# josiahbjorgaard/mca-paper

Hardware: AMD Instinct MI355X
Metric: training samples/sec (fwd+bwd+opt), CMU 4-modality MCA (higher is better)
Workload: dtype bf16; 1 GPU; synthetic CMU 4-modality (MCA fcl), N=2538 D=512 L=5 H=8 F=88, lengths=full, p_drop=0.0; per_gpu_batch=32, global_batch=32, parallelism=dp1, inputs=device-resident, same batch every step, finite_checks=on (device flag, polled), attention_operands=bf16, attention_backward=bf16 one-pass, launch=hipGraph replay (one launch per step), collectives=none

## Files before the change

### include/mca_hip.h

```cpp
#ifndef MCA_HIP_H
#define MCA_HIP_H
#include <stdint.h>

#ifdef __cplusplus
extern "C" {
#endif

typedef void* mca_stream_t;

#define MCA_OK 0
#define MCA_E_BADARG (-1)
#define MCA_E_ALIGN (-2)
#define MCA_E_UNSUPPORTED (-3)
#define MCA_E_LAUNCH (-4)

const char* mca_version(void);

int mca_gemm_nt(const uint16_t* A, int64_t lda, const uint16_t* B, int64_t ldb,
                void* C, int64_t ldc, int out_bf16,
                const float* bias, const float* residual, int64_t ldres, int64_t res_period,
                int64_t M, int64_t N, int64_t K, mca_stream_t stream);

int mca_gemm_nt_lnres(const uint16_t* A, int64_t lda, const uint16_t* B, int64_t ldb, float* C, int64_t ldc,
                      const float* x, int64_t ldx, const float* mean, const float* rstd, const float* gamma,
                      int64_t M, int64_t N, int64_t K, mca_stream_t stream);

int mca_gemm_nt_geglu_bwd(const uint16_t* A, int64_t lda, const uint16_t* B, int64_t ldb, const uint16_t* h,
                          uint16_t* dh, int64_t ldh, int64_t ip, int64_t M, int64_t K, mca_stream_t stream);

int mca_gemm_nt_geglu_fwd(const uint16_t* A, int64_t lda, const uint16_t* W1, int64_t ldb, uint16_t* h, int64_t ldh,
                          uint16_t* g, int64_t ldg, int64_t ip, int64_t M, int64_t K, mca_stream_t stream);

int mca_gemm_tn_acc(const uint16_t* A, int64_t lda, const uint16_t* B, int64_t ldb,
                    float* C, int64_t ldc, int64_t R, int64_t N, int64_t K, mca_stream_t stream);

#define MCA_TN_MAX_GROUP 8
typedef struct mca_tn_desc {
  const uint16_t* A; int64_t lda;
  const uint16_t* B; int64_t ldb;
  float* C; int64_t ldc;
  int64_t N, K;
} mca_tn_desc;
int mca_gemm_tn_acc_group(const mca_tn_desc* d, int n, int64_t R, mca_stream_t stream);

int mca_layernorm_fwd(const float* x, int64_t ldx, const float* gamma, const float* beta,
                      const uint8_t* rowmask, const float* add, int64_t period,
                      float* y, int64_t ldy, int64_t y_bstride,
                      uint16_t* y_bf16, int64_t ld_bf16, int cols_pad,
                      float* mean, float* rstd, int64_t rows, int cols, float eps, mca_stream_t stream);

int mca_layernorm_bwd(const float* dy, int64_t ldy, int64_t y_bstride, int64_t period,
                      const float* x, int64_t ldx, const float* gamma,
                      const float* mean, const float* rstd, const uint8_t* rowmask,
                      float* dx, int64_t lddx, uint16_t* dx_bf16, int64_t ld_bf16,
                      float* dgamma, float* dbeta, float* dxsum, int64_t rows, int cols, mca_stream_t stream);

int mca_geglu_fwd(const uint16_t* h, uint16_t* g, int64_t rows, int ip, mca_stream_t stream);
int mca_geglu_bwd(const uint16_t* dg, const uint16_t* h, uint16_t* dh, int64_t rows, int ip,
                  mca_stream_t stream);

int mca_cast_pad_bf16(const float* src, int64_t lds, int64_t rows, int64_t cols,
                      uint16_t* dst, int64_t ldd, int64_t rows_pad, int64_t cols_pad, int transpose,
                      mca_stream_t stream);
typedef struct { const void* src; void* dst; int64_t lds, rows, cols, ldd, rows_pad, cols_pad; int32_t transpose; float scale; } mca_cast_desc;
int mca_cast_pad_bf16_multi(const mca_cast_desc* descs_dev, int n, mca_stream_t stream);
int mca_f32_to_bf16(const float* src, int64_t lds, uint16_t* dst, int64_t ldd, int64_t rows, int64_t cols,
                    float scale, mca_stream_t stream);
int mca_bcast_rows(const float* src, int64_t lds, float* dst, int64_t ldd, int64_t dst_bstride,
                   int64_t period, int64_t rows, int cols, mca_stream_t stream);
int mca_reduce_rows(const float* src, int64_t lds, int64_t src_bstride, int64_t period,
                    float* dst, int64_t ldd, int64_t rows, int cols, mca_stream_t stream);

int mca_embedding_renorm(float* weight, int64_t rows, int cols, float max_norm, mca_stream_t stream);
int mca_tab_value_fwd(const float* x, const float* w1, const float* b1, uint16_t* h1, uint8_t* padmask,
                      int64_t rows, int cols, float max_value, float padding_value, mca_stream_t stream);
int mca_tab_value_bwd(const float* dh1, int64_t ld, const uint16_t* h1, const float* x, float* dw1, float* db1,
                      int64_t rows, int cols, float max_value, mca_stream_t stream);

#define MCA_MAX_MODALITIES 16
typedef struct { const void* mask; uint8_t* rowmask; int32_t elem_bytes, n, offset, pad_; } mca_mask_desc;
typedef struct { mca_mask_desc m[MCA_MAX_MODALITIES]; int32_t n_mod, batch, n_tokens, n_fusion; } mca_pack_masks_args;
int mca_pack_masks(const mca_pack_masks_args* args, uint8_t* padding, int32_t* present, mca_stream_t stream);

typedef struct { const float* p[MCA_MAX_MODALITIES]; int64_t n[MCA_MAX_MODALITIES]; int32_t count, pad_; } mca_finite_args;
int mca_nonfinite_flag(const mca_finite_args* args, int32_t* flag, int bit, mca_stream_t stream);
int mca_flag_to_host(const int32_t* flag, int32_t* host_pinned, mca_stream_t stream);

int mca_build_keyinfo(const uint8_t* padding, const uint8_t* kgroup, uint8_t* keyinfo,
                      uint8_t* ktile_flags, int batch, int nk, int nk_pad, mca_stream_t stream);

int mca_build_keyhot(const uint8_t* keyinfo, uint16_t* khot, int batch, int nk_pad, mca_stream_t stream);

int mca_attn_vmean(const uint16_t* V, int64_t kv_bstride, int64_t kv_ld, float* vmean,
                   int batch, int nk, int heads, mca_stream_t stream);
int mca_attn_vmean_if_needed(const uint16_t* V, int64_t kv_bstride, int64_t kv_ld, float* vmean, int batch, int nk,
                             int heads, const int32_t* present, int32_t full_bits, mca_stream_t stream);

typedef struct {
  const uint16_t* q; int64_t q_bstride; int64_t q_ld;
  const uint16_t* k; const uint16_t* v; int64_t kv_bstride; int64_t kv_ld;
  uint16_t* o; int64_t o_bstride; int64_t o_ld;
  float* lse;
  const uint32_t* qmask;
  const uint8_t* keyinfo;
  const uint8_t* ktile_flags;
  const int32_t* q_ptr; const uint32_t* q_kt; const int32_t* q_order;
  const float* vmean;
  int batch, heads, nq, nk, nk_pad, n_qtiles, n_ktiles;
  float scale;
  int flags;
  const uint16_t* khot;
} mca_attn_fwd_args;
#define MCA_ATTN_Q_PRESCALED 1
#define MCA_ATTN_LAZY_REFERENCE 2
int mca_attn_fwd(const mca_attn_fwd_args* args, mca_stream_t stream);

int mca_rows_copy_add(const float* src, int64_t src_bstride, float* dst, int64_t dst_bstride, int64_t rows, int cols,
                      int batch, int accumulate, mca_stream_t stream);
int mca_segment_mean_fwd(const float* x, const uint8_t* padding, const int32_t* seg_start, int n_seg, float* out,
                         int32_t* counts, int batch, int n_tokens, int cols, mca_stream_t stream);
int mca_segment_mean_bwd(const float* d_out, const uint8_t* padding, const uint8_t* seg_of_row, const int32_t* counts,
                         int n_seg, float* dx, int batch, int n_tokens, int cols, mca_stream_t stream);

typedef struct { uint8_t* q8; uint8_t* qs; uint8_t* k8; uint8_t* ks; uint8_t* v8t; uint8_t* vs; int n_ktiles; } mca_attn_fp8_operands;
int mca_attn_quant_mxfp8(const uint16_t* q, int64_t q_bstride, int64_t q_ld, const uint16_t* k, const uint16_t* v,
                         int64_t kv_bstride, int64_t kv_ld, const mca_attn_fp8_operands* f, int batch, int heads, int n,
                         mca_stream_t stream);
int mca_attn_fwd_fp8(const mca_attn_fwd_args* args, const mca_attn_fp8_operands* f, mca_stream_t stream);

typedef struct { uint8_t* q8; uint8_t* qs; uint8_t* k8; uint8_t* ks; uint8_t* v8; uint8_t* vs; uint8_t* do8; uint8_t* dos; int n_ktiles; } mca_attn_fp8_bwd_operands;
int mca_attn_quant_bwd_mxfp8(const uint16_t* q, int64_t q_bstride, int64_t q_ld, const uint16_t* k, const uint16_t* v,
                             int64_t kv_bstride, int64_t kv_ld, const uint16_t* d_o, int64_t o_bstride, int64_t o_ld,
                             const mca_attn_fp8_bwd_operands* f, int which, int batch, int heads, int n, mca_stream_t stream);
int mca_attn_bwd_prep(const uint16_t* o, const uint16_t* d_o, int64_t o_bstride, int64_t o_ld,
                      const float* lse, float* delta, float* dvmean,
                      int batch, int heads, int nq, int nk, mca_stream_t stream);

typedef struct {
  const uint16_t* q; int64_t q_bstride; int64_t q_ld;
  const uint16_t* k; const uint16_t* v; int64_t kv_bstride; int64_t kv_ld;
  const uint16_t* d_o; int64_t o_bstride; int64_t o_ld;
  const float* lse; const float* delta; const float* dvmean;
  void* dq; int64_t dq_bstride; int64_t dq_ld; int dq_f32;
  uint16_t* dk; uint16_t* dv; int64_t dkv_bstride; int64_t dkv_ld;
  const uint32_t* qmask; const uint8_t* keyinfo; const uint8_t* ktile_flags;
  const int32_t* q_ptr; const uint32_t* q_kt; const int32_t* q_order; int n_qtiles128, n_ktiles64;
  const int32_t* k_wg; const uint32_t* k_qt; int n_qtiles64, n_kblocks256;
  int batch, heads, nq, nk, nk_pad;
  float scale;
  int flags;
  const uint16_t* khot; const uint16_t* qblk;
  int kblock_keys;
} mca_attn_bwd2_args;
int mca_attn_bwd_dq(const mca_attn_bwd2_args* args, mca_stream_t stream);
int mca_attn_bwd_dkv(const mca_attn_bwd2_args* args, mca_stream_t stream);
int mca_attn_bwd_dq_fp8(const mca_attn_bwd2_args* args, const mca_attn_fp8_bwd_operands* f, mca_stream_t stream);
int mca_attn_bwd_dkv_fp8(const mca_attn_bwd2_args* args, const mca_attn_fp8_bwd_operands* f, mca_stream_t stream);

typedef struct {
  const uint16_t* q; int64_t q_bstride; int64_t q_ld;
  const uint16_t* k; const uint16_t* v; int64_t kv_bstride; int64_t kv_ld;
  const uint16_t* d_o; int64_t o_bstride; int64_t o_ld;
  int64_t q_hstride, o_hstride;
  const float* rowc; const float* dvmean;
  uint16_t* dq; int64_t dq_bstride; int64_t dq_ld;
  uint16_t* dk; uint16_t* dv; int64_t dkv_bstride; int64_t dkv_ld;
  float* dq_acc;
  const uint8_t* keyinfo; const uint8_t* ktile_flags; const uint16_t* khot; const uint16_t* qblk;
  const int32_t* qt_desc; const int32_t* kb_desc; const uint32_t* kb_qt; const uint8_t* visit;
  int n_qtiles, n_kblocks, max_list;
  int n_entries;
  int batch, heads, n, nk_pad, n_ktiles64;
  float scale;
  int flags;
  int split;
} mca_attn_bwd1_args;
int mca_attn_bwd_onepass(const mca_attn_bwd1_args* args, mca_stream_t stream);
int mca_attn_bwd_prep_onepass(const uint16_t* o, const uint16_t* d_o, int64_t o_bstride, int64_t o_ld, const float* lse,
                              const int32_t* row_slot, float* rowc, float* dvmean, int batch, int heads, int n, int n_qtiles,
                              const uint16_t* q, int64_t q_bstride, int64_t q_ld, uint16_t* q_hm, uint16_t* do_hm,
                              mca_stream_t stream);

typedef struct { int32_t slot_a, slot_b; uint32_t and_bits, or_bits; } mca_loss_term;
int64_t mca_contrastive_workspace_bytes(int B, int T);
int mca_contrastive_fwd_bwd(const float* pooled_all, const uint32_t* present_all,
                            const mca_loss_term* terms, int T, const float* logit_scale,
                            int B, int b_local, int row0, int R, int D,
                            float* term_loss, float* loss, float* d_pooled, float* d_logit_scale,
                            void* workspace, mca_stream_t stream);

#define MCA_SQNORM_WORDS 1026
int mca_grad_sqnorm(const float* g, int64_t n, float* sqnorm, mca_stream_t stream);
int mca_adamw_step(float* p, const float* g, float* m, float* v, int64_t n,
                   float lr, float beta1, float beta2, float eps, float weight_decay,
                   float bias_corr1, float bias_corr2, float max_norm, const float* sqnorm,
                   const int32_t* skip_flag, const float* hyper, mca_stream_t stream);
int mca_adamw_hyper(float* hyper, float lr, float bias_corr1, float bias_corr2, mca_stream_t stream);

int mca_rows_normalize_f32(const float* x, int64_t ldx, float* y, int64_t ldy, int64_t n, int64_t d, mca_stream_t stream);
int mca_cosine_rank_f32(const float* q, int64_t ldq, const int32_t* qidx, int64_t nq, const float* t, int64_t ldt, int64_t nt,
                        int64_t d, float* s_true, int32_t* rank, mca_stream_t stream);
int64_t mca_pair_gauss_workspace(int64_t n);
int mca_pair_gauss_sum_f32(const float* x, int64_t ldx, int64_t n, int64_t d, float t, double* partials, int64_t n_partials,
                           double* sum_out, float* value_out, mca_stream_t stream);
int mca_probe_nt_f32(const float* x, int64_t ldx, const int32_t* xidx, const float* w, int64_t ldw, const float* bias, float* y,
                     int64_t ldy, int64_t M, int64_t N, int64_t K, int act, float p, uint64_t seed, int64_t step, mca_stream_t stream);
int64_t mca_probe_head_blocks(int64_t B);
int mca_probe_head_f32(const float* a, int64_t lda, const int32_t* aidx, int64_t K, const float* w, const float* bias, int64_t L,
                       const float* labels, const int32_t* yidx, int64_t B, int loss_type, float* pred, float* dz, float* da,
                       float dact_scale, float* loss_part, mca_stream_t stream);
int64_t mca_probe_tn_workspace(int64_t R, int64_t N, int64_t K);
int mca_probe_tn_f32(const float* a, int64_t lda, const float* b, int64_t ldb, const int32_t* bidx, int64_t R, int64_t N, int64_t K,
                     float* partials, int64_t n_partials, float* gw, float* gb, mca_stream_t stream);
int mca_probe_loss_accum(const float* loss_part, int64_t n, int64_t count, float* acc, mca_stream_t stream);

#ifdef __cplusplus
}
#endif
#endif
```

### mca-paper_amd/csrc/attention_bwd1.hip

```cpp
#include "common.h"

#define DH 64
#define TQ 64
#define TKB 256
#define B1_NST 2
#define B1_STAGE_U16 (TQ * DH * 2 + 256 + TQ * 16)
#define B1_MAX_QT 256
#define B1_MAX_KB 64
#define B1_MAX_LIST 256
#define B1_MAX_META 768
typedef unsigned u32x4v __attribute__((ext_vector_type(4)));
typedef unsigned u32x2v __attribute__((ext_vector_type(2)));

__device__ __forceinline__ int b1_off(int r, int c) {
  const int s = ((r >> 1) & 7) ^ (((r >> 1) & 1) << 2);
  return r * 64 + ((c ^ s) << 3);
}
__device__ __forceinline__ int b1_swz(int r) { return ((r >> 1) & 7) ^ (((r >> 1) & 1) << 2); }

#define B1_DMA(SRC, DST, BYTES) __builtin_amdgcn_global_load_lds((const __attribute__((address_space(1))) void*)(SRC), (__attribute__((address_space(3))) void*)(DST), BYTES, 0, 0)

__global__ __launch_bounds__(256, 1) void attn_bwd1_kernel(mca_attn_bwd1_args a, int dbg) {
  extern __shared__ __attribute__((aligned(16))) u16 lds[];
  u16* stage_s = lds;
  u16* kimg = stage_s + B1_NST * B1_STAGE_U16;
  u16* dsimg = kimg + TKB * DH;
  uint32_t* list_s = reinterpret_cast<uint32_t*>(dsimg + 2 * TKB * TQ);
  uint8_t* first_s = reinterpret_cast<uint8_t*>(list_s + B1_MAX_LIST);
  uint8_t* last_s = first_s + B1_MAX_QT;
  uint8_t* live_s = last_s + B1_MAX_QT;
  float* dvm_s = reinterpret_cast<float*>(live_s + B1_MAX_KB);

  const int lin = (dbg & 16) ? (int)blockIdx.x : xcd_remap((int)blockIdx.x, (int)gridDim.x);
  const int h = lin % a.heads, b = lin / a.heads;
  const int tid = threadIdx.x, lane = tid & 63, wave = __builtin_amdgcn_readfirstlane(tid >> 6);
  const int l31 = lane & 31, lh = lane >> 5;
  const int tq = (lane & 15) >> 2, tp = lane & 3, tg = (lane >> 4) & 1;
  const int64_t bh = (int64_t)b * a.heads + h;

  const u16* qbase = a.q + (int64_t)b * a.q_bstride + h * (a.q_hstride ? a.q_hstride : (int64_t)DH);
  const u16* obase = a.d_o + (int64_t)b * a.o_bstride + h * (a.o_hstride ? a.o_hstride : (int64_t)DH);
  const u16* kbase = a.k + (int64_t)b * a.kv_bstride + h * DH;
  const u16* vbase = a.v + (int64_t)b * a.kv_bstride + h * DH;
  const float* rowc_g = a.rowc + bh * (int64_t)(a.n_qtiles + 1) * 128;
  float* acc_g = a.dq_acc + bh * (int64_t)(a.n_qtiles + 1) * (TQ * DH);
  const uint8_t* kinfo_g = a.keyinfo + (int64_t)b * a.nk_pad;
  const u16* khot_g = a.khot + (int64_t)b * a.nk_pad * 16;

  if (tid < a.n_kblocks) {
    const int4 d = reinterpret_cast<const int4*>(a.kb_desc)[tid];
    const uint8_t* fl = a.ktile_flags + (int64_t)b * a.n_ktiles64;
    int live = 0;
    for (int t = d.x >> 6; t <= (d.x + d.y - 1) >> 6; t++) live |= fl[t];
    live_s[tid] = live ? 1 : 0;
  }
  if (tid < DH) dvm_s[tid] = a.dvmean[(int64_t)b * a.heads * DH + h * DH + tid];
  __syncthreads();
  for (int qt = tid; qt < a.n_qtiles; qt += 256) {
    int first = 255, last = 255;
    for (int kb = 0; kb < a.n_kblocks; kb++)
      if (live_s[kb] && a.visit[kb * a.n_qtiles + qt]) { if (first == 255) first = kb; last = kb; }
    first_s[qt] = (uint8_t)first; last_s[qt] = (uint8_t)last;
  }
  __syncthreads();
  for (int qt = 0; qt < a.n_qtiles; qt++) {
    if (first_s[qt] != 255) continue;
    const int2 qd = reinterpret_cast<const int2*>(a.qt_desc)[qt];
    for (int i = tid; i < qd.y * 8; i += 256)
      *reinterpret_cast<uint4*>(a.dq + (int64_t)b * a.dq_bstride + (int64_t)(qd.x + (i >> 3)) * a.dq_ld + h * DH + (i & 7) * 8) = make_uint4(0, 0, 0, 0);
  }

  int rowfrag[4];
#pragma unroll
  for (int st = 0; st < 4; st++) rowfrag[st] = b1_off(l31, 2 * st + lh);
  const float dk_scale = 0.6931471805599453f;

  for (int kbi = 0; kbi < a.n_kblocks; kbi++) {
    if (!live_s[kbi]) continue;
    const int4 kd = reinterpret_cast<const int4*>(a.kb_desc)[kbi];
    const int key_start = __builtin_amdgcn_readfirstlane(kd.x), n_keys = __builtin_amdgcn_readfirstlane(kd.y);
    const int e_begin = __builtin_amdgcn_readfirstlane(kd.z), n_ent = __builtin_amdgcn_readfirstlane(kd.w);
    for (int i = tid; i < n_ent; i += 256) list_s[i] = a.kb_qt[e_begin + i];

    bf16x8 kf[2][4], vf[2][4], khf[2];
    bool ok[2];
    int keyrow[2];
#pragma unroll
    for (int kb = 0; kb < 2; kb++) {
      const int slot = wave * 64 + kb * 32 + l31;
      const bool valid = slot < n_keys;
      const int key = key_start + (valid ? slot : n_keys - 1);
      keyrow[kb] = valid ? key : -1;
      ok[kb] = valid && kinfo_g[key] != 31;
#pragma unroll
      for (int s = 0; s < 4; s++) {
        kf[kb][s] = *reinterpret_cast<const bf16x8*>(kbase + (int64_t)key * a.kv_ld + 16 * s + 8 * lh);
// ... 280 lines not shown
  asm volatile("s_mov_b32 m0, %2\n\ts_nop 0\n\tglobal_load_lds_dword %0, %1" :: "v"(OFF), "s"(BASE), "s"(LDS_DST) : "memory")
#define LDS_P(T, ADDR) reinterpret_cast<__attribute__((address_space(3))) T*>(static_cast<uintptr_t>(ADDR))
#define LDS_R8(ADDR) (*LDS_P(const bf16x8, ADDR))
#define LDS_RF4(ADDR) (*LDS_P(const f32x4, ADDR))
#define LDS_TR(ADDR) __builtin_amdgcn_ds_read_tr16_b64_v4i16(LDS_P(bf16x4, ADDR))

MCA_TRACE_BUFFER(attn_bwd1)
#ifdef MCA_TRACE_BUILD
#define B1_STAMP() do { if (trace_on) { const unsigned long long t_ = __builtin_amdgcn_s_memtime(); if (lane == 0) mca_trace_attn_bwd1[tr_n & 1023] = t_; tr_n++; } } while (0)
#define B1_NOTE(V) do { if (trace_on) { if (lane == 0) mca_trace_attn_bwd1[tr_n & 1023] = (unsigned long long)(V); tr_n++; } } while (0)
#define B1_TR(K_) asm volatile("s_memtime %0" : "=s"(tr_t[K_]))
#define B1_TR_END() do { asm volatile("s_memtime %0\n\ts_waitcnt lgkmcnt(0)" : "=s"(tr_t[6]) :: "memory");                      \
                         if (trace_on && it == 8 && lane == 0) {                                                                 \
                           for (int k_ = 0; k_ < 7; k_++) mca_trace_attn_bwd1[512 + tr_blk * 8 + k_] = tr_t[k_]; } } while (0)
#else
#define B1_STAMP() do {} while (0)
#define B1_NOTE(V) do {} while (0)
#define B1_TR(K_) do {} while (0)
#define B1_TR_END() do {} while (0)
#endif
#define M_QT(M) ((M).x & 0xffff)
#define M_FIRST(M) (((M).x >> 16) & 1)
#define M_LAST(M) (((M).x >> 17) & 1)
#define M_ROWS(M) ((int)((unsigned)(M).x >> 20))
#define M_ROW0(M) ((M).y)

__device__ __forceinline__ void attn_bwd1p_body(const mca_attn_bwd1_args& a, const int dbg, u16* lds) {
  u16* stage_s = lds;
  u16* kimg = stage_s + B1P_NST * B1_STAGE_U16;
  u16* dsimg = kimg + TKB * DH;
  int2* meta_s = reinterpret_cast<int2*>(dsimg + 2 * TKB * TQ);
  int4* kbd_s = reinterpret_cast<int4*>(meta_s + B1_MAX_META);
  int2* qtd_s = reinterpret_cast<int2*>(dsimg);
  uint8_t* first_s = reinterpret_cast<uint8_t*>(qtd_s + B1_MAX_QT);
  uint8_t* last_s = first_s + B1_MAX_QT;
  uint8_t* live_s = reinterpret_cast<uint8_t*>(kbd_s + B1_MAX_KB);
  float* dvm_s = reinterpret_cast<float*>(live_s + B1_MAX_KB);

  const int lin = (dbg & 16) ? (int)blockIdx.x : xcd_remap((int)blockIdx.x, (int)gridDim.x);
  const int S = a.split > 1 ? a.split : 1;
  const int bh_ = lin / S, sid = lin - bh_ * S;
  const int h = bh_ % a.heads, b = bh_ / a.heads;
  const int tid = threadIdx.x, lane = tid & 63, wave = __builtin_amdgcn_readfirstlane(tid >> 6);
#ifdef MCA_TRACE_BUILD
  const bool trace_on = lin == 0 && wave == 0 && (dbg & 8);
  int tr_n = 0, tr_blk = 0;
#endif
  const int l31 = lane & 31, lh = lane >> 5;
  const int tq = (lane & 15) >> 2, tp = lane & 3, tg = (lane >> 4) & 1;
  const int64_t bh = (int64_t)b * a.heads + h;

  const u16* qbase = a.q + (int64_t)b * a.q_bstride + h * (a.q_hstride ? a.q_hstride : (int64_t)DH);
  const u16* obase = a.d_o + (int64_t)b * a.o_bstride + h * (a.o_hstride ? a.o_hstride : (int64_t)DH);
  const u16* kbase = a.k + (int64_t)b * a.kv_bstride + h * DH;
  const u16* vbase = a.v + (int64_t)b * a.kv_bstride + h * DH;
  const float* rowc_g = a.rowc + bh * (int64_t)(a.n_qtiles + 1) * 128;
  float* acc_s = a.dq_acc + (bh * S + sid) * (int64_t)(a.n_qtiles + 1) * (TQ * DH) + wave * 1024;
  const uint8_t* kinfo_g = a.keyinfo + (int64_t)b * a.nk_pad;
  const u16* khot_g = a.khot + (int64_t)b * a.nk_pad * 16;

  if (tid < a.n_kblocks) {
    const int4 d = reinterpret_cast<const int4*>(a.kb_desc)[tid];
    const uint8_t* fl = a.ktile_flags + (int64_t)b * a.n_ktiles64;
    int live = 0;
    for (int t = d.x >> 6; t <= (d.x + d.y - 1) >> 6; t++) live |= fl[t];
    const bool mine = tid % S == sid;
    live_s[tid] = (live && mine) ? 1 : ((!live && mine) ? 2 : 0);
    kbd_s[tid] = d;
  }
  if (tid < DH) dvm_s[tid] = a.dvmean[(int64_t)b * a.heads * DH + h * DH + tid];
  for (int qt = tid; qt < a.n_qtiles; qt += 256) qtd_s[qt] = reinterpret_cast<const int2*>(a.qt_desc)[qt];
  if (tid == 0) { qtd_s[a.n_qtiles] = make_int2(0, 1); first_s[a.n_qtiles] = 255; last_s[a.n_qtiles] = 255; }
  __syncthreads();
  for (int qt = tid; qt < a.n_qtiles; qt += 256) {
    int first = 255, last = 255;
    for (int kb = 0; kb < a.n_kblocks; kb++)
      if (live_s[kb] == 1 && a.visit[kb * a.n_qtiles + qt]) { if (first == 255) first = kb; last = kb; }
    first_s[qt] = (uint8_t)first; last_s[qt] = (uint8_t)last;
  }
  int* mtot_s = reinterpret_cast<int*>(dvm_s + DH);
  if (tid == 0) {
    int off = 0;
    for (int kb = 0; kb < a.n_kblocks; kb++) {
      int4 d = kbd_s[kb];
      const int e_begin = d.z;
      d.z = off;
      if (live_s[kb] == 1) off += ((d.w + 2) & ~1) + 2;
      kbd_s[kb] = make_int4(d.x, d.y, d.z | (e_begin << 16), d.w);
    }
    *mtot_s = off;
  }
  __syncthreads();
  {
    const int total = *mtot_s;
    for (int e = tid; e < total; e += 256) {
      int kb = 0;
      for (int k = 1; k < a.n_kblocks; k++) if ((kbd_s[k].z & 0xffff) <= e) kb = k;
      while (live_s[kb] != 1) kb--;
      const int4 d = kbd_s[kb];
      const int mo = d.z & 0xffff, e_begin = d.z >> 16, n_ent = d.w, i = e - mo;
      const int qt = i < n_ent ? (int)(a.kb_qt[e_begin + i] & 0x7fffffffu) : a.n_qtiles;
      const int2 qd = qtd_s[qt];
      meta_s[e] = make_int2(qt | (((int)first_s[qt] == kb ? 1 : 0) << 16) | (((int)last_s[qt] == kb && S == 1 ? 2 : 0) << 16) | (qd.y << 20), qd.x);
    }
  }
  __syncthreads();
  for (int qt = 0; qt < a.n_qtiles; qt++) {
    if (first_s[qt] != 255) continue;
// ... 403 lines not shown
    tr_blk++;
#endif
    kbi = nxt;
  }
#ifdef MCA_TRACE_BUILD
  if (trace_on && lane == 0) mca_trace_attn_bwd1[1023] = (unsigned long long)tr_n;
#endif
  for (int kbi = 0; kbi < a.n_kblocks; kbi++) {
    if (live_s[kbi] != 2) continue;
    const int4 kd = reinterpret_cast<const int4*>(a.kb_desc)[kbi];
    for (int i = tid; i < kd.y * 8; i += 256) {
      const int key = kd.x + (i >> 3), c = i & 7;
      *reinterpret_cast<uint4*>(a.dk + (int64_t)b * a.dkv_bstride + (int64_t)key * a.dkv_ld + h * DH + c * 8) = make_uint4(0, 0, 0, 0);
      uint4 pv;
      pv.x = pack2bf(dvm_s[c * 8], dvm_s[c * 8 + 1]); pv.y = pack2bf(dvm_s[c * 8 + 2], dvm_s[c * 8 + 3]);
      pv.z = pack2bf(dvm_s[c * 8 + 4], dvm_s[c * 8 + 5]); pv.w = pack2bf(dvm_s[c * 8 + 6], dvm_s[c * 8 + 7]);
      *reinterpret_cast<uint4*>(a.dv + (int64_t)b * a.dkv_bstride + (int64_t)key * a.dkv_ld + h * DH + c * 8) = pv;
    }
  }
}
__global__ __launch_bounds__(256) void attn_bwd1_reduce_kernel(mca_attn_bwd1_args a) {
  const int qt = blockIdx.x, bh = blockIdx.y, h = bh % a.heads, b = bh / a.heads, S = a.split;
  const int tid = threadIdx.x, lane = tid & 63, wave = tid >> 6;
  const int2 qd = reinterpret_cast<const int2*>(a.qt_desc)[qt];
  const int r = (wave >> 1) * 32 + (lane & 31);
#pragma unroll
  for (int g = 0; g < 4; g++) {
    f32x4 acc = {0.f, 0.f, 0.f, 0.f};
    for (int s = 0; s < S; s++) {
      const f32x4 v = *reinterpret_cast<const f32x4*>(a.dq_acc + (((int64_t)bh * S + s) * (a.n_qtiles + 1) + qt) * (TQ * DH) + wave * 1024 + g * 256 + lane * 4);
      acc[0] += v[0]; acc[1] += v[1]; acc[2] += v[2]; acc[3] += v[3];
    }
    if (r < qd.y) {
      uint2 pk;
      pk.x = pack2bf(acc[0] * a.scale, acc[1] * a.scale); pk.y = pack2bf(acc[2] * a.scale, acc[3] * a.scale);
      *reinterpret_cast<uint2*>(a.dq + (int64_t)b * a.dq_bstride + (int64_t)(qd.x + r) * a.dq_ld + h * DH + (wave & 1) * 32 + 8 * g + 4 * (lane >> 5)) = pk;
    }
  }
}
__global__ __launch_bounds__(256, 1) void attn_bwd1p_kernel(mca_attn_bwd1_args a, int dbg) {
  extern __shared__ __attribute__((aligned(16))) u16 lds_dyn[];
  attn_bwd1p_body(a, dbg, lds_dyn);
}
#define B1P_LDS_BYTES ((B1P_NST * B1_STAGE_U16 + TKB * DH + 2 * TKB * TQ) * 2 + B1_MAX_META * 8 + B1_MAX_KB * 16 + B1_MAX_KB + DH * 4 + 16)

#define B1_LDS_BYTES ((B1_NST * B1_STAGE_U16 + TKB * DH + 2 * TKB * TQ) * 2 + B1_MAX_LIST * 4 + 2 * B1_MAX_QT + B1_MAX_KB + DH * 4)

extern "C" int mca_attn_bwd_onepass(const mca_attn_bwd1_args* a, mca_stream_t stream) {
  if (!a || !a->q || !a->k || !a->v || !a->d_o || !a->rowc || !a->dvmean || !a->dq || !a->dk || !a->dv || !a->dq_acc) return MCA_E_BADARG;
  if (!a->keyinfo || !a->ktile_flags || !a->khot || !a->qblk || !a->qt_desc || !a->kb_desc || !a->kb_qt || !a->visit) return MCA_E_BADARG;
  if (a->batch <= 0 || a->heads <= 0 || a->n <= 0 || a->n_qtiles <= 0 || a->n_kblocks <= 0) return MCA_E_BADARG;
  if (a->n_qtiles >= B1_MAX_QT || a->n_kblocks > B1_MAX_KB || a->max_list + 6 > B1_MAX_LIST ||
      a->n_entries + 4 * a->n_kblocks > B1_MAX_META) return MCA_E_UNSUPPORTED;
  if (a->q_ld % 8 || a->kv_ld % 8 || a->o_ld % 8 || a->q_bstride % 8 || a->kv_bstride % 8 || a->o_bstride % 8 || a->q_hstride % 8 || a->o_hstride % 8) return MCA_E_ALIGN;
  if ((uintptr_t)a->q % 16 || (uintptr_t)a->k % 16 || (uintptr_t)a->v % 16 || (uintptr_t)a->d_o % 16 || (uintptr_t)a->khot % 16 || (uintptr_t)a->qblk % 16) return MCA_E_ALIGN;
  if (a->dq_ld % 8 || a->dq_bstride % 8 || (uintptr_t)a->dq % 16 || a->dkv_ld % 8 || a->dkv_bstride % 8 || (uintptr_t)a->dk % 16 || (uintptr_t)a->dv % 16) return MCA_E_ALIGN;
  if ((uintptr_t)a->dq_acc % 16 || (uintptr_t)a->rowc % 4 || (uintptr_t)a->kb_desc % 16 || (uintptr_t)a->qt_desc % 8) return MCA_E_ALIGN;
  if (a->nk_pad < a->n || a->n_ktiles64 != (a->n + 63) / 64) return MCA_E_BADARG;
  if (!(a->flags & MCA_ATTN_Q_PRESCALED)) return MCA_E_UNSUPPORTED;
  if ((int64_t)a->batch * a->heads > 0x7fffffff) return MCA_E_UNSUPPORTED;
  static bool attr_set[64] = {false};
  bool* done = mca_dev_flag(attr_set);
  if (!*done) {
    if (hipFuncSetAttribute(reinterpret_cast<const void*>(attn_bwd1_kernel), hipFuncAttributeMaxDynamicSharedMemorySize, B1_LDS_BYTES) != hipSuccess ||
        hipFuncSetAttribute(reinterpret_cast<const void*>(attn_bwd1p_kernel), hipFuncAttributeMaxDynamicSharedMemorySize, B1P_LDS_BYTES) != hipSuccess)
      return MCA_E_LAUNCH;
    *done = true;
  }
  const bool packed = a->q_ld == DH && a->o_ld == DH && a->q_hstride && a->o_hstride;
  const int split = a->split > 1 ? a->split : 1;
  if (split > 8) return MCA_E_UNSUPPORTED;
  if (split > 1 && !packed) return MCA_E_UNSUPPORTED;
  if ((mca_knobs[9] & 64 && split == 1) || !packed) hipLaunchKernelGGL(attn_bwd1_kernel, dim3(a->batch * a->heads), dim3(256), B1_LDS_BYTES, as_stream(stream), *a, mca_knobs[9]);
  else hipLaunchKernelGGL(attn_bwd1p_kernel, dim3(a->batch * a->heads * split), dim3(256), B1P_LDS_BYTES, as_stream(stream), *a, mca_knobs[9]);
  if (split > 1) hipLaunchKernelGGL(attn_bwd1_reduce_kernel, dim3(a->n_qtiles, a->batch * a->heads), dim3(256), 0, as_stream(stream), *a);
  return launch_status();
}
```

### mca-paper_amd/csrc/attention_bwd2.hip

```cpp
#include "common.h"

#define DH 64
#define AQ 128
#define AK 64
#define MAX_KTILES 512
#define BQ 64
#define MAX_QTILES 2048
typedef unsigned u32x4v __attribute__((ext_vector_type(4)));

__device__ __forceinline__ int rt_off(int r, int c) {
  const int s = ((r >> 1) & 7) ^ (((r >> 1) & 1) << 2);
  return r * 64 + ((c ^ s) << 3);
}
__device__ __forceinline__ int row_off(int r, int c) { return r * 64 + ((c ^ ((r >> 1) & 7)) << 3); }

template <bool OUT_F32, bool HOT>
__global__ __launch_bounds__(256, 2) void attn_bwd_dq_kernel(mca_attn_bwd2_args a, int dbg) {
  constexpr bool PRESCALED = true;
  __shared__ __attribute__((aligned(16))) u16 lds[2 * 2 * AK * DH];
  __shared__ __attribute__((aligned(16))) uint8_t kinfo[2][AK];
  __shared__ __attribute__((aligned(16))) u16 hot_s[2][AK * 16];
  __shared__ uint8_t flags_s[MAX_KTILES];
  __shared__ uint32_t live_s[MAX_KTILES + 2];
  __shared__ int n_live_s;
// ... 498 lines not shown
#pragma unroll
    for (int n = 0; n < 2; n++)
#pragma unroll
      for (int g = 0; g < 4; g++) {
        const int d = n * 32 + 8 * g + 4 * lh;
        uint2 pk;
        pk.x = pack2bf(dk[n][4 * g] * dk_scale, dk[n][4 * g + 1] * dk_scale);
        pk.y = pack2bf(dk[n][4 * g + 2] * dk_scale, dk[n][4 * g + 3] * dk_scale);
        *reinterpret_cast<uint2*>(dkp + d) = pk;
        const f32x4 dvm = *reinterpret_cast<const f32x4*>(dvm_s + d);
        pk.x = pack2bf(dv[n][4 * g] + dvm[0], dv[n][4 * g + 1] + dvm[1]);
        pk.y = pack2bf(dv[n][4 * g + 2] + dvm[2], dv[n][4 * g + 3] + dvm[3]);
        *reinterpret_cast<uint2*>(dvp + d) = pk;
      }
  }
}
#define DKV_LDS_BYTES (2 * BQ * DH * 2 * 2 + 2 * 192 * 4 + MAX_QTILES * 4 + DH * 4 + 2 * BQ * 16 * 2)

extern "C" int mca_attn_bwd_dkv(const mca_attn_bwd2_args* a, mca_stream_t stream) {
  const int rc = check_bwd2(a);
  if (rc != MCA_OK) return rc;
  if (!a->dk || !a->dv || !a->dvmean || !a->k_wg || !a->k_qt) return MCA_E_BADARG;
  const int BKEYS = a->kblock_keys ? a->kblock_keys : 256;
  if (BKEYS != 256 && BKEYS != 128) return MCA_E_UNSUPPORTED;
  if (a->n_qtiles64 != (a->nq + BQ - 1) / BQ || a->n_kblocks256 != (a->nk + BKEYS - 1) / BKEYS) return MCA_E_BADARG;
  if (a->nk_pad < a->n_kblocks256 * BKEYS) return MCA_E_BADARG;
  if (a->dkv_ld % 4 || a->dkv_bstride % 4 || (uintptr_t)a->dk % 8 || (uintptr_t)a->dv % 8 || (uintptr_t)a->k_wg % 16) return MCA_E_ALIGN;
  if (a->n_qtiles64 > MAX_QTILES) return MCA_E_UNSUPPORTED;
  if ((a->khot != nullptr) != (a->qblk != nullptr)) return MCA_E_BADARG;
  if ((uintptr_t)a->khot % 16 || (uintptr_t)a->qblk % 16) return MCA_E_ALIGN;
  if (!(a->flags & MCA_ATTN_Q_PRESCALED)) return MCA_E_UNSUPPORTED;
  int dev = 0;
  static bool attr_set[64] = {false};
  if (hipGetDevice(&dev) != hipSuccess || dev < 0 || dev >= 64) return MCA_E_LAUNCH;
  if (!attr_set[dev]) {
    if (hipFuncSetAttribute(reinterpret_cast<const void*>(attn_bwd_dkv_kernel<8>), hipFuncAttributeMaxDynamicSharedMemorySize, DKV_LDS_BYTES) != hipSuccess ||
        hipFuncSetAttribute(reinterpret_cast<const void*>(attn_bwd_dkv_kernel<4>), hipFuncAttributeMaxDynamicSharedMemorySize, DKV_LDS_BYTES) != hipSuccess)
      return MCA_E_LAUNCH;
    attr_set[dev] = true;
  }
  const dim3 grid(a->n_kblocks256, a->heads, a->batch);
#define DKV_LAUNCH(W) hipLaunchKernelGGL((attn_bwd_dkv_kernel<W>), grid, dim3(64 * W), DKV_LDS_BYTES, as_stream(stream), *a, mca_knobs[9])
  if (BKEYS == 256) DKV_LAUNCH(8); else DKV_LAUNCH(4);
#undef DKV_LAUNCH
  return launch_status();
}

#define PREP_ROWS 32
__device__ __forceinline__ void attn_bwd_prep_block(const int bx, const int by, const u16* __restrict__ o, const u16* __restrict__ d_o,
                                                    int64_t bstride, int64_t ld, float* __restrict__ delta, int heads, int nq,
                                                    const float* __restrict__ lse, const int32_t* __restrict__ row_slot,
                                                    float* __restrict__ rowc, int n_qtiles,
                                                    const u16* __restrict__ qsrc, int64_t q_bstride, int64_t q_ld,
                                                    u16* __restrict__ q_hm, u16* __restrict__ do_hm) {
  __shared__ float del_s[8][PREP_ROWS];
  const int b = by, tid = threadIdx.x, lane = tid & 63, wave = tid >> 6;
  const int cols = heads * DH;
  const int q_begin = bx * PREP_ROWS;
  int q_end = q_begin + PREP_ROWS; if (q_end > nq) q_end = nq;
  for (int c0 = 0; c0 < cols; c0 += 512) {
    const int h0 = c0 / DH;
    const int c = c0 + lane * 8;
    const int hl = lane >> 3;
    bf16x8 ovs[PREP_ROWS / 4], dvs[PREP_ROWS / 4], qvs[PREP_ROWS / 4];
#pragma unroll
    for (int k = 0; k < PREP_ROWS / 4; k++) {
      int q = q_begin + wave + 4 * k; if (q > nq - 1) q = nq - 1;
      const int cc = c < cols ? c : 0;
      ovs[k] = *reinterpret_cast<const bf16x8*>(o + (int64_t)b * bstride + (int64_t)q * ld + cc);
      dvs[k] = *reinterpret_cast<const bf16x8*>(d_o + (int64_t)b * bstride + (int64_t)q * ld + cc);
      if (do_hm) qvs[k] = *reinterpret_cast<const bf16x8*>(qsrc + (int64_t)b * q_bstride + (int64_t)q * q_ld + cc);
    }
#pragma unroll
    for (int k = 0; k < PREP_ROWS / 4; k++) {
      const int q = q_begin + wave + 4 * k;
      if (q >= q_end) break;
      if (do_hm && c < cols) {
        const int64_t dst = (((int64_t)b * heads + h0 + hl) * nq + q) * DH + (lane & 7) * 8;
        *reinterpret_cast<bf16x8*>(do_hm + dst) = dvs[k];
        *reinterpret_cast<bf16x8*>(q_hm + dst) = qvs[k];
      }
      float part = 0.f;
      if (c < cols) {
#pragma unroll
        for (int j = 0; j < 8; j++) part += bf2f((u16)dvs[k][j]) * bf2f((u16)ovs[k][j]);
      }
      part += __shfl_xor(part, 1, WAVE); part += __shfl_xor(part, 2, WAVE); part += __shfl_xor(part, 4, WAVE);
      if ((lane & 7) == 0) del_s[hl][q - q_begin] = part;
    }
    __syncthreads();
    {
      const int hh = tid / PREP_ROWS, r = tid % PREP_ROWS;
      if (h0 + hh < heads && q_begin + r < q_end) {
        if (!row_slot) delta[((int64_t)b * heads + h0 + hh) * nq + q_begin + r] = del_s[hh][r];
        else {
          const int q = q_begin + r, slot = row_slot[q];
          float* dst = rowc + (((int64_t)b * heads + h0 + hh) * (n_qtiles + 1) + (slot >> 6)) * 128 + (slot & 63);
          dst[0] = -lse[((int64_t)b * heads + h0 + hh) * nq + q];
          dst[64] = -del_s[hh][r];
        }
      }
    }
    __syncthreads();
  }
}

#define DVM_MAX_LIST 4096
__device__ __forceinline__ void attn_dvmean_block(const int bx, const int by, const u16* __restrict__ d_o, int64_t bstride, int64_t ld,
                                                  const float* __restrict__ lse, float* __restrict__ dvmean,
                                                  int heads, int nq, float inv_nk) {
  __shared__ int list_s[DVM_MAX_LIST];
  __shared__ int n_s;
  __shared__ float red[32][DH + 1];
  const int h = bx, b = by, tid = threadIdx.x, lane = tid & 63, wave = tid >> 6;
  const float* l = lse + ((int64_t)b * heads + h) * nq;
  float* out = dvmean + (int64_t)b * heads * DH + h * DH;
  {
    int anyu = 0;
    for (int q = tid; q < nq; q += 256) anyu |= (l[q] == INFINITY) ? 1 : 0;
    if (tid == 0) n_s = 0;
    if (!__syncthreads_or(anyu)) { if (tid < DH) out[tid] = 0.f; return; }
  }
  const int cl = tid & 7, rg = tid >> 3;
  float acc[8] = {0, 0, 0, 0, 0, 0, 0, 0};
  auto flush = [&]() {
    const int n = n_s;
    for (int i = rg; i < n; i += 32) {
      const bf16x8 v = *reinterpret_cast<const bf16x8*>(d_o + (int64_t)b * bstride + (int64_t)list_s[i] * ld + h * DH + cl * 8);
#pragma unroll
      for (int j = 0; j < 8; j++) acc[j] += bf2f((u16)v[j]);
    }
    __syncthreads();
    if (tid == 0) n_s = 0;
    __syncthreads();
  };
  for (int q0 = 0; q0 < nq; q0 += 256) {
    const int q = q0 + tid;
    const bool uni = q < nq && l[q] == INFINITY;
    const unsigned long long m = __ballot(uni);
    for (int w = 0; w < 4; w++) {
      if (wave == w && m) {
        const int base = n_s;
        if (uni) list_s[base + __popcll(m & ((1ull << lane) - 1ull))] = q;
        if (lane == 0) n_s = base + __popcll(m);
      }
      __syncthreads();
    }
    if (n_s > DVM_MAX_LIST - 256) flush();
  }
  flush();
#pragma unroll
  for (int j = 0; j < 8; j++) red[rg][cl * 8 + j] = acc[j];
  __syncthreads();
  if (tid < DH) {
    float t = 0.f;
    for (int r = 0; r < 32; r++) t += red[r][tid];
    out[tid] = t * inv_nk;
  }
}
__global__ __launch_bounds__(256) void attn_bwd_prep_kernel(const u16* __restrict__ o, const u16* __restrict__ d_o, int64_t bstride, int64_t ld,
                                                             const float* __restrict__ lse, float* __restrict__ delta,
                                                             float* __restrict__ dvmean, int heads, int nq, float inv_nk, int n_prep,
                                                             const int32_t* __restrict__ row_slot, float* __restrict__ rowc, int n_qtiles,
                                                             const u16* __restrict__ qsrc, int64_t q_bstride, int64_t q_ld,
                                                             u16* __restrict__ q_hm, u16* __restrict__ do_hm) {
  if ((int)blockIdx.x < n_prep) attn_bwd_prep_block((int)blockIdx.x, (int)blockIdx.y, o, d_o, bstride, ld, delta, heads, nq, lse, row_slot, rowc, n_qtiles,
                                                    qsrc, q_bstride, q_ld, q_hm, do_hm);
  else attn_dvmean_block((int)blockIdx.x - n_prep, (int)blockIdx.y, d_o, bstride, ld, lse, dvmean, heads, nq, inv_nk);
}
extern "C" int mca_attn_bwd_prep(const uint16_t* o, const uint16_t* d_o, int64_t o_bstride, int64_t o_ld,
                                 const float* lse, float* delta, float* dvmean, int batch, int heads, int nq, int nk,
                                 mca_stream_t stream) {
  if (!o || !d_o || !lse || !delta || !dvmean || batch <= 0 || heads <= 0 || nq <= 0 || nk <= 0) return MCA_E_BADARG;
  if (o_ld % 8 || o_bstride % 8 || (uintptr_t)o % 16 || (uintptr_t)d_o % 16) return MCA_E_ALIGN;
  if (heads > 65535 || batch > 65535) return MCA_E_UNSUPPORTED;
  const int n_prep = (nq + PREP_ROWS - 1) / PREP_ROWS;
  hipLaunchKernelGGL(attn_bwd_prep_kernel, dim3(n_prep + heads, batch), dim3(256), 0, as_stream(stream), o, d_o, o_bstride, o_ld, lse, delta,
                     dvmean, heads, nq, 1.f / (float)nk, n_prep, (const int32_t*)nullptr, (float*)nullptr, 0, (const u16*)nullptr, (int64_t)0, (int64_t)0,
                     (u16*)nullptr, (u16*)nullptr);
  return launch_status();
}
extern "C" int mca_attn_bwd_prep_onepass(const uint16_t* o, const uint16_t* d_o, int64_t o_bstride, int64_t o_ld, const float* lse,
                                         const int32_t* row_slot, float* rowc, float* dvmean, int batch, int heads, int n, int n_qtiles,
                                         const uint16_t* q, int64_t q_bstride, int64_t q_ld, uint16_t* q_hm, uint16_t* do_hm,
                                         mca_stream_t stream) {
  if (!o || !d_o || !lse || !row_slot || !rowc || !dvmean || batch <= 0 || heads <= 0 || n <= 0 || n_qtiles <= 0) return MCA_E_BADARG;
  if ((q_hm != nullptr) != (do_hm != nullptr) || (q_hm && !q)) return MCA_E_BADARG;
  if (q_hm && (q_ld % 8 || q_bstride % 8 || (uintptr_t)q % 16 || (uintptr_t)q_hm % 16 || (uintptr_t)do_hm % 16)) return MCA_E_ALIGN;
  if (o_ld % 8 || o_bstride % 8 || (uintptr_t)o % 16 || (uintptr_t)d_o % 16) return MCA_E_ALIGN;
  if (heads > 65535 || batch > 65535) return MCA_E_UNSUPPORTED;
  const int n_prep = (n + PREP_ROWS - 1) / PREP_ROWS;
  hipLaunchKernelGGL(attn_bwd_prep_kernel, dim3(n_prep + heads, batch), dim3(256), 0, as_stream(stream), o, d_o, o_bstride, o_ld, lse, (float*)nullptr,
                     dvmean, heads, n, 1.f / (float)n, n_prep, row_slot, rowc, n_qtiles, q, q_bstride, q_ld, q_hm, do_hm);
  return launch_status();
}
```

### mca-paper_amd/csrc/attention_fwd.hip

```cpp
#include "common.h"

#define AQ 128
#define AK 64
#define DH 64
#define MAX_KTILES 512
typedef unsigned u32x4v __attribute__((ext_vector_type(4)));

MCA_TRACE_BUFFER(attn_fwd)
#ifdef MCA_TRACE_BUILD
#define FW_STAMP() do { if (tracing && ti < 1017) mca_trace_attn_fwd[ti++] = __builtin_readcyclecounter(); } while (0)
#else
#define FW_STAMP() do { } while (0)
#endif

__device__ __forceinline__ int k_off(int r, int c) { return r * 64 + ((c ^ ((r >> 1) & 7)) << 3); }
__device__ __forceinline__ int v_off(int r, int c) { return r * 64 + ((c ^ (((r >> 1) & 1) << 2)) << 3); }

__global__ __launch_bounds__(256) void attn_fwd_kernel(mca_attn_fwd_args a, int dbg) {
  constexpr bool PRESCALED = true;
  __shared__ __attribute__((aligned(16))) u16 lds[2 * 2 * AK * DH];
  __shared__ __attribute__((aligned(16))) uint8_t kinfo[2][AK];
  __shared__ __attribute__((aligned(16))) u16 hot_s[2][AK * 16];
  __shared__ uint8_t flags_s[MAX_KTILES];
  __shared__ uint32_t live_s[MAX_KTILES];
  __shared__ int n_live_s;
  u16* Ks = lds;
  u16* Vs = lds + 2 * AK * DH;

  const int lin0 = (int)(blockIdx.x + gridDim.x * (blockIdx.y + gridDim.y * blockIdx.z));
  const int lin = (dbg & 16) ? lin0 : xcd_remap(lin0, (int)(gridDim.x * gridDim.y * gridDim.z));
  const int qt = a.q_order[lin % (int)gridDim.x];
  const int h = (lin / (int)gridDim.x) % (int)gridDim.y, b = lin / (int)(gridDim.x * gridDim.y);
  const int tid = threadIdx.x, lane = tid & 63, wave = tid >> 6;
  const int l31 = lane & 31, lh = lane >> 5;
  const int q0 = qt * AQ + wave * 32;
  int qrow = q0 + l31;
  const bool qvalid = qrow < a.nq;
  if (qrow > a.nq - 1) qrow = a.nq - 1;

  bf16x8 qf[4];
  {
    const u16* qp = a.q + (int64_t)b * a.q_bstride + (int64_t)qrow * a.q_ld + h * DH + 8 * lh;
#pragma unroll
    for (int s = 0; s < 4; s++) qf[s] = *reinterpret_cast<const bf16x8*>(qp + 16 * s);
  }
  const uint32_t qm = a.qmask[qrow];
  const bool use_hot = a.khot != nullptr;
  bf16x8 qblk;
#pragma unroll
  for (int j = 0; j < 8; j++) {
    const int g = 8 * lh + j;
    qblk[j] = (g < 15 && ((qm >> g) & 1u)) ? (short)0 : (short)0xC700;
  }
  const float c2 = PRESCALED ? 1.f : a.scale * 1.4426950408889634f;

  f32x16 o[2];
#pragma unroll
  for (int n = 0; n < 2; n++)
#pragma unroll
    for (int r = 0; r < 16; r++) o[n][r] = 0.f;
  float m_run = -INFINITY, l_run = 0.f;

  const u16* kbase = a.k + (int64_t)b * a.kv_bstride + h * DH;
  const u16* vbase = a.v + (int64_t)b * a.kv_bstride + h * DH;
  const uint8_t* kinfo_g = a.keyinfo + (int64_t)b * a.nk_pad;
  const u16* khot_g = use_hot ? a.khot + (int64_t)b * a.nk_pad * 16 : nullptr;
  {
    const uint8_t* flags_g = a.ktile_flags + (int64_t)b * a.n_ktiles;
    for (int i = tid; i < a.n_ktiles; i += 256) flags_s[i] = flags_g[i];
  }
  __syncthreads();

  int srow[2], sc[2];
  unsigned loff[2];
#pragma unroll
  for (int i = 0; i < 2; i++) {
    const int id = tid + 256 * i; srow[i] = id >> 3; sc[i] = id & 7;
    loff[i] = (unsigned)(srow[i] * (int)a.kv_ld + sc[i] * 8);
  }
  const int last_kt = a.n_ktiles - 1;
  bf16x8 rk[2], rv[2];
  uint32_t rinfo = 0;
  uint4 rhot = make_uint4(0, 0, 0, 0);
  auto gload = [&](int kt) {
    if (use_hot) { if (tid < 128) rhot = *reinterpret_cast<const uint4*>(khot_g + ((int64_t)kt * AK + (tid >> 1)) * 16 + (tid & 1) * 8); }
    else if (tid < 16) rinfo = *reinterpret_cast<const uint32_t*>(kinfo_g + kt * AK + tid * 4);
    const u16* kb = kbase + (int64_t)kt * AK * a.kv_ld;
    const u16* vb = vbase + (int64_t)kt * AK * a.kv_ld;
    if (kt != last_kt) {
#pragma unroll
      for (int i = 0; i < 2; i++) {
        rk[i] = *reinterpret_cast<const bf16x8*>(kb + loff[i]);
        rv[i] = *reinterpret_cast<const bf16x8*>(vb + loff[i]);
      }
    } else {
#pragma unroll
      for (int i = 0; i < 2; i++) {
        int key = kt * AK + srow[i]; if (key > a.nk - 1) key = a.nk - 1;
        rk[i] = *reinterpret_cast<const bf16x8*>(kbase + (int64_t)key * a.kv_ld + sc[i] * 8);
        rv[i] = *reinterpret_cast<const bf16x8*>(vbase + (int64_t)key * a.kv_ld + sc[i] * 8);
      }
    }
  };
  auto swrite = [&](int buf) {
#pragma unroll
    for (int i = 0; i < 2; i++) {
      *reinterpret_cast<bf16x8*>(Ks + buf * AK * DH + k_off(srow[i], sc[i])) = rk[i];
      *reinterpret_cast<bf16x8*>(Vs + buf * AK * DH + v_off(srow[i], sc[i])) = rv[i];
    }
    if (use_hot) { if (tid < 128) *reinterpret_cast<uint4*>(&hot_s[buf][(tid >> 1) * 16 + (tid & 1) * 8]) = rhot; }
    else if (tid < 16) *reinterpret_cast<uint32_t*>(&kinfo[buf][tid * 4]) = rinfo;
  };

  if (wave == 0) {
    const int lb = a.q_ptr[qt], le = a.q_ptr[qt + 1];
    int n = 0;
    for (int i0 = lb; i0 < le; i0 += 64) {
// ... 115 lines not shown
    buf ^= 1;
    it = nit;
  }

#ifdef MCA_TRACE_BUILD
  if (tracing) {
    mca_trace_attn_fwd[1020] = __builtin_amdgcn_s_memrealtime() - rt0; mca_trace_attn_fwd[1021] = __builtin_readcyclecounter() - cy0;
  }
#endif
  const bool uniform = !(l_run > 0.f) || m_run < -16384.f * c2;
  const float inv = uniform ? 0.f : 1.f / l_run;
  if (qvalid) {
    if (lh == 0) a.lse[((int64_t)b * a.heads + h) * a.nq + qrow] = uniform ? INFINITY : m_run + log2f(l_run);
    u16* op = a.o + (int64_t)b * a.o_bstride + (int64_t)qrow * a.o_ld + h * DH;
    const float* vm = a.vmean + (int64_t)b * a.heads * DH + h * DH;
#pragma unroll
    for (int n = 0; n < 2; n++)
#pragma unroll
      for (int g = 0; g < 4; g++) {
        const int d = n * 32 + 8 * g + 4 * lh;
        float v0, v1, v2, v3;
        if (uniform) { v0 = vm[d]; v1 = vm[d + 1]; v2 = vm[d + 2]; v3 = vm[d + 3]; }
        else { v0 = o[n][4 * g] * inv; v1 = o[n][4 * g + 1] * inv; v2 = o[n][4 * g + 2] * inv; v3 = o[n][4 * g + 3] * inv; }
        uint2 pk; pk.x = pack2bf(v0, v1); pk.y = pack2bf(v2, v3);
        *reinterpret_cast<uint2*>(op + d) = pk;
      }
  }
}



__global__ __launch_bounds__(256, 4) void attn_fwd4_kernel(mca_attn_fwd_args a, int dbg) {
  __shared__ __attribute__((aligned(16))) u16 lds[2 * 2 * AK * DH + 2 * AK * 16];
  __shared__ uint8_t flags_s[MAX_KTILES];
  __shared__ uint32_t live_s[MAX_KTILES];
  __shared__ int n_live_s;
  u16* Ks = lds;
  u16* Vs = lds + 2 * AK * DH;
  u16* Hs = lds + 4 * AK * DH;

  const int lin0 = (int)(blockIdx.x + gridDim.x * (blockIdx.y + gridDim.y * blockIdx.z));
  const int lin = (dbg & 16) ? lin0 : xcd_remap(lin0, (int)(gridDim.x * gridDim.y * gridDim.z));
  const int qt = a.q_order[lin % (int)gridDim.x];
  const int h = (lin / (int)gridDim.x) % (int)gridDim.y, b = lin / (int)(gridDim.x * gridDim.y);
  const int tid = threadIdx.x, lane = tid & 63, wave = __builtin_amdgcn_readfirstlane(tid >> 6);
  const int l31 = lane & 31, lh = lane >> 5;
  const int q0 = qt * AQ + wave * 32;
  int qrow = q0 + l31;
  const bool qvalid = qrow < a.nq;
  if (qrow > a.nq - 1) qrow = a.nq - 1;

  bf16x8 qf[4];
  {
    const u16* qp = a.q + (int64_t)b * a.q_bstride + (int64_t)qrow * a.q_ld + h * DH + 8 * lh;
#pragma unroll
    for (int s = 0; s < 4; s++) qf[s] = *reinterpret_cast<const bf16x8*>(qp + 16 * s);
  }
  const uint32_t qm = a.qmask[qrow];
  const uint32_t qm8 = ((qm >> (8 * lh)) & 0xffu) & (lh ? 0x7fu : 0xffu);

  f32x16 o[2];
#pragma unroll
  for (int n = 0; n < 2; n++)
#pragma unroll
    for (int r = 0; r < 16; r++) o[n][r] = 0.f;
  float m_run = -INFINITY, l_run = 0.f;

  const u16* kbase = a.k + (int64_t)b * a.kv_bstride + h * DH;
  const u16* vbase = a.v + (int64_t)b * a.kv_bstride + h * DH;
  const u16* khot_g = a.khot + (int64_t)b * a.nk_pad * 16;
  {
    const uint8_t* flags_g = a.ktile_flags + (int64_t)b * a.n_ktiles;
    for (int i = tid; i < a.n_ktiles; i += 256) flags_s[i] = flags_g[i];
  }
  __syncthreads();

  int prow[2];
  unsigned koff[2], voff[2];
#pragma unroll
  for (int i = 0; i < 2; i++) {
    const int p = 256 * i + tid, r = p >> 3, sl = p & 7;
    prow[i] = r;
    koff[i] = (unsigned)(r * (int)a.kv_ld + ((sl ^ ((r >> 1) & 7)) << 3));
    voff[i] = (unsigned)(r * (int)a.kv_ld + ((sl ^ (((r >> 1) & 1) << 2)) << 3));
  }
  const int last_kt = a.n_ktiles - 1;
  auto stage = [&](int kt, int buf) {
    const u16* kb = kbase + (int64_t)kt * AK * a.kv_ld;
    const u16* vb = vbase + (int64_t)kt * AK * a.kv_ld;
#pragma unroll
    for (int i = 0; i < 2; i++) {
      unsigned ko = koff[i], vo = voff[i];
      if (kt == last_kt) {
        int key = kt * AK + prow[i]; const int over = key - (a.nk - 1);
        if (over > 0) { ko -= (unsigned)(over * (int)a.kv_ld); vo -= (unsigned)(over * (int)a.kv_ld); }
      }
      u16* dk = Ks + buf * AK * DH + (i * 4 + wave) * 512;
      u16* dv = Vs + buf * AK * DH + (i * 4 + wave) * 512;
      __builtin_amdgcn_global_load_lds((const __attribute__((address_space(1))) void*)(kb + ko), (__attribute__((address_space(3))) void*)dk, 16, 0, 0);
      __builtin_amdgcn_global_load_lds((const __attribute__((address_space(1))) void*)(vb + vo), (__attribute__((address_space(3))) void*)dv, 16, 0, 0);
    }
    if (wave < 2) {
      u16* dh = Hs + buf * AK * 16 + wave * 512;
      __builtin_amdgcn_global_load_lds((const __attribute__((address_space(1))) void*)(khot_g + (int64_t)kt * (AK * 16) + tid * 8),
                                       (__attribute__((address_space(3))) void*)dh, 16, 0, 0);
    }
  };

  if (wave == 0) {
    const int lb = a.q_ptr[qt], le = a.q_ptr[qt + 1];
    int n = 0;
    for (int i0 = lb; i0 < le; i0 += 64) {
      const int i = i0 + lane;
      const uint32_t e = i < le ? a.q_kt[i] : 0u;
      const uint8_t fl = i < le ? flags_s[e & 0x7fffffffu] : (uint8_t)0;
      const bool keep = fl != 0;
      const unsigned long long m = __ballot(keep);
      if (keep) live_s[n + __popcll(m & ((1ull << lane) - 1ull))] = (e & 0x7fffffffu) | (((e >> 31) && fl == 2) ? 0x80000000u : 0u);
      n += __popcll(m);
    }
    if (lane == 0) n_live_s = n;
  }
// ... 75 lines not shown
            const bf16x4 v4 = lds_read_tr16(vs + v_off(key, d >> 3) + (d & 7));
#pragma unroll
            for (int e = 0; e < 4; e++) vf[4 * t + e] = v4[e];
          }
          o[n] = __builtin_amdgcn_mfma_f32_32x32x16_bf16(vf, *reinterpret_cast<const bf16x8*>(&pw[kb][sp]), o[n], 0, 0, 0);
        }
    asm volatile("s_waitcnt vmcnt(0)" ::: "memory");
    __syncthreads();
    buf ^= 1;
  }

  const bool uniform = !(l_run > 0.f) || m_run < -16384.f;
  const float inv = uniform ? 0.f : 1.f / l_run;
  if (qvalid) {
    if (lh == 0) a.lse[((int64_t)b * a.heads + h) * a.nq + qrow] = uniform ? INFINITY : m_run + log2f(l_run);
    u16* op = a.o + (int64_t)b * a.o_bstride + (int64_t)qrow * a.o_ld + h * DH;
    const float* vm = a.vmean + (int64_t)b * a.heads * DH + h * DH;
#pragma unroll
    for (int n = 0; n < 2; n++)
#pragma unroll
      for (int g = 0; g < 4; g++) {
        const int d = n * 32 + 8 * g + 4 * lh;
        float v0, v1, v2, v3;
        if (uniform) { v0 = vm[d]; v1 = vm[d + 1]; v2 = vm[d + 2]; v3 = vm[d + 3]; }
        else { v0 = o[n][4 * g] * inv; v1 = o[n][4 * g + 1] * inv; v2 = o[n][4 * g + 2] * inv; v3 = o[n][4 * g + 3] * inv; }
        uint2 pk; pk.x = pack2bf(v0, v1); pk.y = pack2bf(v2, v3);
        *reinterpret_cast<uint2*>(op + d) = pk;
      }
  }
}

__global__ __launch_bounds__(256, 3) void attn_fwd4l_kernel(mca_attn_fwd_args a, int dbg, float thr) {
  __shared__ __attribute__((aligned(16))) u16 lds[2 * 2 * AK * DH + 2 * AK * 16];
  __shared__ uint8_t flags_s[MAX_KTILES];
  __shared__ uint32_t live_s[MAX_KTILES];
  __shared__ int n_live_s;
  u16* Ks = lds;
  u16* Vs = lds + 2 * AK * DH;
  u16* Hs = lds + 4 * AK * DH;

  const int lin0 = (int)(blockIdx.x + gridDim.x * (blockIdx.y + gridDim.y * blockIdx.z));
  const int lin = (dbg & 16) ? lin0 : xcd_remap(lin0, (int)(gridDim.x * gridDim.y * gridDim.z));
  const int qt = a.q_order[lin % (int)gridDim.x];
  const int h = (lin / (int)gridDim.x) % (int)gridDim.y, b = lin / (int)(gridDim.x * gridDim.y);
  const int tid = threadIdx.x, lane = tid & 63, wave = __builtin_amdgcn_readfirstlane(tid >> 6);
  const int l31 = lane & 31, lh = lane >> 5;
  const int q0 = qt * AQ + wave * 32;
  int qrow = q0 + l31;
  const bool qvalid = qrow < a.nq;
  if (qrow > a.nq - 1) qrow = a.nq - 1;

  bf16x8 qf[4];
  {
    const u16* qp = a.q + (int64_t)b * a.q_bstride + (int64_t)qrow * a.q_ld + h * DH + 8 * lh;
#pragma unroll
    for (int s = 0; s < 4; s++) qf[s] = *reinterpret_cast<const bf16x8*>(qp + 16 * s);
  }
  const uint32_t qm = a.qmask[qrow];
  const uint32_t qm8 = ((qm >> (8 * lh)) & 0xffu) & (lh ? 0x7fu : 0xffu);

  f32x16 o[2];
#pragma unroll
  for (int n = 0; n < 2; n++)
#pragma unroll
    for (int r = 0; r < 16; r++) o[n][r] = 0.f;
  f32x16 negm;
#pragma unroll
  for (int r = 0; r < 16; r++) negm[r] = 0.f;
  float l_run = 0.f;

  const u16* kbase = a.k + (int64_t)b * a.kv_bstride + h * DH;
  const u16* vbase = a.v + (int64_t)b * a.kv_bstride + h * DH;
  const u16* khot_g = a.khot + (int64_t)b * a.nk_pad * 16;
  {
    const uint8_t* flags_g = a.ktile_flags + (int64_t)b * a.n_ktiles;
    for (int i = tid; i < a.n_ktiles; i += 256) flags_s[i] = flags_g[i];
  }
  __syncthreads();

  int prow[2];
  unsigned koff[2], voff[2];
#pragma unroll
  for (int i = 0; i < 2; i++) {
    const int p = 256 * i + tid, r = p >> 3, sl = p & 7;
    prow[i] = r;
    koff[i] = (unsigned)(r * (int)a.kv_ld + ((sl ^ ((r >> 1) & 7)) << 3));
    voff[i] = (unsigned)(r * (int)a.kv_ld + ((sl ^ (((r >> 1) & 1) << 2)) << 3));
  }
  const int last_kt = a.n_ktiles - 1;
  auto stage = [&](int kt, int buf) {
    const u16* kb = kbase + (int64_t)kt * AK * a.kv_ld;
    const u16* vb = vbase + (int64_t)kt * AK * a.kv_ld;
#pragma unroll
    for (int i = 0; i < 2; i++) {
      unsigned ko = koff[i], vo = voff[i];
      if (kt == last_kt) {
        int key = kt * AK + prow[i]; const int over = key - (a.nk - 1);
        if (over > 0) { ko -= (unsigned)(over * (int)a.kv_ld); vo -= (unsigned)(over * (int)a.kv_ld); }
      }
      u16* dk = Ks + buf * AK * DH + (i * 4 + wave) * 512;
      u16* dv = Vs + buf * AK * DH + (i * 4 + wave) * 512;
      __builtin_amdgcn_global_load_lds((const __attribute__((address_space(1))) void*)(kb + ko), (__attribute__((address_space(3))) void*)dk, 16, 0, 0);
      __builtin_amdgcn_global_load_lds((const __attribute__((address_space(1))) void*)(vb + vo), (__attribute__((address_space(3))) void*)dv, 16, 0, 0);
    }
    if (wave < 2) {
      u16* dh = Hs + buf * AK * 16 + wave * 512;
      __builtin_amdgcn_global_load_lds((const __attribute__((address_space(1))) void*)(khot_g + (int64_t)kt * (AK * 16) + tid * 8),
                                       (__attribute__((address_space(3))) void*)dh, 16, 0, 0);
    }
  };

  if (wave == 0) {
    const int lb = a.q_ptr[qt], le = a.q_ptr[qt + 1];
    int n = 0;
    for (int i0 = lb; i0 < le; i0 += 64) {
      const int i = i0 + lane;
      const uint32_t e = i < le ? a.q_kt[i] : 0u;
      const uint8_t fl = i < le ? flags_s[e & 0x7fffffffu] : (uint8_t)0;
      const bool keep = fl != 0;
      const unsigned long long m = __ballot(keep);
      if (keep) live_s[n + __popcll(m & ((1ull << lane) - 1ull))] = (e & 0x7fffffffu) | (((e >> 31) && fl == 2) ? 0x80000000u : 0u);
      n += __popcll(m);
    }
    if (lane == 0) n_live_s = n;
  }
// ... 71 lines not shown
#pragma unroll
      for (int sp = 0; sp < 2; sp++)
#pragma unroll
        for (int n = 0; n < 2; n++) {
          bf16x8 vf;
#pragma unroll
          for (int t = 0; t < 2; t++) {
            const int key = kb * 32 + 16 * sp + 8 * t + 4 * lh + tq;
            const int d = n * 32 + 16 * tg + 4 * tp;
            const bf16x4 v4 = lds_read_tr16(vs + v_off(key, d >> 3) + (d & 7));
#pragma unroll
            for (int e = 0; e < 4; e++) vf[4 * t + e] = v4[e];
          }
          o[n] = __builtin_amdgcn_mfma_f32_32x32x16_bf16(vf, *reinterpret_cast<const bf16x8*>(&pw[kb][sp]), o[n], 0, 0, 0);
        }
    asm volatile("s_waitcnt vmcnt(0)" ::: "memory");
    __syncthreads();
    buf ^= 1;
  }

  const float l_tot = l_run + __shfl_xor(l_run, 32, WAVE);
  const float m_run = -negm[0];
  const bool uniform = !(l_tot > 0.f);
  const float inv = uniform ? 0.f : 1.f / l_tot;
  if (qvalid) {
    if (lh == 0) a.lse[((int64_t)b * a.heads + h) * a.nq + qrow] = uniform ? INFINITY : m_run + log2f(l_tot);
    u16* op = a.o + (int64_t)b * a.o_bstride + (int64_t)qrow * a.o_ld + h * DH;
    const float* vm = a.vmean + (int64_t)b * a.heads * DH + h * DH;
#pragma unroll
    for (int n = 0; n < 2; n++)
#pragma unroll
      for (int g = 0; g < 4; g++) {
        const int d = n * 32 + 8 * g + 4 * lh;
        float v0, v1, v2, v3;
        if (uniform) { v0 = vm[d]; v1 = vm[d + 1]; v2 = vm[d + 2]; v3 = vm[d + 3]; }
        else { v0 = o[n][4 * g] * inv; v1 = o[n][4 * g + 1] * inv; v2 = o[n][4 * g + 2] * inv; v3 = o[n][4 * g + 3] * inv; }
        uint2 pk; pk.x = pack2bf(v0, v1); pk.y = pack2bf(v2, v3);
        *reinterpret_cast<uint2*>(op + d) = pk;
      }
  }
}

extern "C" int mca_attn_fwd(const mca_attn_fwd_args* a, mca_stream_t stream) {
  if (!a || !a->q || !a->k || !a->v || !a->o || !a->lse || !a->qmask || !a->keyinfo || !a->ktile_flags || !a->q_ptr ||
      !a->q_kt || !a->q_order || !a->vmean)
    return MCA_E_BADARG;
  if (a->batch <= 0 || a->heads <= 0 || a->nq <= 0 || a->nk <= 0) return MCA_E_BADARG;
  if (a->n_qtiles != (a->nq + AQ - 1) / AQ || a->n_ktiles != (a->nk + AK - 1) / AK) return MCA_E_BADARG;
  if (a->nk_pad < a->n_ktiles * AK || a->nk_pad % 4) return MCA_E_BADARG;
  if (a->q_ld % 8 || a->kv_ld % 8 || a->o_ld % 4 || a->q_bstride % 8 || a->kv_bstride % 8 || a->o_bstride % 4) return MCA_E_ALIGN;
  if ((uintptr_t)a->q % 16 || (uintptr_t)a->k % 16 || (uintptr_t)a->v % 16 || (uintptr_t)a->o % 8 ||
      (uintptr_t)a->keyinfo % 4)
    return MCA_E_ALIGN;
  if (a->heads > 65535 || a->batch > 65535 || a->n_ktiles > MAX_KTILES) return MCA_E_UNSUPPORTED;
  const dim3 grid(a->n_qtiles, a->heads, a->batch);
  if (!(a->flags & MCA_ATTN_Q_PRESCALED)) return MCA_E_UNSUPPORTED;
  if ((uintptr_t)a->khot % 16) return MCA_E_ALIGN;
  const bool dma = a->khot && (int64_t)a->kv_ld * 64 < (1ll << 30);
  if (dma && (a->flags & MCA_ATTN_LAZY_REFERENCE))
    hipLaunchKernelGGL(attn_fwd4l_kernel, grid, dim3(256), 0, as_stream(stream), *a, mca_knobs[9], 12.f);
  else if (dma)
    hipLaunchKernelGGL(attn_fwd4_kernel, grid, dim3(256), 0, as_stream(stream), *a, mca_knobs[9]);
  else
    hipLaunchKernelGGL(attn_fwd_kernel, grid, dim3(256), 0, as_stream(stream), *a, mca_knobs[9] | mca_knobs[8]);
  return launch_status();
}

__global__ __launch_bounds__(64) void build_keyinfo_kernel(const uint8_t* __restrict__ padding,
                                                            const uint8_t* __restrict__ kgroup,
                                                            uint8_t* __restrict__ keyinfo, uint8_t* __restrict__ flags,
                                                            int nk, int nk_pad, int n_ktiles) {
  const int b = blockIdx.y, kt = blockIdx.x, lane = threadIdx.x;
  const int key = kt * AK + lane;
  uint8_t info = 31;
  if (key < nk && !padding[(int64_t)b * nk + key]) info = kgroup[key];
  if (key < nk_pad) keyinfo[(int64_t)b * nk_pad + key] = info;
  const unsigned long long valid = __ballot(info != 31);
  if (lane == 0 && kt < n_ktiles) {
    const int in_tile = (nk - kt * AK) < AK ? (nk - kt * AK) : AK;
    const int nvalid = __popcll(valid);
    flags[(int64_t)b * n_ktiles + kt] = nvalid == 0 ? 0 : (nvalid == AK && in_tile == AK ? 2 : 1);
  }
}
extern "C" int mca_build_keyinfo(const uint8_t* padding, const uint8_t* kgroup, uint8_t* keyinfo,
                                 uint8_t* ktile_flags, int batch, int nk, int nk_pad, mca_stream_t stream) {
  if (!padding || !kgroup || !keyinfo || !ktile_flags || batch <= 0 || nk <= 0) return MCA_E_BADARG;
  const int n_ktiles = (nk + AK - 1) / AK;
  if (nk_pad < n_ktiles * AK) return MCA_E_BADARG;
  const int ntile_pad = (nk_pad + AK - 1) / AK;
  hipLaunchKernelGGL(build_keyinfo_kernel, dim3(ntile_pad, batch), dim3(64), 0, as_stream(stream), padding, kgroup,
                     keyinfo, ktile_flags, nk, nk_pad, n_ktiles);
  return launch_status();
}

__global__ __launch_bounds__(256) void build_keyhot_kernel(const uint8_t* __restrict__ keyinfo, u16* __restrict__ khot, int64_t n) {
  const int64_t i = (int64_t)blockIdx.x * 256 + threadIdx.x;
  if (i >= n) return;
  const int g = keyinfo[i] >= 15 ? 15 : keyinfo[i];
  uint32_t w[8];
#pragma unroll
  for (int k = 0; k < 8; k++) w[k] = (g >> 1) == k ? (0x3F80u << (16 * (g & 1))) : 0u;
  uint4* dst = reinterpret_cast<uint4*>(khot + i * 16);
  dst[0] = make_uint4(w[0], w[1], w[2], w[3]);
  dst[1] = make_uint4(w[4], w[5], w[6], w[7]);
}
extern "C" int mca_build_keyhot(const uint8_t* keyinfo, uint16_t* khot, int batch, int nk_pad, mca_stream_t stream) {
  if (!keyinfo || !khot || batch <= 0 || nk_pad <= 0) return MCA_E_BADARG;
  if ((uintptr_t)khot % 16) return MCA_E_ALIGN;
  const int64_t n = (int64_t)batch * nk_pad;
  hipLaunchKernelGGL(build_keyhot_kernel, dim3((unsigned)((n + 255) / 256)), dim3(256), 0, as_stream(stream), keyinfo, khot, n);
  return launch_status();
}

__global__ __launch_bounds__(512) void vmean_kernel(const u16* __restrict__ V, int64_t bstride, int64_t ld,
                                                     float* __restrict__ vmean, int nk, int cols,
                                                     const int32_t* __restrict__ present, int32_t full_bits) {
  __shared__ float red[64][65];
  const int b = blockIdx.y, c0 = blockIdx.x * 64;
  if (present && present[b] == full_bits) return;
  const int cl = threadIdx.x & 7, rg = threadIdx.x >> 3;
  const u16* base = V + (int64_t)b * bstride + c0 + cl * 8;
  float acc[8] = {0, 0, 0, 0, 0, 0, 0, 0};
  for (int j = rg; j < nk; j += 64) {
    const bf16x8 v = *reinterpret_cast<const bf16x8*>(base + (int64_t)j * ld);
#pragma unroll
    for (int e = 0; e < 8; e++) acc[e] += bf2f((u16)v[e]);
  }
#pragma unroll
  for (int e = 0; e < 8; e++) red[rg][cl * 8 + e] = acc[e];
  __syncthreads();
  if (threadIdx.x < 64) {
    float t = 0.f;
    for (int r = 0; r < 64; r++) t += red[r][threadIdx.x];
    vmean[(int64_t)b * cols + c0 + threadIdx.x] = t * (1.f / (float)nk);
  }
}
extern "C" int mca_attn_vmean(const uint16_t* V, int64_t kv_bstride, int64_t kv_ld, float* vmean, int batch, int nk,
                              int heads, mca_stream_t stream) {
  if (!V || !vmean || batch <= 0 || nk <= 0 || heads <= 0) return MCA_E_BADARG;
  const int cols = heads * DH;
  if (kv_ld % 8 || kv_bstride % 8 || (uintptr_t)V % 16) return MCA_E_ALIGN;
  if (batch > 65535) return MCA_E_UNSUPPORTED;
  hipLaunchKernelGGL(vmean_kernel, dim3(heads, batch), dim3(512), 0, as_stream(stream), V, kv_bstride, kv_ld, vmean, nk, cols,
                     (const int32_t*)nullptr, 0);
  return launch_status();
}
extern "C" int mca_attn_vmean_if_needed(const uint16_t* V, int64_t kv_bstride, int64_t kv_ld, float* vmean, int batch, int nk,
                                        int heads, const int32_t* present, int32_t full_bits, mca_stream_t stream) {
  if (!V || !vmean || !present || batch <= 0 || nk <= 0 || heads <= 0) return MCA_E_BADARG;
  const int cols = heads * DH;
  if (kv_ld % 8 || kv_bstride % 8 || (uintptr_t)V % 16) return MCA_E_ALIGN;
  if (batch > 65535) return MCA_E_UNSUPPORTED;
  hipLaunchKernelGGL(vmean_kernel, dim3(heads, batch), dim3(512), 0, as_stream(stream), V, kv_bstride, kv_ld, vmean, nk, cols,
                     present, full_bits);
  return launch_status();
}
```

### mca-paper_amd/csrc/gemm.hip

```cpp
#include "common.h"

#define g_knob mca_knobs

#define BM 128
#define BN 128
#define BK 64

static int num_cus() {
  static int n = 0;
  if (!n) {
    int dev = 0;
    if (hipGetDevice(&dev) != hipSuccess || hipDeviceGetAttribute(&n, hipDeviceAttributeMultiprocessorCount, dev) != hipSuccess || n <= 0) n = 256;
  }
  return n;
}

#define PS_PANELS 4
__device__ __forceinline__ void ps_tile_decode(int tile, int tiles_m, int tiles_n, int flat, int& tm, int& tn) {
  if (flat == 1) { tm = tile / tiles_n; tn = tile % tiles_n; return; }
  const int P = flat > 1 ? flat : PS_PANELS;
  const int per_group = P * tiles_n;
  const int g = tile / per_group;
  const int gh = (g + 1) * P <= tiles_m ? P : tiles_m - g * P;
  const int rem = tile - g * per_group;
// ... 604 lines not shown
#pragma unroll
            for (int e = 0; e < 4; e++) {
              float t = __uint_as_float(o[u][e]);
              if (BIAS) t += __uint_as_float(bvec[0][e]);
              if (MODE == 2) t += __uint_as_float(pre[(i * 8 + u) % NPRE][e]);
              ov[e] = __float_as_uint(t);
            }
            float* cp = reinterpret_cast<float*>(Cv) + (int64_t)m * ldc + nw + 4 * (lane & 15);
            if (m < M) PS_GSTORE(cp, ov);
          }
        } else {
          u32x4v o[4][2];
#pragma unroll
          for (int u = 0; u < 4; u++) {
            const int row = (lane >> 3) + 8 * u, ch = 2 * (lane & 7);
            NT_DSREAD(o[u][0], scratch + (unsigned)(row * 256 + ((ch ^ (row & 15)) << 4)));
            NT_DSREAD(o[u][1], scratch + (unsigned)(row * 256 + (((ch + 1) ^ (row & 15)) << 4)));
          }
          asm volatile("s_waitcnt lgkmcnt(0)" ::: "memory");
#pragma unroll
          for (int u = 0; u < 4; u++) {
            const int m = mw + i * 32 + (lane >> 3) + 8 * u;
            const u32x4v av = pre[((i * 4 + u) * 2) % NPRE], gv = pre[((i * 4 + u) * 2 + 1) % NPRE];
            u32x4v da, dgt;
#pragma unroll
            for (int e = 0; e < 4; e++) {
              const float d0 = __uint_as_float(o[u][e >> 1][2 * (e & 1)]), d1 = __uint_as_float(o[u][e >> 1][2 * (e & 1) + 1]);
              const float a0 = __uint_as_float(av[e] << 16), a1 = __uint_as_float(av[e] & 0xffff0000u);
              const float g0 = __uint_as_float(gv[e] << 16), g1 = __uint_as_float(gv[e] & 0xffff0000u);
              float ge0, dge0, ge1, dge1;
              gelu_pair(g0, ge0, dge0); gelu_pair(g1, ge1, dge1);
              da[e] = pack2bf(d0 * ge0, d1 * ge1);
              dgt[e] = pack2bf(d0 * a0 * dge0, d1 * a1 * dge1);
            }
            u16* cp = reinterpret_cast<u16*>(Cv) + (int64_t)m * ldc + nw + 8 * (lane & 7);
            if (m < M) { PS_GSTORE(cp, da); PS_GSTORE(cp + N, dgt); }
          }
        }
      }
    }
    if (edge) ps_wait_vm<0>();
    PS_STAMP();
    first = false;
    v = vn;
  }
}


#define P2_STAGE (512 * 32)
#define P2_LDS_BYTES (5 * P2_STAGE * 2)
template <bool GEGLU>
__global__ __launch_bounds__(512) void gemm_nt_persist256_kernel(
    const u16* __restrict__ A, int64_t lda, const u16* __restrict__ B, int64_t ldb, u16* __restrict__ C, int64_t ldc,
    u16* __restrict__ G, int64_t ldg, int M, int N, int K, int tiles_n, int nwg, int dbg) {
  extern __shared__ __attribute__((aligned(16))) u16 lds2[];
  constexpr int NST = GEGLU ? 24 : 16;
  const int tid = threadIdx.x, lane = tid & 63, wave = tid >> 6;
  const int wm = wave >> 1, wn = wave & 1;
  const int l31 = lane & 31, lh = lane >> 5;
  const int nkt = K / 32;
  const int tiles_m = nwg / tiles_n;
  const unsigned lds_base = (unsigned)(uintptr_t)(__attribute__((address_space(3))) const u16*)lds2;
  const unsigned scratch = lds_base + 3u * (unsigned)(P2_STAGE * 2) + (unsigned)wave * 8192u;

  unsigned fa_addr[2], fb_addr[4];
#pragma unroll
  for (int i = 0; i < 2; i++) { const int r = wm * 64 + i * 32 + l31; fa_addr[i] = lds_base + (unsigned)(r * 64 + ((lh ^ gl_sw<32>(r)) << 4)); }
#pragma unroll
  for (int j = 0; j < 4; j++) { const int r = wn * 128 + j * 32 + l31; fb_addr[j] = lds_base + 256u * 64u + (unsigned)(r * 64 + ((lh ^ gl_sw<32>(r)) << 4)); }

  const u16* ga[2];
  const u16* gb[2];
  auto tile_ptrs = [&](int tile) {
    int tm, tn;
    ps_tile_decode(tile, tiles_m, tiles_n, 0, tm, tn);
    const int m0 = tm * 256, n0 = tn * 256;
#pragma unroll
    for (int i = 0; i < 2; i++) {
      const int p = (i * 8 + wave) * 64 + lane, r = p >> 2, c = (p & 3) ^ gl_sw<32>(r);
      int ra = m0 + r; if (ra > M - 1) ra = M - 1;
      ga[i] = A + (int64_t)ra * lda + c * 8;
      const int rb = GEGLU ? (r < 128 ? tn * 128 + r : N + tn * 128 + (r - 128)) : n0 + r;
      gb[i] = B + (int64_t)rb * ldb + c * 8;
    }
  };
  auto stage = [&](int k0, int st) {
    u16* base = lds2 + st * P2_STAGE;
#pragma unroll
    for (int i = 0; i < 2; i++) {
      __builtin_amdgcn_global_load_lds((const __attribute__((address_space(1))) void*)(ga[i] + k0),
                                       (__attribute__((address_space(3))) void*)(base + (i * 8 + wave) * 512), 16, 0, 0);
      __builtin_amdgcn_global_load_lds((const __attribute__((address_space(1))) void*)(gb[i] + k0),
                                       (__attribute__((address_space(3))) void*)(base + 256 * 32 + (i * 8 + wave) * 512), 16, 0, 0);
    }
  };

  int v = blockIdx.x;
  if (v >= nwg) return;
  tile_ptrs(xcd_remap(v, nwg));
  stage(0, 0); stage(32, 1); stage(64, 2);
  bool first = true;
  while (v < nwg) {
    const int tile = xcd_remap(v, nwg);
    int tm, tn;
    ps_tile_decode(tile, tiles_m, tiles_n, 0, tm, tn);
    const int m0 = tm * 256, n0 = tn * 256;
    f32x16 acc[2][4];
// ... 26 lines not shown
      if (kt < 2) { if (first) asm volatile("s_waitcnt vmcnt(8) lgkmcnt(0)" ::: "memory"); else { asm volatile("s_waitcnt lgkmcnt(0)" ::: "memory"); ps_wait_vm<8 + NST>(); } }
      else if (kt + 3 < nkt) asm volatile("s_waitcnt vmcnt(8) lgkmcnt(0)" ::: "memory");
      else if (kt + 2 < nkt) asm volatile("s_waitcnt vmcnt(4) lgkmcnt(0)" ::: "memory");
      else asm volatile("s_waitcnt vmcnt(0) lgkmcnt(0)" ::: "memory");
      __builtin_amdgcn_s_barrier();
      P2_SB
      const unsigned son = (unsigned)nxt * (unsigned)(P2_STAGE * 2);
      const bool fetch = kt + 4 < nkt;
      P2_GROUP_READING(1, 0, son, if (fetch) stage((kt + 4) * 32, prev); P2_SB)
      prev = slot; slot = nxt;
    }
    {
      const unsigned so = (unsigned)slot * (unsigned)(P2_STAGE * 2);
      asm volatile("s_waitcnt lgkmcnt(0)" ::: "memory"); P2_SB
      P2_GROUP_READING(0, 1, so, )
      asm volatile("s_waitcnt lgkmcnt(0)" ::: "memory"); P2_SB
      P2_MM(1, 0, 0) P2_MM(1, 0, 1) P2_MM(1, 0, 2) P2_MM(1, 0, 3) P2_MM(1, 1, 0) P2_MM(1, 1, 1) P2_MM(1, 1, 2) P2_MM(1, 1, 3)
    }
#undef P2_SB
#undef P2_RA
#undef P2_RB
#undef P2_MM
#undef P2_GROUP_READING
    __builtin_amdgcn_s_barrier();
    const int mw = m0 + wm * 64, nw = GEGLU ? (wn == 0 ? tn * 128 : N + tn * 128) : n0 + wn * 128;
    const bool edge = m0 + 256 > M;
    const int vn = v + gridDim.x;
    const bool has_next = vn < nwg;
    if (has_next) {
      tile_ptrs(xcd_remap(vn, nwg));
      stage(0, 0); stage(32, 1); stage(64, 2);
    }
#pragma unroll
    for (int i = 0; i < 2; i++) {
#pragma unroll
      for (int j = 0; j < 4; j++)
#pragma unroll
        for (int q = 0; q < 4; q++) {
          u32x2v pk;
          pk[0] = pack2bf(acc[i][j][4 * q], acc[i][j][4 * q + 1]); pk[1] = pack2bf(acc[i][j][4 * q + 2], acc[i][j][4 * q + 3]);
          const int ch = j * 4 + q;
          PS_DSW64(scratch + (unsigned)(l31 * 256 + ((ch ^ (l31 & 15)) << 4) + 8 * lh), pk);
        }
      u32x4v o[8];
#pragma unroll
      for (int u = 0; u < 8; u++) {
        const int row = (lane >> 4) + 4 * u, ch = lane & 15;
        NT_DSREAD(o[u], scratch + (unsigned)(row * 256 + ((ch ^ (row & 15)) << 4)));
      }
      asm volatile("s_waitcnt lgkmcnt(0)" ::: "memory");
#pragma unroll
      for (int u = 0; u < 8; u++) {
        const int m = mw + i * 32 + (lane >> 4) + 4 * u;
        u16* cp = C + (int64_t)m * ldc + nw + 8 * (lane & 15);
        if (m < M) PS_GSTORE(cp, o[u]);
      }
      if (GEGLU) {
        asm volatile("s_waitcnt lgkmcnt(0)\n\ts_barrier" ::: "memory");
        const unsigned sa = lds_base + 3u * (unsigned)(P2_STAGE * 2) + (unsigned)(wave & ~1) * 8192u, sg = sa + 8192u;
        u32x4v av[4], gv[4];
#pragma unroll
        for (int u = 0; u < 4; u++) {
          const int row = 16 * wn + (lane >> 4) + 4 * u, ch = lane & 15;
          NT_DSREAD(av[u], sa + (unsigned)(row * 256 + ((ch ^ (row & 15)) << 4)));
          NT_DSREAD(gv[u], sg + (unsigned)(row * 256 + ((ch ^ (row & 15)) << 4)));
        }
        asm volatile("s_waitcnt lgkmcnt(0)" ::: "memory");
#pragma unroll
        for (int u = 0; u < 4; u++) {
          const int m = m0 + wm * 64 + i * 32 + 16 * wn + (lane >> 4) + 4 * u;
          u32x4v gg;
#pragma unroll
          for (int e = 0; e < 4; e++) {
            const float a0 = __uint_as_float(av[u][e] << 16), a1 = __uint_as_float(av[u][e] & 0xffff0000u);
            const float g0 = __uint_as_float(gv[u][e] << 16), g1 = __uint_as_float(gv[u][e] & 0xffff0000u);
            float ge0, ge1, unused;
            gelu_pair(g0, ge0, unused); gelu_pair(g1, ge1, unused);
            gg[e] = pack2bf(a0 * ge0, a1 * ge1);
          }
          u16* gp = G + (int64_t)m * ldg + tn * 128 + 8 * (lane & 15);
          if (m < M) PS_GSTORE(gp, gg);
        }
        if (i == 0) asm volatile("s_barrier" ::: "memory");
      }
    }
    if (edge) ps_wait_vm<0>();
    first = false;
    v = vn;
  }
}

extern "C" int mca_gemm_nt(const uint16_t* A, int64_t lda, const uint16_t* B, int64_t ldb, void* C, int64_t ldc,
                           int out_bf16, const float* bias, const float* residual, int64_t ldres,
                           int64_t res_period, int64_t M, int64_t N, int64_t K, mca_stream_t stream) {
  if (!A || !B || !C || M <= 0 || N <= 0 || K <= 0) return MCA_E_BADARG;
  if (K % 64 || lda % 8 || ldb % 8 || (uintptr_t)A % 16 || (uintptr_t)B % 16) return MCA_E_ALIGN;
  if (lda < K || ldb < K || ldc < N) return MCA_E_BADARG;
  if (M > (1LL << 30) || N > (1LL << 30)) return MCA_E_UNSUPPORTED;
  const int tiles_m = (int)((M + BM - 1) / BM), tiles_n = (int)((N + BN - 1) / BN);
  const int nwg = tiles_m * tiles_n;
  const int res = !residual ? 0 : (res_period > 0 ? 2 : 1);
  const bool big = M >= 2048 && g_knob[1] != 1;
  const int nwg2 = (int)((M + BM2 - 1) / BM2) * tiles_n;
#define NT_LAUNCH_G(OB, RS)                                                                                              \
  hipLaunchKernelGGL((gemm_nt_glds_kernel<OB, RS, 64, 0>), dim3(nwg), dim3(256), 0, as_stream(stream), A, lda, B, ldb, C,   \
                     ldc, bias, residual, ldres, res_period, (int)M, (int)N, (int)K, tiles_n, nwg)
#define NT_LAUNCH_256(OB, RS, PFV)                                                                                          \
  do {                                                                                                                   \
    static bool attr_dev[64] = {false}; bool& attr = *mca_dev_flag(attr_dev);                                                                                            \
    if (!attr) {                                                                                                         \
      if (hipFuncSetAttribute(reinterpret_cast<const void*>(gemm_nt_256_kernel<OB, RS, PFV, 0>),                            \
                              hipFuncAttributeMaxDynamicSharedMemorySize, NT256_LDS_BYTES) != hipSuccess)                \
        return MCA_E_LAUNCH;                                                                                             \
      attr = true;                                                                                                       \
    }                                                                                                                    \
    hipLaunchKernelGGL((gemm_nt_256_kernel<OB, RS, PFV, 0>), dim3(nwg2), dim3(512), NT256_LDS_BYTES, as_stream(stream), A, lda, \
                       B, ldb, C, ldc, bias, residual, ldres, res_period, (int)M, (int)N, (int)K, tiles_n, nwg2);        \
  } while (0)
#define NT_PICK_PF(OB, RS) do { if (big) NT_LAUNCH_256(OB, RS, 0); else NT_LAUNCH_G(OB, RS); } while (0)
  const bool c16 = (uintptr_t)C % 16 == 0 && ldc % (out_bf16 ? 8 : 4) == 0;
  const bool ps_res = res == 1 && !out_bf16 && ldres % 4 == 0 && (uintptr_t)residual % 16 == 0 && g_knob[7] == 3;
  if (big && g_knob[7] == 0 && g_knob[10] != 1 && out_bf16 && res == 0 && !bias && N % 256 == 0 && K >= 192 && K % 32 == 0 && c16) {
    static bool attr_dev[64] = {false}; bool& attr = *mca_dev_flag(attr_dev);
    if (!attr) {
      if (hipFuncSetAttribute(reinterpret_cast<const void*>(gemm_nt_persist256_kernel<false>), hipFuncAttributeMaxDynamicSharedMemorySize,
                              P2_LDS_BYTES) != hipSuccess)
        return MCA_E_LAUNCH;
      attr = true;
    }
    const int tn2 = (int)(N / 256), nw2 = (int)((M + 255) / 256) * tn2;
    const int grid = nw2 < num_cus() ? nw2 : num_cus();
    hipLaunchKernelGGL(gemm_nt_persist256_kernel<false>, dim3(grid), dim3(512), P2_LDS_BYTES, as_stream(stream), A, lda, B, ldb,
                       reinterpret_cast<u16*>(C), ldc, (u16*)nullptr, (int64_t)0, (int)M, (int)N, (int)K, tn2, nw2, g_knob[0]);
    return launch_status();
  }
  if (big && (g_knob[7] == 0 || g_knob[7] == 3) && N % BN == 0 && K >= 320 && c16 && (res == 0 || ps_res) && (!bias || (uintptr_t)bias % 16 == 0)) {
    const int grid = nwg2 < num_cus() ? nwg2 : num_cus();
#define NT_LAUNCH_PS(MODE, BI)                                                                                               \
  do {                                                                                                                   \
    static bool attr_dev[64] = {false}; bool& attr = *mca_dev_flag(attr_dev);                                                                                            \
    if (!attr) {                                                                                                         \
      if (hipFuncSetAttribute(reinterpret_cast<const void*>(gemm_nt_persist_kernel<MODE, BI>),                           \
                              hipFuncAttributeMaxDynamicSharedMemorySize, NTPS_LDS_BYTES) != hipSuccess)                 \
        return MCA_E_LAUNCH;                                                                                             \
      attr = true;                                                                                                       \
    }                                                                                                                    \
    hipLaunchKernelGGL((gemm_nt_persist_kernel<MODE, BI>), dim3(grid), dim3(512), NTPS_LDS_BYTES, as_stream(stream), A, lda, B, \
                       ldb, C, ldc, bias, residual, ldres, (int)M, (int)N, (int)K, tiles_n, nwg2, g_knob[0]);            \
  } while (0)
    if (out_bf16) { if (bias) NT_LAUNCH_PS(0, true); else NT_LAUNCH_PS(0, false); }
    else if (res == 0) { if (bias) NT_LAUNCH_PS(1, true); else NT_LAUNCH_PS(1, false); }
    else { if (bias) NT_LAUNCH_PS(2, true); else NT_LAUNCH_PS(2, false); }
    return launch_status();
  }
  const bool pf = big && !out_bf16 && res == 1 && N % BN == 0 && K >= 512 && ldres % 4 == 0 && ldc % 4 == 0 &&
                  (uintptr_t)residual % 16 == 0 && (uintptr_t)C % 16 == 0 && (!bias || (uintptr_t)bias % 4 == 0) && g_knob[4] != 1;
  if (pf) { NT_LAUNCH_256(false, 1, 1); return launch_status(); }
  if (out_bf16) { if (res == 0) NT_PICK_PF(true, 0); else if (res == 1) NT_PICK_PF(true, 1); else NT_PICK_PF(true, 2); }
  else { if (res == 0) NT_PICK_PF(false, 0); else if (res == 1) NT_PICK_PF(false, 1); else NT_PICK_PF(false, 2); }
  return launch_status();
}


extern "C" int mca_gemm_nt_lnres(const uint16_t* A, int64_t lda, const uint16_t* B, int64_t ldb, float* C, int64_t ldc,
                                 const float* x, int64_t ldx, const float* mean, const float* rstd, const float* gamma,
                                 int64_t M, int64_t N, int64_t K, mca_stream_t stream) {
  if (!A || !B || !C || !x || !mean || !rstd || !gamma || M <= 0 || N <= 0 || K <= 0) return MCA_E_BADARG;
  if (K % 64 || lda % 8 || ldb % 8 || ldc % 4 || ldx % 4 || (uintptr_t)A % 16 || (uintptr_t)B % 16 || (uintptr_t)C % 16 ||
      (uintptr_t)x % 16 || (uintptr_t)gamma % 16)
    return MCA_E_ALIGN;
  if (lda < K || ldb < K || ldc < N || ldx < N) return MCA_E_BADARG;
  if (M < 2048 || M > (1LL << 30) || N % BN || K < 512) return MCA_E_UNSUPPORTED;
  const int tiles_n = (int)(N / BN);
  const int nwg2 = (int)((M + BM2 - 1) / BM2) * tiles_n;
  static bool attr_dev[64] = {false}; bool& attr = *mca_dev_flag(attr_dev);
  if (!attr) {
    if (hipFuncSetAttribute(reinterpret_cast<const void*>(gemm_nt_256_kernel<false, 1, 1, 2>), hipFuncAttributeMaxDynamicSharedMemorySize,
                            NT256LN_LDS_BYTES) != hipSuccess)
      return MCA_E_LAUNCH;
    attr = true;
  }
  hipLaunchKernelGGL((gemm_nt_256_kernel<false, 1, 1, 2>), dim3(nwg2), dim3(512), NT256LN_LDS_BYTES, as_stream(stream), A, lda, B, ldb,
                     (void*)C, ldc, (const float*)nullptr, x, ldx, (int64_t)0, (int)M, (int)N, (int)K, tiles_n, nwg2, mean, rstd, gamma);
  return launch_status();
}

extern "C" int mca_gemm_nt_geglu_bwd(const uint16_t* A, int64_t lda, const uint16_t* B, int64_t ldb, const uint16_t* h,
                                     uint16_t* dh, int64_t ldh, int64_t ip, int64_t M, int64_t K, mca_stream_t stream) {
  if (!A || !B || !h || !dh || M <= 0 || ip <= 0 || K <= 0) return MCA_E_BADARG;
  if (K % 64 || lda % 8 || ldb % 8 || ldh % 8 || ip % 8 || (uintptr_t)A % 16 || (uintptr_t)B % 16 || (uintptr_t)h % 16 || (uintptr_t)dh % 16)
    return MCA_E_ALIGN;
  if (lda < K || ldb < K || ldh < 2 * ip) return MCA_E_BADARG;
  if (M > (1LL << 30)) return MCA_E_UNSUPPORTED;
  const int64_t N = ip;
  const int tiles_n = (int)((N + BN - 1) / BN);
  const float* hres = reinterpret_cast<const float*>(h);
  void* C = dh;
  if (M >= 40960 && g_knob[1] != 1) {
    const int nwg2 = (int)((M + BM2 - 1) / BM2) * tiles_n;
    static bool attr_dev[64] = {false}; bool& attr = *mca_dev_flag(attr_dev);
    if (!attr) {
      if (hipFuncSetAttribute(reinterpret_cast<const void*>(gemm_nt_256_kernel<true, 0, 0, 1>), hipFuncAttributeMaxDynamicSharedMemorySize,
                              NT256_LDS_BYTES) != hipSuccess ||
          hipFuncSetAttribute(reinterpret_cast<const void*>(gemm_nt_persist_kernel<3, false>), hipFuncAttributeMaxDynamicSharedMemorySize,
                              NTPS_LDS_BYTES) != hipSuccess)
        return MCA_E_LAUNCH;
      attr = true;
    }
    if (g_knob[7] != 1 && N % BN == 0 && K >= 320) {
      const int grid = nwg2 < num_cus() ? nwg2 : num_cus();
      hipLaunchKernelGGL((gemm_nt_persist_kernel<3, false>), dim3(grid), dim3(512), NTPS_LDS_BYTES, as_stream(stream), A, lda, B, ldb, C, ldh,
                         nullptr, hres, ldh, (int)M, (int)N, (int)K, tiles_n, nwg2, g_knob[0]);
// ... 677 lines not shown
```

### mca-paper_amd/engine.py

```python
from __future__ import annotations

import os

import ctypes as C
import math
from typing import Callable, Dict, List, Optional

import numpy as np
import torch

from . import hip
from .encoders import EmbeddedSequenceEncoder, TabularEncoder
from .hip import AttnBwd1Args, AttnBwd2Args, AttnFp8BwdOperands, AttnFp8Operands, AttnFwdArgs, LossTerm, call, ptr, stream_ptr

LN_EPS = 1e-5
FWD_BQ, FWD_BK = 128, 64
BWD_BQ = 64


def _pad_to(x: int, m: int) -> int:
    return (x + m - 1) // m * m


def _dev(a: np.ndarray, device) -> torch.Tensor:
    return torch.from_numpy(np.ascontiguousarray(a)).to(device)


def debug_options() -> dict:
    opts = {"overlap_wgrad": None, "group_wgrad": True, "mask_mfma": True, "dkv_keys": 128, "lazy_softmax": True,
            "onepass": None}
    for item in filter(None, os.environ.get("MCA_DEBUG", "").split(",")):
        k, _, v = item.partition("=")
        k = k.strip()
        if k not in opts:
            raise ValueError(f"MCA_DEBUG: unknown switch '{k}' (known: {sorted(opts)})")
        opts[k] = int(v) if k == "dkv_keys" else (v.strip() not in ("0", "", "false"))
    return opts


class _Sched:

    def __init__(self, s, device):
        self.s = s
        pack = lambda idx, full: (idx.astype(np.uint32) | (full.astype(np.uint32) << 31)).view(np.int32)
        self.q_ptr, self.q_kt, self.q_order = _dev(s.q_ptr, device), _dev(pack(s.q_kt, s.q_full), device), _dev(s.q_order, device)
        self.k_ptr, self.k_qt, self.k_order = _dev(s.k_ptr, device), _dev(pack(s.k_qt, s.k_full), device), _dev(s.k_order, device)
        wg = np.zeros((len(s.k_order), 4), np.int32)
        for i, kb in enumerate(s.k_order):
            lo, hi = int(s.k_ptr[kb]), int(s.k_ptr[kb + 1])
            wg[i] = (kb, lo, hi - lo, int(s.k_qt[lo]) if hi > lo else 0)
        self.k_wg = _dev(wg, device)


class _OnePassSched:

    def __init__(self, s, device):
        self.s = s
        self.qt_desc, self.kb_desc = _dev(s.qt_desc.astype(np.int32), device), _dev(s.kb_desc.astype(np.int32), device)
        self.kb_qt = _dev(s.kb_qt.astype(np.uint32).view(np.int32), device)
        self.visit, self.row_slot = _dev(s.visit.astype(np.uint8), device), _dev(s.row_slot.astype(np.int32), device)
        self.n_qt, self.n_kb, self.max_list = len(s.qt_desc), len(s.kb_desc), int(s.kb_desc[:, 3].max())
        self.n_entries = int(len(s.kb_qt))
        self.fits = self.n_qt < 256 and self.n_kb <= 64 and self.max_list + 6 <= 256 and self.n_entries + 4 * self.n_kb <= 768


class FusionEngine:
    def __init__(self, model):
        self.model = model
        p0 = next(model.parameters())
        self.eao = model.attn_pool is None
        if p0.device.type != "cuda":
            raise hip.MCAHipError("the MCA step runs only on a HIP device: move the model to cuda first "
                                  "(there is no CPU fallback)")
        hip.lib()
        self.device = p0.device
        self.D, self.H, self.L = model.dim, model.heads, model.depth
        st = model.structure
        self.st = st
        self.N, self.R, self.F, self.M = st.n_tokens, st.n_return, st.num_fusion_tokens, st.n_modalities
        if self.D != self.H * 64:
            raise NotImplementedError("native path needs dim == heads * 64")
        self.I = model.layers[0].ff.inner_dim if self.L else int(self.D * 4 * 2 / 3)
        self.Ip = _pad_to(self.I, 64)
# ... 181 lines not shown
        if not force and v == self._weights_version:
            return
        if getattr(self, "_cast_table", None) is not None:
            call("mca_cast_pad_bf16_multi", ptr(self._cast_table), self._cast_n, stream_ptr())
            self._weights_version = v
            return
        self._cast_list = []
        m, D, I, Ip = self.model, self.D, self.I, self.Ip
        for i, ly in enumerate(m.layers):
            w = self.wl[i]
            self._cast(ly.attn.to_q.weight.data, w["qkv"], scale=self.q_scale)
            self._cast(ly.attn.to_kv.weight.data, w["qkv"], dst_row0=D)
            self._cast(ly.attn.to_q.weight.data, w["qkvT"], transpose=True)
            self._cast(ly.attn.to_kv.weight.data, w["qkvT"], transpose=True, dst_col0=D)
            self._cast(ly.attn.to_out.weight.data, w["o"])
            self._cast(ly.attn.to_out.weight.data, w["oT"], transpose=True)
            w1 = ly.ff.feedforward[0].weight.data
            self._cast(w1[:I], w["w1"])
            self._cast(w1[I:], w["w1"], dst_row0=Ip)
            self._cast(w1[:I], w["w1T"], transpose=True)
            self._cast(w1[I:], w["w1T"], transpose=True, dst_col0=Ip)
            w2 = ly.ff.feedforward[2].weight.data
            self._cast(w2, w["w2"])
            self._cast(w2, w["w2T"], transpose=True)
        ap = m.attn_pool
        if ap is not None:
            self._cast(ap.to_q.weight.data, self.wp["q"], scale=self.q_scale); self._cast(ap.to_q.weight.data, self.wp["qT"], transpose=True)
            self._cast(ap.to_kv.weight.data, self.wp["kv"]); self._cast(ap.to_kv.weight.data, self.wp["kvT"], transpose=True)
            self._cast(ap.to_out.weight.data, self.wp["o"]); self._cast(ap.to_out.weight.data, self.wp["oT"], transpose=True)
        for name in m.modality_types:
            enc = m.encoders[name]
            if isinstance(enc, EmbeddedSequenceEncoder):
                self._cast(enc.token_encoder[1].weight.data, self.we[name]["w"])
                self._cast(enc.token_encoder[1].weight.data, self.we[name]["wT"], transpose=True)
            elif isinstance(enc, TabularEncoder):
                self._cast(enc.value_encoder.linear2.weight.data, self.we[name]["w2"])
                self._cast(enc.value_encoder.linear2.weight.data, self.we[name]["w2T"], transpose=True)
        arr = (hip.CastDesc * len(self._cast_list))(*self._cast_list)
        self._cast_n = len(self._cast_list)
        self._cast_table = torch.frombuffer(bytearray(bytes(arr)), dtype=torch.uint8).to(self.device)
        call("mca_cast_pad_bf16_multi", ptr(self._cast_table), self._cast_n, stream_ptr())
        self._weights_version = v

    def workspace(self, b: int) -> dict:
        if b in self._ws:
            return self._ws[b]
        D, N, H, Ip, R, dev = self.D, self.N, self.H, self.Ip, self.R, self.device
        T = b * N
        f32 = lambda *s: torch.empty(*s, dtype=torch.float32, device=dev)
        bf = lambda *s: torch.empty(*s, dtype=torch.bfloat16, device=dev)
        u8 = lambda *s: torch.empty(*s, dtype=torch.uint8, device=dev)
        ws = dict(b=b, T=T, gen=0)
        ws["x"] = [f32(T, D) for _ in range(self.L + 1)]
        ws["layers"] = [dict(x1=f32(T, D), m1=f32(T), r1=f32(T), m2=f32(T), r2=f32(T), xn_b=bf(T, D), qkv=bf(T, 3 * D),
                             o=bf(T, D), lse=f32(b, H, N), x1n_b=bf(T, D), h=bf(T, 2 * Ip), g=bf(T, Ip),
                             dxo_b=bf(T, D), dx1_b=bf(T, D), dh=bf(T, 2 * Ip), dqkv=bf(T, 3 * D))
                        for _ in range(self.L)]
        ws["xn"], ws["x1n"] = f32(T, D), f32(T, D)
        ws["mf"], ws["rf"] = f32(T), f32(T)
        ws["t_b"], ws["kvp"] = (None, None) if self.eao else (bf(T, D), bf(T, 2 * D))
        ws["rt_b"], ws["qp"], ws["op"], ws["lse_p"] = bf(R, D), bf(R, D), bf(b * R, D), f32(b, H, R)
        ws["pooled"] = f32(b * R, D)
        if self.eao:
            ws["seg_counts"] = torch.zeros(b, R, dtype=torch.int32, device=dev)
        ws["vmean"], ws["dvmean"], ws["delta"], ws["delta_p"] = torch.zeros(b, D, dtype=torch.float32, device=dev), f32(b, D), f32(b, H, N), f32(b, H, R)
        ws["keyinfo"], ws["kflags"] = u8(b, self.nk_pad), u8(b, (N + 63) // 64)
        ws["khot"] = bf(b, self.nk_pad, 16) if self.mask_mfma else None
        ws["padding"] = u8(b, N)
        ws["present"] = torch.zeros(b, dtype=torch.int32, device=dev)
        ws["present_native"] = torch.zeros(b, dtype=torch.int32, device=dev)
        ws["dxa"], ws["dxb"], ws["dx_b"] = f32(T, D), f32(T, D), bf(T, D)
        ws["dg"], ws["do"] = bf(T, Ip), bf(T, D)
        ws["dpool_b"], ws["dop"], ws["dqp32"], ws["dqp_sum"], ws["dqp_b"] = bf(b * R, D), bf(b * R, D), f32(b * R, D), f32(R, D), bf(R, D)
        ws["dkvp"], ws["drt"] = (None if self.eao else bf(T, 2 * D)), f32(R, D)
        ws["enc"] = {}
        for mi, name in enumerate(self.model.modality_types):
            enc = self.model.encoders[name]
            n = self.st.token_dims[mi]
            rows = b * n
            if isinstance(enc, EmbeddedSequenceEncoder):
                kp = self.we[name]["kp"]
                ws["enc"][name] = dict(xin_b=bf(rows, kp), m0=f32(rows), r0=f32(rows), y=f32(rows, D), m2=f32(rows), r2=f32(rows),
                                       dy=f32(rows, D), dy_b=bf(rows, D), dxin=f32(rows, kp), mask=u8(rows))
            elif isinstance(enc, TabularEncoder):
                ws["enc"][name] = dict(h1_b=bf(rows, D), y=f32(rows, D), m2=f32(rows), r2=f32(rows), dy=f32(rows, D),
                                       dy_b=bf(rows, D), dh1=f32(rows, D), mask=u8(rows))
        ws["side"], ws["side_events"] = torch.cuda.Stream(device=dev), []
        self._ws[b] = ws
        return ws

    @staticmethod
    def gemm_nt(A, B, C, M, N, K, bias=None, residual=None, res_period=0):
        if hip.PROFILE is not None:
            hip.set_tag(f"{M}x{N}x{K}{'' if C.dtype == torch.bfloat16 else ' f32'}{' +res' if residual is not None else ''}")
        call("mca_gemm_nt", ptr(A), A.stride(0), ptr(B), B.stride(0), ptr(C), C.stride(0), int(C.dtype == torch.bfloat16),
             ptr(bias), ptr(residual), residual.stride(0) if residual is not None else 0, res_period, M, N, K, stream_ptr(),
             flops=2.0 * M * N * K)
        if hip.PROFILE is not None:
            hip.set_tag("")

    @staticmethod
    def gemm_tn_acc(A, B, Cgrad, R, N, K):
        call("mca_gemm_tn_acc", ptr(A), A.stride(0), ptr(B), B.stride(0), ptr(Cgrad), Cgrad.stride(0), R, N, K, stream_ptr(),
             flops=2.0 * R * N * K)

    @staticmethod
    def gemm_tn_acc_group(members, R):
        arr = (hip.TnDesc * len(members))()
        fl = 0.0
        for d, (A, B, Cg, N, K) in zip(arr, members):
            d.A, d.lda, d.B, d.ldb, d.C, d.ldc, d.N, d.K = ptr(A), A.stride(0), ptr(B), B.stride(0), ptr(Cg), Cg.stride(0), N, K
            fl += 2.0 * R * N * K
        call("mca_gemm_tn_acc_group", C.byref(arr), len(members), R, stream_ptr(), flops=fl)

    @staticmethod
    def ln_fwd(x, gamma, rows, cols, mean, rstd, beta=None, rowmask=None, add=None, period=0, y=None, ldy=0, y_bstride=0,
               y_bf16=None, cols_pad=0):
        call("mca_layernorm_fwd", ptr(x), x.stride(0), ptr(gamma), ptr(beta), ptr(rowmask), ptr(add), period,
             ptr(y), ldy, y_bstride, ptr(y_bf16), y_bf16.stride(0) if y_bf16 is not None else 0, cols_pad,
             ptr(mean), ptr(rstd), rows, cols, LN_EPS, stream_ptr())

    @staticmethod
    def ln_bwd(dy, ldy, x, gamma, mean, rstd, rows, cols, dgamma, dbeta=None, rowmask=None, dx=None, dx_bf16=None,
               y_bstride=0, period=0, dxsum=None):
        call("mca_layernorm_bwd", ptr(dy), ldy, y_bstride, period, ptr(x), x.stride(0), ptr(gamma), ptr(mean), ptr(rstd),
             ptr(rowmask), ptr(dx), dx.stride(0) if dx is not None else 0, ptr(dx_bf16),
             dx_bf16.stride(0) if dx_bf16 is not None else 0, ptr(dgamma), ptr(dbeta), ptr(dxsum), rows, cols, stream_ptr())

    def _attn_fwd(self, q, q_bstride, q_ld, kv, k_off, v_off, kv_ld, o, lse, qmask, sched, ws, b, nq, layer=0):
        N = self.N
        a = AttnFwdArgs()
        esz = 2
        a.q, a.q_bstride, a.q_ld = q, q_bstride, q_ld
        a.k, a.v = kv.data_ptr() + k_off * esz, kv.data_ptr() + v_off * esz
        a.kv_bstride, a.kv_ld = N * kv_ld, kv_ld
        a.o, a.o_bstride, a.o_ld = o.data_ptr(), nq * o.stride(0), o.stride(0)
        a.lse = lse.data_ptr()
        a.qmask, a.keyinfo, a.ktile_flags = qmask.data_ptr(), ws["keyinfo"].data_ptr(), ws["kflags"].data_ptr()
        a.q_ptr, a.q_kt, a.q_order = sched.q_ptr.data_ptr(), sched.q_kt.data_ptr(), sched.q_order.data_ptr()
        a.vmean = ws["vmean"].data_ptr()
        a.batch, a.heads, a.nq, a.nk, a.nk_pad = b, self.H, nq, N, self.nk_pad
        a.n_qtiles, a.n_ktiles, a.scale, a.flags = sched.s.n_q, sched.s.n_k, self.scale, self.attn_flags
        a.khot = ws["khot"].data_ptr() if ws.get("khot") is not None else None
        if ws.get("present_cur") is not None:
            call("mca_attn_vmean_if_needed", a.v, a.kv_bstride, a.kv_ld, ws["vmean"].data_ptr(), b, N, self.H, ptr(ws["present_cur"]),
                 (1 << self.M) - 1, stream_ptr())
        else:
            call("mca_attn_vmean", a.v, a.kv_bstride, a.kv_ld, ws["vmean"].data_ptr(), b, N, self.H, stream_ptr())
        hip.set_tag("pool" if nq != N else "layer")
        if self.attn_dtype == "fp8" and nq == N:
            f = self._fp8_operands(ws, b, layer)[1]
            ws[("fp8gen", layer)] = ws["gen"]
            call("mca_attn_quant_mxfp8", a.q, a.q_bstride, a.q_ld, a.k, a.v, a.kv_bstride, a.kv_ld, C.byref(f), b, self.H, N, stream_ptr())
            call("mca_attn_fwd_fp8", C.byref(a), C.byref(f), stream_ptr(), flops=4.0 * 64 * sched.s.allowed_pairs * self.H * b)
        else:
            call("mca_attn_fwd", C.byref(a), stream_ptr(), flops=4.0 * 64 * sched.s.allowed_pairs * self.H * b)
        hip.set_tag("")

    def _attn_bwd2(self, q, q_bstride, q_ld, kv, k_off, v_off, kv_ld, o, d_o, lse, delta, dq_ptr, dq_bstride, dq_ld, dq_f32, dkv,
                   dk_off, dv_off, dkv_ld, qmask, sched_f, sched_b, ws, b, nq, layer=0):
        N, esz = self.N, 2
        if self.use_onepass(ws, b, nq, dq_f32):
            return self._attn_bwd1(q, q_bstride, q_ld, kv, k_off, v_off, kv_ld, o, d_o, lse, dq_ptr, dq_bstride, dq_ld, dkv, dk_off, dv_off,
                                   dkv_ld, ws, b)
        call("mca_attn_bwd_prep", o.data_ptr(), d_o.data_ptr(), nq * o.stride(0), o.stride(0), lse.data_ptr(),
             delta.data_ptr(), ws["dvmean"].data_ptr(), b, self.H, nq, N, stream_ptr())
        a = AttnBwd2Args()
        a.q, a.q_bstride, a.q_ld = q, q_bstride, q_ld
        a.k, a.v = kv.data_ptr() + k_off * esz, kv.data_ptr() + v_off * esz
        a.kv_bstride, a.kv_ld = N * kv_ld, kv_ld
        a.d_o, a.o_bstride, a.o_ld = d_o.data_ptr(), nq * d_o.stride(0), d_o.stride(0)
        a.lse, a.delta, a.dvmean = lse.data_ptr(), delta.data_ptr(), ws["dvmean"].data_ptr()
        a.dq, a.dq_bstride, a.dq_ld, a.dq_f32 = dq_ptr, dq_bstride, dq_ld, int(dq_f32)
        a.dk, a.dv = dkv.data_ptr() + dk_off * esz, dkv.data_ptr() + dv_off * esz
        a.dkv_bstride, a.dkv_ld = N * dkv_ld, dkv_ld
        a.qmask, a.keyinfo, a.ktile_flags = qmask.data_ptr(), ws["keyinfo"].data_ptr(), ws["kflags"].data_ptr()
        a.q_ptr, a.q_kt, a.q_order = sched_f.q_ptr.data_ptr(), sched_f.q_kt.data_ptr(), sched_f.q_order.data_ptr()
        a.n_qtiles128, a.n_ktiles64 = sched_f.s.n_q, sched_f.s.n_k
        a.k_wg, a.k_qt, a.n_qtiles64, a.n_kblocks256 = sched_b.k_wg.data_ptr(), sched_b.k_qt.data_ptr(), sched_b.s.n_q, sched_b.s.n_k
        a.batch, a.heads, a.nq, a.nk, a.nk_pad, a.scale, a.flags = b, self.H, nq, N, self.nk_pad, self.scale, self.attn_flags
        if ws.get("khot") is not None:
            a.khot, a.qblk = ws["khot"].data_ptr(), (self.qblk_attn if qmask is self.qmask_attn else self.qblk_pool).data_ptr()
        a.kblock_keys = sched_b.s.bk
        pairs = sched_b.s.allowed_pairs
        hip.set_tag("pool" if nq != N else "layer")
        if self.fp8_backward_on(ws, nq):
            f, which = self._fp8_bwd_operands(ws, b, layer)
            call("mca_attn_quant_bwd_mxfp8", a.q, a.q_bstride, a.q_ld, a.k, a.v, a.kv_bstride, a.kv_ld, a.d_o, a.o_bstride, a.o_ld,
                 C.byref(f), which, b, self.H, N, stream_ptr())
            call("mca_attn_bwd_dkv_fp8", C.byref(a), C.byref(f), stream_ptr(), flops=8.0 * 64 * pairs * self.H * b * 0.6)
            call("mca_attn_bwd_dq_fp8", C.byref(a), C.byref(f), stream_ptr(), flops=8.0 * 64 * pairs * self.H * b * 0.4)
        else:
            call("mca_attn_bwd_dkv", C.byref(a), stream_ptr(), flops=8.0 * 64 * pairs * self.H * b * 0.6)
            call("mca_attn_bwd_dq", C.byref(a), stream_ptr(), flops=8.0 * 64 * pairs * self.H * b * 0.4)
        hip.set_tag("")

    ONEPASS_MIN_WG = 192

    def use_onepass(self, ws, b, nq, dq_f32=False) -> bool:
        if self.sched_onepass is None or nq != self.N or dq_f32 or ws.get("khot") is None:
            return False
        want = self.dbg["onepass"]
        return bool(want) if want is not None else b * self.H * self.onepass_split(b) >= self.ONEPASS_MIN_WG

    def onepass_split(self, b) -> int:
        wg = b * self.H
        return 1 if wg >= self.ONEPASS_MIN_WG else max(1, min(4, self.sched_onepass.n_kb if self.sched_onepass else 1, -(-256 // wg)))

    def backward_form(self, b) -> str:
        ws = {"khot": True if self.mask_mfma else None}
        if self.use_onepass(ws, b, self.N):
            return "bf16 one-pass" + (f" (key blocks split {self.onepass_split(b)} ways)" if self.onepass_split(b) > 1 else "")
        return "fp8 two-pass" if (self.attn_dtype == "fp8" and self.mask_mfma and self.dkv_keys == 128) else "bf16 two-pass"

    def _attn_bwd1(self, q, q_bstride, q_ld, kv, k_off, v_off, kv_ld, o, d_o, lse, dq_ptr, dq_bstride, dq_ld, dkv, dk_off, dv_off, dkv_ld, ws, b):
        N, esz, sc = self.N, 2, self.sched_onepass
        if "rowc" not in ws:
            rc = torch.empty(b, self.H, sc.n_qt + 1, 2, 64, dtype=torch.float32, device=self.device)
            rc[:, :, :, 0] = float("-inf"); rc[:, :, :, 1] = 0.0
            ws["rowc"] = rc
            ws["dq_acc"] = torch.empty(b * self.H * self.onepass_split(b) * (sc.n_qt + 1) * 4096, dtype=torch.float32, device=self.device)
            ws["q_hm"] = torch.zeros((b * self.H * N + 64) * 64, dtype=torch.bfloat16, device=self.device)
            ws["do_hm"] = torch.zeros((b * self.H * N + 64) * 64, dtype=torch.bfloat16, device=self.device)
        call("mca_attn_bwd_prep_onepass", o.data_ptr(), d_o.data_ptr(), N * o.stride(0), o.stride(0), lse.data_ptr(), sc.row_slot.data_ptr(),
             ws["rowc"].data_ptr(), ws["dvmean"].data_ptr(), b, self.H, N, sc.n_qt, q, q_bstride, q_ld, ws["q_hm"].data_ptr(),
             ws["do_hm"].data_ptr(), stream_ptr())
        a = AttnBwd1Args()
        a.q, a.q_bstride, a.q_hstride, a.q_ld = ws["q_hm"].data_ptr(), self.H * N * 64, N * 64, 64
        a.k, a.v = kv.data_ptr() + k_off * esz, kv.data_ptr() + v_off * esz
        a.kv_bstride, a.kv_ld = N * kv_ld, kv_ld
        a.d_o, a.o_bstride, a.o_hstride, a.o_ld = ws["do_hm"].data_ptr(), self.H * N * 64, N * 64, 64
        a.rowc, a.dvmean = ws["rowc"].data_ptr(), ws["dvmean"].data_ptr()
        a.dq, a.dq_bstride, a.dq_ld = dq_ptr, dq_bstride, dq_ld
        a.dk, a.dv = dkv.data_ptr() + dk_off * esz, dkv.data_ptr() + dv_off * esz
        a.dkv_bstride, a.dkv_ld = N * dkv_ld, dkv_ld
        a.dq_acc = ws["dq_acc"].data_ptr()
        a.keyinfo, a.ktile_flags, a.khot, a.qblk = ws["keyinfo"].data_ptr(), ws["kflags"].data_ptr(), ws["khot"].data_ptr(), self.qblk_attn.data_ptr()
        a.qt_desc, a.kb_desc, a.kb_qt, a.visit = sc.qt_desc.data_ptr(), sc.kb_desc.data_ptr(), sc.kb_qt.data_ptr(), sc.visit.data_ptr()
        a.n_qtiles, a.n_kblocks, a.max_list, a.n_entries = sc.n_qt, sc.n_kb, sc.max_list, sc.n_entries
        a.batch, a.heads, a.n, a.nk_pad, a.n_ktiles64 = b, self.H, N, self.nk_pad, (N + 63) // 64
        a.scale, a.flags, a.split = self.scale, self.attn_flags, self.onepass_split(b)
        hip.set_tag("layer")
        call("mca_attn_bwd_onepass", C.byref(a), stream_ptr(), flops=8.0 * 64 * sc.s.allowed_pairs * self.H * b)
        hip.set_tag("")

    def _encode(self, batch, ws, need_grad: bool, renorm: bool = True):
        m, D, N, b = self.model, self.D, self.N, ws["b"]
        x0 = ws["x"][0]
        ws["foreign"] = {}
        pk = hip.PackMasksArgs()
        keep = []
        native_idx = []
        for mi, name in enumerate(m.modality_types):
            enc = m.encoders[name]
            if not isinstance(enc, (EmbeddedSequenceEncoder, TabularEncoder)):
                continue
            n, off = self.st.token_dims[mi], self.offsets[mi]
            am = batch[name]["attention_mask"]
            if am.dtype == torch.bool or am.dtype == torch.uint8:
                eb = 1
            elif am.dtype == torch.int64:
                eb = 8
            else:
                am, eb = am.to(torch.bool), 1
            if not am.is_contiguous():
                am = am.contiguous()
            if am.shape != (b, n):
                raise AssertionError(f"{name}: attention_mask {tuple(am.shape)} != {(b, n)}")
            keep.append(am)
            d = pk.m[len(native_idx)]
            d.mask, d.elem_bytes, d.n, d.offset = am.data_ptr(), eb, n, off
            d.rowmask = ws["enc"][name]["mask"].data_ptr() if isinstance(enc, EmbeddedSequenceEncoder) else None
            native_idx.append(mi)
        foreign = len(native_idx) != len(m.modality_types)
        if native_idx:
            pk.n_mod, pk.batch, pk.n_tokens, pk.n_fusion = len(native_idx), b, N, (0 if foreign else self.F)
            call("mca_pack_masks", C.byref(pk), ptr(ws["padding"]), ptr(ws["present_native"]), stream_ptr())
        present = ws["present"]
        if not foreign:
            present = ws["present_native"]
        else:
            present.zero_()
            for k, mi in enumerate(native_idx):
                present |= ((ws["present_native"] >> k) & 1) << mi
# ... 22 lines not shown
                self._encode_tabular(name, enc, bm, ws, mi, renorm)
            else:
                with torch.enable_grad() if need_grad else torch.no_grad():
                    toks, amask = enc(bm)
                ws["foreign"][name] = toks
                x0.view(b, N, D)[:, off:off + n].copy_(toks.detach().float())
                ws["padding"].view(b, N)[:, off:off + n].copy_(amask.to(torch.bool))
                present |= ((amask == 0).sum(dim=1) != 0).to(torch.int32) << mi
        if self.F:
            call("mca_bcast_rows", ptr(m.fusion_tokens.data), D, x0.data_ptr() + (N - self.F) * D * 4, D, N * D, self.F,
                 b * self.F, D, stream_ptr())
            if foreign:
                ws["padding"].view(b, N)[:, N - self.F:] = 0
        if self.eao:
            pad2 = ws["padding"].view(b, N)
            for src, dst, n in self.st.copies:
                call("mca_rows_copy_add", x0.data_ptr() + src * D * 4, N * D, x0.data_ptr() + dst * D * 4, N * D, n, D, b, 0, stream_ptr())
                pad2[:, dst:dst + n].copy_(pad2[:, src:src + n])
        ws["present_cur"] = present
        bits = ((present[:, None] >> self._mod_shifts) & 1).to(torch.bool)
        return {name: bits[:, mi] for mi, name in enumerate(m.modality_types)}

    def _renorm_table(self, enc, n):
        emb = enc.token_encoder.embedding.weight
        call("mca_embedding_renorm", ptr(emb.data), n, self.D, float(enc.token_encoder.max_norm), stream_ptr())

    def _encode_tabular(self, name, enc, bm, ws, mi, renorm=True):
        D, N, b = self.D, self.N, ws["b"]
        n, off = self.st.token_dims[mi], self.offsets[mi]
        rows = b * n
        e, ve = ws["enc"][name], enc.value_encoder
        vals = bm["values"]
        if vals.dtype != torch.float32 or not vals.is_contiguous():
            vals = vals.float().contiguous()
        if vals.shape != (b, n):
            raise AssertionError(f"{vals.shape[1]} - {n}")
        e["values"] = vals
        emb = enc.token_encoder.embedding.weight
        if renorm:
            self._renorm_table(enc, n)
        call("mca_tab_value_fwd", ptr(vals), ptr(ve.linear1.weight.data), ptr(ve.linear1.bias.data), ptr(e["h1_b"]), ptr(e["mask"]),
             rows, D, float(ve.max_value), float(ve.padding_value), stream_ptr())
        self.gemm_nt(e["h1_b"], self.we[name]["w2"], e["y"], rows, D, D, bias=ve.linear2.bias)
        self.ln_fwd(e["y"], ve.norm.weight, rows, D, e["m2"], e["r2"], beta=ve.norm.bias, rowmask=e["mask"], add=emb.data,
                    period=n, y=ws["x"][0][off:], ldy=D, y_bstride=N * D)

    def forward_trunk(self, ws):
        m, D, N, H, Ip, R, b, T = self.model, self.D, self.N, self.H, self.Ip, self.R, ws["b"], ws["T"]
        call("mca_build_keyinfo", ptr(ws["padding"]), ptr(self.kgroup), ptr(ws["keyinfo"]), ptr(ws["kflags"]), b, N,
             self.nk_pad, stream_ptr())
        if ws["khot"] is not None:
            call("mca_build_keyhot", ptr(ws["keyinfo"]), ptr(ws["khot"]), b, self.nk_pad, stream_ptr())
        ln_in_gemm = self.fuse_ln_residual and T >= 2048 and D % 128 == 0 and D >= 512 and Ip >= 512
        for i, ly in enumerate(m.layers):
            w, a = self.wl[i], ws["layers"][i]
            xin, xout = ws["x"][i], ws["x"][i + 1]
            g = ly.norm.gamma
            self.ln_fwd(xin, g, T, D, a["m1"], a["r1"], y=None if ln_in_gemm else ws["xn"], ldy=D, y_bf16=a["xn_b"], cols_pad=D)
            self.gemm_nt(a["xn_b"], w["qkv"], a["qkv"], T, 3 * D, D)
            self._attn_fwd(a["qkv"].data_ptr(), N * 3 * D, 3 * D, a["qkv"], D, 2 * D, 3 * D, a["o"], a["lse"],
                           self.qmask_attn, self.sched_attn_f, ws, b, N, layer=i)
            if ln_in_gemm:
                call("mca_gemm_nt_lnres", ptr(a["o"]), D, ptr(w["o"]), D, ptr(a["x1"]), D, ptr(xin), D, ptr(a["m1"]), ptr(a["r1"]),
                     ptr(g.data), T, D, D, stream_ptr(), flops=2.0 * T * D * D)
            else:
                self.gemm_nt(a["o"], w["o"], a["x1"], T, D, D, residual=ws["xn"])
            self.ln_fwd(a["x1"], g, T, D, a["m2"], a["r2"], y=None if ln_in_gemm else ws["x1n"], ldy=D, y_bf16=a["x1n_b"], cols_pad=D)
            call("mca_gemm_nt_geglu_fwd", ptr(a["x1n_b"]), D, ptr(w["w1"]), D, ptr(a["h"]), 2 * Ip, ptr(a["g"]), Ip, Ip, T, D,
                 stream_ptr(), flops=2.0 * T * 2 * Ip * D)
            if ln_in_gemm:
                call("mca_gemm_nt_lnres", ptr(a["g"]), Ip, ptr(w["w2"]), Ip, ptr(xout), D, ptr(a["x1"]), D, ptr(a["m2"]), ptr(a["r2"]),
                     ptr(g.data), T, D, Ip, stream_ptr(), flops=2.0 * T * D * Ip)
            else:
                self.gemm_nt(a["g"], w["w2"], xout, T, D, Ip, residual=ws["x1n"])
        xl = ws["x"][self.L]
        if self.eao:
            self.ln_fwd(xl, m.norm.gamma, T, D, ws["mf"], ws["rf"], y=ws["xn"], ldy=D)
            call("mca_segment_mean_fwd", ptr(ws["xn"]), ptr(ws["padding"]), ptr(self.seg_start), R, ptr(ws["pooled"]),
                 ptr(ws["seg_counts"]), b, N, D, stream_ptr())
            return ws["pooled"]
        self.ln_fwd(xl, m.norm.gamma, T, D, ws["mf"], ws["rf"], y_bf16=ws["t_b"], cols_pad=D)
        self.gemm_nt(ws["t_b"], self.wp["kv"], ws["kvp"], T, 2 * D, D)
        call("mca_f32_to_bf16", ptr(m.return_tokens.data), D, ptr(ws["rt_b"]), D, R, D, 1.0, stream_ptr())
        self.gemm_nt(ws["rt_b"], self.wp["q"], ws["qp"], R, D, D)
        self._attn_fwd(ws["qp"].data_ptr(), 0, D, ws["kvp"], 0, D, 2 * D, ws["op"], ws["lse_p"], self.qmask_pool,
                       self.sched_pool_f, ws, b, R)
        self.gemm_nt(ws["op"], self.wp["o"], ws["pooled"], b * R, D, D, residual=m.return_tokens.data, res_period=R)
        return ws["pooled"]

    def loss_fwd_bwd(self, pooled_all, present_all, b_local, row0):
        B, R, D, T = pooled_all.shape[0], self.R, self.D, self.n_terms
        dev = self.device
        nbytes = hip.lib().mca_contrastive_workspace_bytes(B, T)
        key = ("lossws", B)
        if key not in self._ws:
            self._ws[key] = torch.empty(nbytes, dtype=torch.uint8, device=dev)
        out = dict(term_loss=torch.empty(T, dtype=torch.float32, device=dev), loss=torch.empty(1, dtype=torch.float32, device=dev),
                   d_pooled=torch.empty(b_local, R, D, dtype=torch.float32, device=dev),
                   d_logit=torch.empty(1, dtype=torch.float32, device=dev))
        ls = self.model.loss.loss_fn.logit_scale
        call("mca_contrastive_fwd_bwd", ptr(pooled_all), ptr(present_all), ptr(self.loss_terms_dev), T, ptr(ls.data), B, b_local,
             row0, R, D, ptr(out["term_loss"]), ptr(out["loss"]), ptr(out["d_pooled"]), ptr(out["d_logit"]),
             ptr(self._ws[key]), stream_ptr())
        return out

    def _on_side(self, fn, slot: int, ws: dict):
        if not self.overlap_on(ws):
            fn()
            return
        side, events = ws["side"], ws["side_events"]
        while len(events) <= slot:
            events.append(torch.cuda.Event())
        ev = events[slot]
        ev.record()
# ... 46 lines not shown
        call("mca_reduce_rows", ptr(ws["dqp32"]), D, R * D, R, ptr(ws["dqp_sum"]), D, b * R, D, stream_ptr())
        call("mca_f32_to_bf16", ptr(ws["dqp_sum"]), D, ptr(ws["dqp_b"]), D, R, D, 1.0, stream_ptr())
        self.gemm_nt(ws["dqp_b"], self.wp["qT"], ws["drt"], R, D, D)
        call("mca_reduce_rows", ptr(ws["drt"]), D, R * D, R, ptr(G(m.return_tokens)), D, R, D, stream_ptr())
        on_side(lambda: tn(ws["dqp_b"], ws["rt_b"], G(ap.to_q.weight), R, D, D))
        pool_kv = (ws["dkvp"], ws["t_b"], G(ap.to_kv.weight), 2 * D, D)
        if not (self.L > 0 and self.group_wgrad and T >= 4096):
            on_side(lambda pk=pool_kv: tn(pk[0], pk[1], pk[2], T, 2 * D, D))
            pool_kv = None
        dx, dx_other = ws["dxa"], ws["dxb"]
        self.gemm_nt(ws["dkvp"], self.wp["kvT"], dx, T, D, 2 * D)
        top = ws["layers"][self.L - 1]["dxo_b"] if self.L else ws["dx_b"]
        self.ln_bwd(dx, D, ws["x"][self.L], m.norm.gamma, ws["mf"], ws["rf"], T, D, G(m.norm.gamma), dx=dx_other, dx_bf16=top)
        dx, dx_other = dx_other, dx
        on_side(lambda: bucket_ready(0))
        self._backward_layers_and_encoders(ws, dx, dx_other, bucket_ready, on_side, extra_top=pool_kv)

    def _backward_part_eao(self, ws, dpool, bucket_ready, on_side):
        m, D, N, R, b, T = self.model, self.D, self.N, self.R, ws["b"], ws["T"]
        dx, dx_other = ws["dxa"], ws["dxb"]
        call("mca_segment_mean_bwd", ptr(dpool), ptr(ws["padding"]), ptr(self.kgroup), ptr(ws["seg_counts"]), R, ptr(dx), b, N, D,
             stream_ptr())
        top = ws["layers"][self.L - 1]["dxo_b"] if self.L else ws["dx_b"]
        self.ln_bwd(dx, D, ws["x"][self.L], m.norm.gamma, ws["mf"], ws["rf"], T, D, self.grad_of(m.norm.gamma), dx=dx_other, dx_bf16=top)
        dx, dx_other = dx_other, dx
        on_side(lambda: bucket_ready(0))
        self._backward_layers_and_encoders(ws, dx, dx_other, bucket_ready, on_side)

    def _backward_layers_and_encoders(self, ws, dx, dx_other, bucket_ready, on_side, extra_top=None):
        m, D, N, H, Ip, I, R, b, T = self.model, self.D, self.N, self.H, self.Ip, self.I, self.R, ws["b"], ws["T"]
        G = self.grad_of
        tn = self.gemm_tn_acc
        for bi, i in enumerate(reversed(range(self.L))):
            ly, w, a = m.layers[i], self.wl[i], ws["layers"][i]
            g = ly.norm.gamma
            dxo, dx1, dh, dqkv = a["dxo_b"], a["dx1_b"], a["dh"], a["dqkv"]
            below = ws["layers"][i - 1]["dxo_b"] if i > 0 else ws["dx_b"]
            grouped = self.group_wgrad and T >= 4096
            if not grouped:
                on_side(lambda dxo=dxo, a=a, ly=ly: tn(dxo, a["g"], G(ly.ff.feedforward[2].weight), T, D, I))
            if self.fuse_geglu_bwd:
                call("mca_gemm_nt_geglu_bwd", ptr(dxo), D, ptr(w["w2T"]), D, ptr(a["h"]), ptr(dh), 2 * Ip, Ip, T, D,
                     stream_ptr(), flops=2.0 * T * Ip * D)
            else:
                self.gemm_nt(dxo, w["w2T"], ws["dg"], T, Ip, D)
                call("mca_geglu_bwd", ptr(ws["dg"]), ptr(a["h"]), ptr(dh), T, Ip, stream_ptr())
            gw1 = G(ly.ff.feedforward[0].weight)
            if not grouped:
                on_side(lambda dh=dh, a=a, gw1=gw1: (tn(dh, a["x1n_b"], gw1, T, I, D), tn(dh[:, Ip:], a["x1n_b"], gw1[I:], T, I, D)))
            self.gemm_nt(dh, w["w1T"], dx_other, T, D, 2 * Ip, residual=dx)
            self.ln_bwd(dx_other, D, a["x1"], g, a["m2"], a["r2"], T, D, G(g), dx=dx, dx_bf16=dx1)
            if not grouped:
                on_side(lambda dx1=dx1, a=a, ly=ly: tn(dx1, a["o"], G(ly.attn.to_out.weight), T, D, D))
            self.gemm_nt(dx1, w["oT"], ws["do"], T, D, D)
            self._attn_bwd2(a["qkv"].data_ptr(), N * 3 * D, 3 * D, a["qkv"], D, 2 * D, 3 * D, a["o"], ws["do"], a["lse"],
                            ws["delta"], dqkv.data_ptr(), N * 3 * D, 3 * D, False, dqkv, D, 2 * D, 3 * D, self.qmask_attn,
                            self.sched_attn_f, self.sched_attn_b2, ws, b, N, layer=i)
            gq = G(ly.attn.to_q.weight)
            assert G(ly.attn.to_kv.weight).data_ptr() == gq.data_ptr() + D * D * 4
            if grouped:
                gw2, gwo = G(ly.ff.feedforward[2].weight), G(ly.attn.to_out.weight)
                extra = [extra_top] if (bi == 0 and extra_top is not None) else []
                on_side(lambda dqkv=dqkv, dh=dh, dxo=dxo, dx1=dx1, a=a, gq=gq, gw1=gw1, gw2=gw2, gwo=gwo, extra=extra: self.gemm_tn_acc_group(
                    [(dqkv, a["xn_b"], gq, 3 * D, D), (dh, a["x1n_b"], gw1, I, D), (dh[:, Ip:], a["x1n_b"], gw1[I:], I, D),
                     (dxo, a["g"], gw2, D, I), (dx1, a["o"], gwo, D, D)] + extra, T))
            else:
                on_side(lambda dqkv=dqkv, a=a, gq=gq: tn(dqkv, a["xn_b"], gq, T, 3 * D, D))
            self.gemm_nt(dqkv, w["qkvT"], dx_other, T, D, 3 * D, residual=dx)
            self.ln_bwd(dx_other, D, ws["x"][i], g, a["m1"], a["r1"], T, D, G(g), dx=dx, dx_bf16=below)
            on_side(lambda bi=bi: bucket_ready(bi + 1))
        if self.eao:
            for src, dst, n in self.st.copies:
                call("mca_rows_copy_add", dx.data_ptr() + dst * D * 4, N * D, dx.data_ptr() + src * D * 4, N * D, n, D, b, 1, stream_ptr())
        if self.F:
            call("mca_reduce_rows", dx.data_ptr() + (N - self.F) * D * 4, D, N * D, self.F, ptr(G(m.fusion_tokens)), D,
                 b * self.F, D, stream_ptr())
        for mi, name in enumerate(m.modality_types):
            enc = m.encoders[name]
            n, off = self.st.token_dims[mi], self.offsets[mi]
            rows = b * n
            if isinstance(enc, EmbeddedSequenceEncoder):
                e, te = ws["enc"][name], enc.token_encoder
                kp = self.we[name]["kp"]
                self.ln_bwd(dx[off:], D, e["y"], te[2].weight, e["m2"], e["r2"], rows, D, G(te[2].weight), dbeta=G(te[2].bias),
                            rowmask=e["mask"], dx=e["dy"], dx_bf16=e["dy_b"], y_bstride=N * D, period=n, dxsum=G(te[1].bias))
                on_side(lambda e=e, te=te, rows=rows, enc=enc: tn(e["dy_b"], e["xin_b"], G(te[1].weight), rows, D, enc.input_size))
                self.gemm_nt(e["dy_b"], self.we[name]["wT"], e["dxin"], rows, kp, D)
                t2 = e["tokens"].view(rows, enc.input_size)
                self.ln_bwd(e["dxin"], kp, t2, te[0].weight, e["m0"], e["r0"], rows, enc.input_size, G(te[0].weight),
                            dbeta=G(te[0].bias), rowmask=e["mask"])
            elif isinstance(enc, TabularEncoder):
                self._backward_tabular(name, enc, ws, mi, dx)
            else:
                toks = ws["foreign"][name]
                if toks.requires_grad:
                    for p in enc.parameters():
                        p.grad = G(p)
                    torch.autograd.backward(toks, dx.view(b, N, D)[:, off:off + n].to(toks.dtype))
        on_side(lambda: bucket_ready(len(self.bucket_bounds) - 1))

    def _backward_tabular(self, name, enc, ws, mi, dx):
        D, N, b = self.D, self.N, ws["b"]
        n, off = self.st.token_dims[mi], self.offsets[mi]
        rows = b * n
        e, ve, G = ws["enc"][name], enc.value_encoder, self.grad_of
        gemb = G(enc.token_encoder.embedding.weight)
        call("mca_reduce_rows", dx.data_ptr() + off * D * 4, D, N * D, n, ptr(gemb), D, rows, D, stream_ptr())
        gemb[n - 1].zero_()
        self.ln_bwd(dx[off:], D, e["y"], ve.norm.weight, e["m2"], e["r2"], rows, D, G(ve.norm.weight), dbeta=G(ve.norm.bias),
                    rowmask=e["mask"], dx=e["dy"], dx_bf16=e["dy_b"], y_bstride=N * D, period=n, dxsum=G(ve.linear2.bias))
# ... 156 lines not shown
```

### mca-paper_amd/hip.py

```python
from __future__ import annotations

import ctypes as C
import os
from typing import Optional

import torch

_HERE = os.path.dirname(os.path.abspath(__file__))
LIB_PATH = os.environ.get("MCA_HIP_LIB") or os.path.join(_HERE, "libmca_hip.so")

_ERR = {-1: "bad argument", -2: "misaligned pointer / leading dimension", -3: "unsupported size", -4: "launch failed"}


class MCAHipError(RuntimeError):
    pass


class LossTerm(C.Structure):
    _fields_ = [("slot_a", C.c_int32), ("slot_b", C.c_int32), ("and_bits", C.c_uint32), ("or_bits", C.c_uint32)]


class CastDesc(C.Structure):
    _fields_ = [("src", C.c_void_p), ("dst", C.c_void_p), ("lds", C.c_int64), ("rows", C.c_int64), ("cols", C.c_int64),
                ("ldd", C.c_int64), ("rows_pad", C.c_int64), ("cols_pad", C.c_int64), ("transpose", C.c_int32), ("scale", C.c_float)]


MAX_MODALITIES = 16


class TnDesc(C.Structure):
    _fields_ = [("A", C.c_void_p), ("lda", C.c_int64), ("B", C.c_void_p), ("ldb", C.c_int64), ("C", C.c_void_p), ("ldc", C.c_int64),
                ("N", C.c_int64), ("K", C.c_int64)]


class MaskDesc(C.Structure):
    _fields_ = [("mask", C.c_void_p), ("rowmask", C.c_void_p), ("elem_bytes", C.c_int32), ("n", C.c_int32), ("offset", C.c_int32),
                ("pad_", C.c_int32)]


class FiniteArgs(C.Structure):
    _fields_ = [("p", C.c_void_p * MAX_MODALITIES), ("n", C.c_int64 * MAX_MODALITIES), ("count", C.c_int32), ("pad_", C.c_int32)]


class PackMasksArgs(C.Structure):
    _fields_ = [("m", MaskDesc * MAX_MODALITIES), ("n_mod", C.c_int32), ("batch", C.c_int32), ("n_tokens", C.c_int32),
                ("n_fusion", C.c_int32)]


class AttnFwdArgs(C.Structure):
    _fields_ = [
        ("q", C.c_void_p), ("q_bstride", C.c_int64), ("q_ld", C.c_int64),
        ("k", C.c_void_p), ("v", C.c_void_p), ("kv_bstride", C.c_int64), ("kv_ld", C.c_int64),
        ("o", C.c_void_p), ("o_bstride", C.c_int64), ("o_ld", C.c_int64),
        ("lse", C.c_void_p), ("qmask", C.c_void_p), ("keyinfo", C.c_void_p), ("ktile_flags", C.c_void_p),
        ("q_ptr", C.c_void_p), ("q_kt", C.c_void_p), ("q_order", C.c_void_p),
        ("vmean", C.c_void_p),
        ("batch", C.c_int), ("heads", C.c_int), ("nq", C.c_int), ("nk", C.c_int), ("nk_pad", C.c_int),
        ("n_qtiles", C.c_int), ("n_ktiles", C.c_int), ("scale", C.c_float), ("flags", C.c_int),
        ("khot", C.c_void_p),
    ]


ATTN_Q_PRESCALED = 1
ATTN_LAZY_REFERENCE = 2


class AttnFp8Operands(C.Structure):
    _fields_ = [("q8", C.c_void_p), ("qs", C.c_void_p), ("k8", C.c_void_p), ("ks", C.c_void_p), ("v8t", C.c_void_p), ("vs", C.c_void_p),
                ("n_ktiles", C.c_int)]


class AttnFp8BwdOperands(C.Structure):
    _fields_ = [("q8", C.c_void_p), ("qs", C.c_void_p), ("k8", C.c_void_p), ("ks", C.c_void_p), ("v8", C.c_void_p), ("vs", C.c_void_p),
                ("do8", C.c_void_p), ("dos", C.c_void_p), ("n_ktiles", C.c_int)]


class AttnBwd2Args(C.Structure):
    _fields_ = [
        ("q", C.c_void_p), ("q_bstride", C.c_int64), ("q_ld", C.c_int64),
        ("k", C.c_void_p), ("v", C.c_void_p), ("kv_bstride", C.c_int64), ("kv_ld", C.c_int64),
        ("d_o", C.c_void_p), ("o_bstride", C.c_int64), ("o_ld", C.c_int64),
        ("lse", C.c_void_p), ("delta", C.c_void_p), ("dvmean", C.c_void_p),
        ("dq", C.c_void_p), ("dq_bstride", C.c_int64), ("dq_ld", C.c_int64), ("dq_f32", C.c_int),
        ("dk", C.c_void_p), ("dv", C.c_void_p), ("dkv_bstride", C.c_int64), ("dkv_ld", C.c_int64),
        ("qmask", C.c_void_p), ("keyinfo", C.c_void_p), ("ktile_flags", C.c_void_p),
        ("q_ptr", C.c_void_p), ("q_kt", C.c_void_p), ("q_order", C.c_void_p), ("n_qtiles128", C.c_int), ("n_ktiles64", C.c_int),
        ("k_wg", C.c_void_p), ("k_qt", C.c_void_p), ("n_qtiles64", C.c_int), ("n_kblocks256", C.c_int),
        ("batch", C.c_int), ("heads", C.c_int), ("nq", C.c_int), ("nk", C.c_int), ("nk_pad", C.c_int),
        ("scale", C.c_float), ("flags", C.c_int),
        ("khot", C.c_void_p), ("qblk", C.c_void_p), ("kblock_keys", C.c_int),
    ]


class AttnBwd1Args(C.Structure):
    _fields_ = [
        ("q", C.c_void_p), ("q_bstride", C.c_int64), ("q_ld", C.c_int64),
        ("k", C.c_void_p), ("v", C.c_void_p), ("kv_bstride", C.c_int64), ("kv_ld", C.c_int64),
        ("d_o", C.c_void_p), ("o_bstride", C.c_int64), ("o_ld", C.c_int64),
        ("q_hstride", C.c_int64), ("o_hstride", C.c_int64),
        ("rowc", C.c_void_p), ("dvmean", C.c_void_p),
        ("dq", C.c_void_p), ("dq_bstride", C.c_int64), ("dq_ld", C.c_int64),
        ("dk", C.c_void_p), ("dv", C.c_void_p), ("dkv_bstride", C.c_int64), ("dkv_ld", C.c_int64),
        ("dq_acc", C.c_void_p),
        ("keyinfo", C.c_void_p), ("ktile_flags", C.c_void_p), ("khot", C.c_void_p), ("qblk", C.c_void_p),
        ("qt_desc", C.c_void_p), ("kb_desc", C.c_void_p), ("kb_qt", C.c_void_p), ("visit", C.c_void_p),
        ("n_qtiles", C.c_int), ("n_kblocks", C.c_int), ("max_list", C.c_int), ("n_entries", C.c_int),
        ("batch", C.c_int), ("heads", C.c_int), ("n", C.c_int), ("nk_pad", C.c_int), ("n_ktiles64", C.c_int),
        ("scale", C.c_float), ("flags", C.c_int), ("split", C.c_int),
    ]


_P, _I64, _I, _F = C.c_void_p, C.c_int64, C.c_int, C.c_float

SIGNATURES = {
    "mca_version": (C.c_char_p, []),
    "mca_flag_to_host": (_I, [_P, _P, _P]),
    "mca_build_keyhot": (_I, [_P, _P, _I, _I, _P]),
    "mca_rows_copy_add": (_I, [_P, _I64, _P, _I64, _I64, _I, _I, _I, _P]),
    "mca_segment_mean_fwd": (_I, [_P, _P, _P, _I, _P, _P, _I, _I, _I, _P]),
    "mca_segment_mean_bwd": (_I, [_P, _P, _P, _P, _I, _P, _I, _I, _I, _P]),
    "mca_gemm_nt": (_I, [_P, _I64, _P, _I64, _P, _I64, _I, _P, _P, _I64, _I64, _I64, _I64, _I64, _P]),
    "mca_gemm_nt_geglu_bwd": (_I, [_P, _I64, _P, _I64, _P, _P, _I64, _I64, _I64, _I64, _P]),
    "mca_gemm_nt_lnres": (_I, [_P, _I64, _P, _I64, _P, _I64, _P, _I64, _P, _P, _P, _I64, _I64, _I64, _P]),
    "mca_gemm_nt_geglu_fwd": (_I, [_P, _I64, _P, _I64, _P, _I64, _P, _I64, _I64, _I64, _I64, _P]),
    "mca_gemm_tn_acc": (_I, [_P, _I64, _P, _I64, _P, _I64, _I64, _I64, _I64, _P]),
    "mca_gemm_tn_acc_group": (_I, [_P, _I, _I64, _P]),
    "mca_layernorm_fwd": (_I, [_P, _I64, _P, _P, _P, _P, _I64, _P, _I64, _I64, _P, _I64, _I, _P, _P, _I64, _I, _F, _P]),
    "mca_layernorm_bwd": (_I, [_P, _I64, _I64, _I64, _P, _I64, _P, _P, _P, _P, _P, _I64, _P, _I64, _P, _P, _P, _I64, _I, _P]),
    "mca_geglu_fwd": (_I, [_P, _P, _I64, _I, _P]),
    "mca_geglu_bwd": (_I, [_P, _P, _P, _I64, _I, _P]),
    "mca_cast_pad_bf16": (_I, [_P, _I64, _I64, _I64, _P, _I64, _I64, _I64, _I, _P]),
    "mca_cast_pad_bf16_multi": (_I, [_P, _I, _P]),
    "mca_f32_to_bf16": (_I, [_P, _I64, _P, _I64, _I64, _I64, _F, _P]),
    "mca_bcast_rows": (_I, [_P, _I64, _P, _I64, _I64, _I64, _I64, _I, _P]),
    "mca_reduce_rows": (_I, [_P, _I64, _I64, _I64, _P, _I64, _I64, _I, _P]),
    "mca_embedding_renorm": (_I, [_P, _I64, _I, _F, _P]),
    "mca_tab_value_fwd": (_I, [_P, _P, _P, _P, _P, _I64, _I, _F, _F, _P]),
    "mca_tab_value_bwd": (_I, [_P, _I64, _P, _P, _P, _P, _I64, _I, _F, _P]),
    "mca_pack_masks": (_I, [_P, _P, _P, _P]),
    "mca_build_keyinfo": (_I, [_P, _P, _P, _P, _I, _I, _I, _P]),
    "mca_attn_vmean": (_I, [_P, _I64, _I64, _P, _I, _I, _I, _P]),
    "mca_attn_vmean_if_needed": (_I, [_P, _I64, _I64, _P, _I, _I, _I, _P, _I, _P]),
    "mca_attn_fwd": (_I, [C.POINTER(AttnFwdArgs), _P]),
    "mca_attn_quant_mxfp8": (_I, [_P, _I64, _I64, _P, _P, _I64, _I64, C.POINTER(AttnFp8Operands), _I, _I, _I, _P]),
    "mca_attn_fwd_fp8": (_I, [C.POINTER(AttnFwdArgs), C.POINTER(AttnFp8Operands), _P]),
    "mca_attn_bwd_prep": (_I, [_P, _P, _I64, _I64, _P, _P, _P, _I, _I, _I, _I, _P]),
    "mca_attn_bwd_onepass": (_I, [C.POINTER(AttnBwd1Args), _P]),
    "mca_attn_bwd_prep_onepass": (_I, [_P, _P, _I64, _I64, _P, _P, _P, _P, _I, _I, _I, _I, _P, _I64, _I64, _P, _P, _P]),
    "mca_attn_bwd_dq": (_I, [C.POINTER(AttnBwd2Args), _P]),
    "mca_attn_bwd_dkv": (_I, [C.POINTER(AttnBwd2Args), _P]),
    "mca_attn_quant_bwd_mxfp8": (_I, [_P, _I64, _I64, _P, _P, _I64, _I64, _P, _I64, _I64, C.POINTER(AttnFp8BwdOperands), _I, _I, _I, _I, _P]),
    "mca_attn_bwd_dq_fp8": (_I, [C.POINTER(AttnBwd2Args), C.POINTER(AttnFp8BwdOperands), _P]),
    "mca_attn_bwd_dkv_fp8": (_I, [C.POINTER(AttnBwd2Args), C.POINTER(AttnFp8BwdOperands), _P]),
    "mca_contrastive_workspace_bytes": (_I64, [_I, _I]),
    "mca_contrastive_fwd_bwd": (_I, [_P, _P, _P, _I, _P, _I, _I, _I, _I, _I, _P, _P, _P, _P, _P, _P]),
    "mca_grad_sqnorm": (_I, [_P, _I64, _P, _P]),
    "mca_adamw_step": (_I, [_P, _P, _P, _P, _I64, _F, _F, _F, _F, _F, _F, _F, _F, _P, _P, _P, _P]),
    "mca_adamw_hyper": (_I, [_P, _F, _F, _F, _P]),
    "mca_nonfinite_flag": (_I, [C.POINTER(FiniteArgs), _P, _I, _P]),
    "mca_rows_normalize_f32": (_I, [_P, _I64, _P, _I64, _I64, _I64, _P]),
    "mca_cosine_rank_f32": (_I, [_P, _I64, _P, _I64, _P, _I64, _I64, _I64, _P, _P, _P]),
    "mca_pair_gauss_workspace": (_I64, [_I64]),
    "mca_pair_gauss_sum_f32": (_I, [_P, _I64, _I64, _I64, _F, _P, _I64, _P, _P, _P]),
    "mca_probe_nt_f32": (_I, [_P, _I64, _P, _P, _I64, _P, _P, _I64, _I64, _I64, _I64, _I, _F, C.c_uint64, _I64, _P]),
    "mca_probe_head_blocks": (_I64, [_I64]),
    "mca_probe_head_f32": (_I, [_P, _I64, _P, _I64, _P, _P, _I64, _P, _P, _I64, _I, _P, _P, _P, _F, _P, _P]),
    "mca_probe_tn_workspace": (_I64, [_I64, _I64, _I64]),
    "mca_probe_tn_f32": (_I, [_P, _I64, _P, _I64, _P, _I64, _I64, _I64, _P, _I64, _P, _P, _P]),
    "mca_probe_loss_accum": (_I, [_P, _I64, _I64, _P, _P]),
}
DEBUG_SIGNATURES = {
    "mca_debug_set": (_I, [_I, _I]),
    "mca_debug_reset": (_I, []),
}

_lib: Optional[C.CDLL] = None


def lib() -> C.CDLL:
    global _lib
    if _lib is None:
        if not os.path.exists(LIB_PATH):
            raise MCAHipError(
                f"{LIB_PATH} not found: the HIP extension is not built (run `python __graft_entry__.py build`). "
                "There is no CPU or eager fallback for the MCA step.")
        l = C.CDLL(LIB_PATH)
        for name, (res, args) in list(SIGNATURES.items()) + list(DEBUG_SIGNATURES.items()):
            fn = getattr(l, name)
            fn.restype = res
            fn.argtypes = args
        _lib = l
    return _lib


_STREAM_CACHE = None


def stream_ptr() -> int:
    if _STREAM_CACHE is not None:
        return _STREAM_CACHE
    return torch.cuda.current_stream().cuda_stream
# ... 37 lines not shown
        return self

    def __exit__(self, *exc):
        lib().mca_debug_reset()


def ptr(t: Optional[torch.Tensor]) -> Optional[int]:
    if t is None:
        return None
    return t.data_ptr()


def check(rc: int, what: str):
    if rc != 0:
        raise MCAHipError(f"{what} failed: {_ERR.get(rc, rc)}")


PROFILE = None
_PROFILE_ON = True
_TAG = ""


def profile_enable(flag: bool):
    global _PROFILE_ON
    _PROFILE_ON = bool(flag)


def set_tag(tag: str):
    global _TAG
    _TAG = tag


def profile_start(names):
    global PROFILE
    PROFILE = {"names": set(names), "records": {}}


def profile_collect():
    torch.cuda.synchronize()
    tot = PROFILE.setdefault("totals", {})
    for key, recs in PROFILE["records"].items():
        n, ms, fl = tot.get(key, (0, 0.0, 0.0))
        tot[key] = (n + len(recs), ms + sum(s.elapsed_time(e) for s, e, _ in recs), fl + sum(f for _, _, f in recs))
    PROFILE["records"] = {}


def profile_stop():
    global PROFILE
    profile_collect()
    prof, PROFILE = PROFILE, None
    return prof["totals"]


def call(name: str, *args, flops: float = 0.0):
    if PROFILE is not None and _PROFILE_ON and name in PROFILE["names"]:
        s, e = torch.cuda.Event(enable_timing=True), torch.cuda.Event(enable_timing=True)
        s.record()
        check(getattr(lib(), name)(*args), name)
        e.record()
        PROFILE["records"].setdefault(name + ("/" + _TAG if _TAG else ""), []).append((s, e, flops))
        return
    check(getattr(lib(), name)(*args), name)
```

Measured before the change: 1719 samples/s.

## Write QKV and dO head-major from GEMM epilogue to skip attention repacking

Adds a GEMM variant that writes its output in head-major layout (per batch, per head, seq x 64). The forward QKV projection and the backward dO projection use it, so the attention kernels read Q/K/V and dO with head strides. The goal is to drop the separate transpose or repack into head-major buffers (q_hm/do_hm) that the one-pass backward prep used to do, and to give the attention kernels contiguous per-head loads. Attention fwd, bwd, vmean and rowc kernels gain head-stride parameters. If the heads GEMM refuses the shape, the code falls back to the old layout.

```diff
diff --git a/include/mca_hip.h b/include/mca_hip.h
--- a/include/mca_hip.h
+++ b/include/mca_hip.h
@@ -20,6 +20,9 @@
                 void* C, int64_t ldc, int out_bf16,
                 const float* bias, const float* residual, int64_t ldres, int64_t res_period,
                 int64_t M, int64_t N, int64_t K, mca_stream_t stream);
+
+int mca_gemm_nt_heads(const uint16_t* A, int64_t lda, const uint16_t* B, int64_t ldb, uint16_t* C,
+                      int64_t M, int64_t N, int64_t K, int64_t seq, int64_t heads, mca_stream_t stream);
 
 int mca_gemm_nt_lnres(const uint16_t* A, int64_t lda, const uint16_t* B, int64_t ldb, float* C, int64_t ldc,
                       const float* x, int64_t ldx, const float* mean, const float* rstd, const float* gamma,
@@ -95,6 +98,8 @@
                    int batch, int nk, int heads, mca_stream_t stream);
 int mca_attn_vmean_if_needed(const uint16_t* V, int64_t kv_bstride, int64_t kv_ld, float* vmean, int batch, int nk,
                              int heads, const int32_t* present, int32_t full_bits, mca_stream_t stream);
+int mca_attn_vmean_heads(const uint16_t* V, int64_t kv_bstride, int64_t kv_hstride, int64_t kv_ld, float* vmean, int batch, int nk,
+                         int heads, const int32_t* present, int32_t full_bits, mca_stream_t stream);
 
 typedef struct {
   const uint16_t* q; int64_t q_bstride; int64_t q_ld;
@@ -110,6 +115,7 @@
   float scale;
   int flags;
   const uint16_t* khot;
+  int64_t q_hstride, kv_hstride;
 } mca_attn_fwd_args;
 #define MCA_ATTN_Q_PRESCALED 1
 #define MCA_ATTN_LAZY_REFERENCE 2
@@ -174,12 +180,16 @@
   float scale;
   int flags;
   int split;
+  int64_t kv_hstride;
 } mca_attn_bwd1_args;
 int mca_attn_bwd_onepass(const mca_attn_bwd1_args* args, mca_stream_t stream);
 int mca_attn_bwd_prep_onepass(const uint16_t* o, const uint16_t* d_o, int64_t o_bstride, int64_t o_ld, const float* lse,
                               const int32_t* row_slot, float* rowc, float* dvmean, int batch, int heads, int n, int n_qtiles,
                               const uint16_t* q, int64_t q_bstride, int64_t q_ld, uint16_t* q_hm, uint16_t* do_hm,
                               mca_stream_t stream);
+int mca_attn_bwd_rowc_onepass(const uint16_t* o, int64_t o_bstride, int64_t o_ld, const uint16_t* d_o, int64_t do_bstride,
+                              int64_t do_hstride, int64_t do_ld, const float* lse, const int32_t* row_slot, float* rowc,
+                              float* dvmean, int batch, int heads, int n, int n_qtiles, mca_stream_t stream);
 
 typedef struct { int32_t slot_a, slot_b; uint32_t and_bits, or_bits; } mca_loss_term;
 int64_t mca_contrastive_workspace_bytes(int B, int T);
diff --git a/mca-paper_amd/csrc/attention_bwd1.hip b/mca-paper_amd/csrc/attention_bwd1.hip
--- a/mca-paper_amd/csrc/attention_bwd1.hip
+++ b/mca-paper_amd/csrc/attention_bwd1.hip
@@ -40,8 +40,8 @@
 
   const u16* qbase = a.q + (int64_t)b * a.q_bstride + h * (a.q_hstride ? a.q_hstride : (int64_t)DH);
   const u16* obase = a.d_o + (int64_t)b * a.o_bstride + h * (a.o_hstride ? a.o_hstride : (int64_t)DH);
-  const u16* kbase = a.k + (int64_t)b * a.kv_bstride + h * DH;
-  const u16* vbase = a.v + (int64_t)b * a.kv_bstride + h * DH;
+  const u16* kbase = a.k + (int64_t)b * a.kv_bstride + h * (a.kv_hstride ? a.kv_hstride : (int64_t)DH);
+  const u16* vbase = a.v + (int64_t)b * a.kv_bstride + h * (a.kv_hstride ? a.kv_hstride : (int64_t)DH);
   const float* rowc_g = a.rowc + bh * (int64_t)(a.n_qtiles + 1) * 128;
   float* acc_g = a.dq_acc + bh * (int64_t)(a.n_qtiles + 1) * (TQ * DH);
   const uint8_t* kinfo_g = a.keyinfo + (int64_t)b * a.nk_pad;
@@ -428,8 +428,8 @@
 
   const u16* qbase = a.q + (int64_t)b * a.q_bstride + h * (a.q_hstride ? a.q_hstride : (int64_t)DH);
   const u16* obase = a.d_o + (int64_t)b * a.o_bstride + h * (a.o_hstride ? a.o_hstride : (int64_t)DH);
-  const u16* kbase = a.k + (int64_t)b * a.kv_bstride + h * DH;
-  const u16* vbase = a.v + (int64_t)b * a.kv_bstride + h * DH;
+  const u16* kbase = a.k + (int64_t)b * a.kv_bstride + h * (a.kv_hstride ? a.kv_hstride : (int64_t)DH);
+  const u16* vbase = a.v + (int64_t)b * a.kv_bstride + h * (a.kv_hstride ? a.kv_hstride : (int64_t)DH);
   const float* rowc_g = a.rowc + bh * (int64_t)(a.n_qtiles + 1) * 128;
   float* acc_s = a.dq_acc + (bh * S + sid) * (int64_t)(a.n_qtiles + 1) * (TQ * DH) + wave * 1024;
   const uint8_t* kinfo_g = a.keyinfo + (int64_t)b * a.nk_pad;
@@ -939,7 +939,7 @@
   if (a->batch <= 0 || a->heads <= 0 || a->n <= 0 || a->n_qtiles <= 0 || a->n_kblocks <= 0) return MCA_E_BADARG;
   if (a->n_qtiles >= B1_MAX_QT || a->n_kblocks > B1_MAX_KB || a->max_list + 6 > B1_MAX_LIST ||
       a->n_entries + 4 * a->n_kblocks > B1_MAX_META) return MCA_E_UNSUPPORTED;
-  if (a->q_ld % 8 || a->kv_ld % 8 || a->o_ld % 8 || a->q_bstride % 8 || a->kv_bstride % 8 || a->o_bstride % 8 || a->q_hstride % 8 || a->o_hstride % 8) return MCA_E_ALIGN;
+  if (a->q_ld % 8 || a->kv_ld % 8 || a->o_ld % 8 || a->q_bstride % 8 || a->kv_bstride % 8 || a->o_bstride % 8 || a->q_hstride % 8 || a->o_hstride % 8 || a->kv_hstride % 8) return MCA_E_ALIGN;
   if ((uintptr_t)a->q % 16 || (uintptr_t)a->k % 16 || (uintptr_t)a->v % 16 || (uintptr_t)a->d_o % 16 || (uintptr_t)a->khot % 16 || (uintptr_t)a->qblk % 16) return MCA_E_ALIGN;
   if (a->dq_ld % 8 || a->dq_bstride % 8 || (uintptr_t)a->dq % 16 || a->dkv_ld % 8 || a->dkv_bstride % 8 || (uintptr_t)a->dk % 16 || (uintptr_t)a->dv % 16) return MCA_E_ALIGN;
   if ((uintptr_t)a->dq_acc % 16 || (uintptr_t)a->rowc % 4 || (uintptr_t)a->kb_desc % 16 || (uintptr_t)a->qt_desc % 8) return MCA_E_ALIGN;
diff --git a/mca-paper_amd/csrc/attention_bwd2.hip b/mca-paper_amd/csrc/attention_bwd2.hip
--- a/mca-paper_amd/csrc/attention_bwd2.hip
+++ b/mca-paper_amd/csrc/attention_bwd2.hip
@@ -574,7 +574,8 @@
                                                     const float* __restrict__ lse, const int32_t* __restrict__ row_slot,
                                                     float* __restrict__ rowc, int n_qtiles,
                                                     const u16* __restrict__ qsrc, int64_t q_bstride, int64_t q_ld,
-                                                    u16* __restrict__ q_hm, u16* __restrict__ do_hm) {
+                                                    u16* __restrict__ q_hm, u16* __restrict__ do_hm,
+                                                    int64_t do_bstride, int64_t do_hstride, int64_t do_ld) {
   __shared__ float del_s[8][PREP_ROWS];
   const int b = by, tid = threadIdx.x, lane = tid & 63, wave = tid >> 6;
   const int cols = heads * DH;
@@ -585,12 +586,13 @@
     const int c = c0 + lane * 8;
     const int hl = lane >> 3;
     bf16x8 ovs[PREP_ROWS / 4], dvs[PREP_ROWS / 4], qvs[PREP_ROWS / 4];
+    const int64_t dcc = c < cols ? (int64_t)(h0 + hl) * do_hstride + (lane & 7) * 8 : 0;
 #pragma unroll
     for (int k = 0; k < PREP_ROWS / 4; k++) {
       int q = q_begin + wave + 4 * k; if (q > nq - 1) q = nq - 1;
       const int cc = c < cols ? c : 0;
       ovs[k] = *reinterpret_cast<const bf16x8*>(o + (int64_t)b * bstride + (int64_t)q * ld + cc);
-      dvs[k] = *reinterpret_cast<const bf16x8*>(d_o + (int64_t)b * bstride + (int64_t)q * ld + cc);
+      dvs[k] = *reinterpret_cast<const bf16x8*>(d_o + (int64_t)b * do_bstride + (int64_t)q * do_ld + dcc);
       if (do_hm) qvs[k] = *reinterpret_cast<const bf16x8*>(qsrc + (int64_t)b * q_bstride + (int64_t)q * q_ld + cc);
     }
 #pragma unroll
@@ -628,8 +630,8 @@
 }
 
 #define DVM_MAX_LIST 4096
-__device__ __forceinline__ void attn_dvmean_block(const int bx, const int by, const u16* __restrict__ d_o, int64_t bstride, int64_t ld,
-                                                  const float* __restrict__ lse, float* __restrict__ dvmean,
+__device__ __forceinline__ void attn_dvmean_block(const int bx, const int by, const u16* __restrict__ d_o, int64_t bstride, int64_t hstride,
+                                                  int64_t ld, const float* __restrict__ lse, float* __restrict__ dvmean,
                                                   int heads, int nq, float inv_nk) {
   __shared__ int list_s[DVM_MAX_LIST];
   __shared__ int n_s;
@@ -648,7 +650,7 @@
   auto flush = [&]() {
     const int n = n_s;
     for (int i = rg; i < n; i += 32) {
-      const bf16x8 v = *reinterpret_cast<const bf16x8*>(d_o + (int64_t)b * bstride + (int64_t)list_s[i] * ld + h * DH + cl * 8);
+      const bf16x8 v = *reinterpret_cast<const bf16x8*>(d_o + (int64_t)b * bstride + (int64_t)list_s[i] * ld + h * hstride + cl * 8);
 #pragma unroll
       for (int j = 0; j < 8; j++) acc[j] += bf2f((u16)v[j]);
     }
@@ -685,10 +687,11 @@
                                                              float* __restrict__ dvmean, int heads, int nq, float inv_nk, int n_prep,
                                                              const int32_t* __restrict__ row_slot, float* __restrict__ rowc, int n_qtiles,
                                                              const u16* __restrict__ qsrc, int64_t q_bstride, int64_t q_ld,
-                                                             u16* __restrict__ q_hm, u16* __restrict__ do_hm) {
+                                                             u16* __restrict__ q_hm, u16* __restrict__ do_hm,
+                                                             int64_t do_bstride, int64_t do_hstride, int64_t do_ld) {
   if ((int)blockIdx.x < n_prep) attn_bwd_prep_block((int)blockIdx.x, (int)blockIdx.y, o, d_o, bstride, ld, delta, heads, nq, lse, row_slot, rowc, n_qtiles,
-                                                    qsrc, q_bstride, q_ld, q_hm, do_hm);
-  else attn_dvmean_block((int)blockIdx.x - n_prep, (int)blockIdx.y, d_o, bstride, ld, lse, dvmean, heads, nq, inv_nk);
+                                                    qsrc, q_bstride, q_ld, q_hm, do_hm, do_bstride, do_hstride, do_ld);
+  else attn_dvmean_block((int)blockIdx.x - n_prep, (int)blockIdx.y, d_o, do_bstride, do_hstride, do_ld, lse, dvmean, heads, nq, inv_nk);
 }
 extern "C" int mca_attn_bwd_prep(const uint16_t* o, const uint16_t* d_o, int64_t o_bstride, int64_t o_ld,
                                  const float* lse, float* delta, float* dvmean, int batch, int heads, int nq, int nk,
@@ -699,7 +702,7 @@
   const int n_prep = (nq + PREP_ROWS - 1) / PREP_ROWS;
   hipLaunchKernelGGL(attn_bwd_prep_kernel, dim3(n_prep + heads, batch), dim3(256), 0, as_stream(stream), o, d_o, o_bstride, o_ld, lse, delta,
                      dvmean, heads, nq, 1.f / (float)nk, n_prep, (const int32_t*)nullptr, (float*)nullptr, 0, (const u16*)nullptr, (int64_t)0, (int64_t)0,
-                     (u16*)nullptr, (u16*)nullptr);
+                     (u16*)nullptr, (u16*)nullptr, o_bstride, (int64_t)DH, o_ld);
   return launch_status();
 }
 extern "C" int mca_attn_bwd_prep_onepass(const uint16_t* o, const uint16_t* d_o, int64_t o_bstride, int64_t o_ld, const float* lse,
@@ -713,6 +716,19 @@
   if (heads > 65535 || batch > 65535) return MCA_E_UNSUPPORTED;
   const int n_prep = (n + PREP_ROWS - 1) / PREP_ROWS;
   hipLaunchKernelGGL(attn_bwd_prep_kernel, dim3(n_prep + heads, batch), dim3(256), 0, as_stream(stream), o, d_o, o_bstride, o_ld, lse, (float*)nullptr,
-                     dvmean, heads, n, 1.f / (float)n, n_prep, row_slot, rowc, n_qtiles, q, q_bstride, q_ld, q_hm, do_hm);
+                     dvmean, heads, n, 1.f / (float)n, n_prep, row_slot, rowc, n_qtiles, q, q_bstride, q_ld, q_hm, do_hm,
+                     o_bstride, (int64_t)DH, o_ld);
   return launch_status();
 }
+extern "C" int mca_attn_bwd_rowc_onepass(const uint16_t* o, int64_t o_bstride, int64_t o_ld, const uint16_t* d_o, int64_t do_bstride,
+                                         int64_t do_hstride, int64_t do_ld, const float* lse, const int32_t* row_slot, float* rowc,
+                                         float* dvmean, int batch, int heads, int n, int n_qtiles, mca_stream_t stream) {
+  if (!o || !d_o || !lse || !row_slot || !rowc || !dvmean || batch <= 0 || heads <= 0 || n <= 0 || n_qtiles <= 0 || do_hstride < 0) return MCA_E_BADARG;
+  if (o_ld % 8 || o_bstride % 8 || do_ld % 8 || do_bstride % 8 || do_hstride % 8 || (uintptr_t)o % 16 || (uintptr_t)d_o % 16) return MCA_E_ALIGN;
+  if (heads > 65535 || batch > 65535) return MCA_E_UNSUPPORTED;
+  const int n_prep = (n + PREP_ROWS - 1) / PREP_ROWS;
+  hipLaunchKernelGGL(attn_bwd_prep_kernel, dim3(n_prep + heads, batch), dim3(256), 0, as_stream(stream), o, d_o, o_bstride, o_ld, lse, (float*)nullptr,
+                     dvmean, heads, n, 1.f / (float)n, n_prep, row_slot, rowc, n_qtiles, (const u16*)nullptr, (int64_t)0, (int64_t)0,
+                     (u16*)nullptr, (u16*)nullptr, do_bstride, do_hstride ? do_hstride : (int64_t)DH, do_ld);
+  return launch_status();
+}
diff --git a/mca-paper_amd/csrc/attention_fwd.hip b/mca-paper_amd/csrc/attention_fwd.hip
--- a/mca-paper_amd/csrc/attention_fwd.hip
+++ b/mca-paper_amd/csrc/attention_fwd.hip
@@ -40,7 +40,7 @@
 
   bf16x8 qf[4];
   {
-    const u16* qp = a.q + (int64_t)b * a.q_bstride + (int64_t)qrow * a.q_ld + h * DH + 8 * lh;
+    const u16* qp = a.q + (int64_t)b * a.q_bstride + (int64_t)qrow * a.q_ld + h * (a.q_hstride ? a.q_hstride : (int64_t)DH) + 8 * lh;
 #pragma unroll
     for (int s = 0; s < 4; s++) qf[s] = *reinterpret_cast<const bf16x8*>(qp + 16 * s);
   }
@@ -61,8 +61,8 @@
     for (int r = 0; r < 16; r++) o[n][r] = 0.f;
   float m_run = -INFINITY, l_run = 0.f;
 
-  const u16* kbase = a.k + (int64_t)b * a.kv_bstride + h * DH;
-  const u16* vbase = a.v + (int64_t)b * a.kv_bstride + h * DH;
+  const u16* kbase = a.k + (int64_t)b * a.kv_bstride + h * (a.kv_hstride ? a.kv_hstride : (int64_t)DH);
+  const u16* vbase = a.v + (int64_t)b * a.kv_bstride + h * (a.kv_hstride ? a.kv_hstride : (int64_t)DH);
   const uint8_t* kinfo_g = a.keyinfo + (int64_t)b * a.nk_pad;
   const u16* khot_g = use_hot ? a.khot + (int64_t)b * a.nk_pad * 16 : nullptr;
   {
@@ -284,7 +284,7 @@
 
   bf16x8 qf[4];
   {
-    const u16* qp = a.q + (int64_t)b * a.q_bstride + (int64_t)qrow * a.q_ld + h * DH + 8 * lh;
+    const u16* qp = a.q + (int64_t)b * a.q_bstride + (int64_t)qrow * a.q_ld + h * (a.q_hstride ? a.q_hstride : (int64_t)DH) + 8 * lh;
 #pragma unroll
     for (int s = 0; s < 4; s++) qf[s] = *reinterpret_cast<const bf16x8*>(qp + 16 * s);
   }
@@ -298,8 +298,8 @@
     for (int r = 0; r < 16; r++) o[n][r] = 0.f;
   float m_run = -INFINITY, l_run = 0.f;
 
-  const u16* kbase = a.k + (int64_t)b * a.kv_bstride + h * DH;
-  const u16* vbase = a.v + (int64_t)b * a.kv_bstride + h * DH;
+  const u16* kbase = a.k + (int64_t)b * a.kv_bstride + h * (a.kv_hstride ? a.kv_hstride : (int64_t)DH);
+  const u16* vbase = a.v + (int64_t)b * a.kv_bstride + h * (a.kv_hstride ? a.kv_hstride : (int64_t)DH);
   const u16* khot_g = a.khot + (int64_t)b * a.nk_pad * 16;
   {
     const uint8_t* flags_g = a.ktile_flags + (int64_t)b * a.n_ktiles;
@@ -481,7 +481,7 @@
 
   bf16x8 qf[4];
   {
-    const u16* qp = a.q + (int64_t)b * a.q_bstride + (int64_t)qrow * a.q_ld + h * DH + 8 * lh;
+    const u16* qp = a.q + (int64_t)b * a.q_bstride + (int64_t)qrow * a.q_ld + h * (a.q_hstride ? a.q_hstride : (int64_t)DH) + 8 * lh;
 #pragma unroll
     for (int s = 0; s < 4; s++) qf[s] = *reinterpret_cast<const bf16x8*>(qp + 16 * s);
   }
@@ -498,8 +498,8 @@
   for (int r = 0; r < 16; r++) negm[r] = 0.f;
   float l_run = 0.f;
 
-  const u16* kbase = a.k + (int64_t)b * a.kv_bstride + h * DH;
-  const u16* vbase = a.v + (int64_t)b * a.kv_bstride + h * DH;
+  const u16* kbase = a.k + (int64_t)b * a.kv_bstride + h * (a.kv_hstride ? a.kv_hstride : (int64_t)DH);
+  const u16* vbase = a.v + (int64_t)b * a.kv_bstride + h * (a.kv_hstride ? a.kv_hstride : (int64_t)DH);
   const u16* khot_g = a.khot + (int64_t)b * a.nk_pad * 16;
   {
     const uint8_t* flags_g = a.ktile_flags + (int64_t)b * a.n_ktiles;
@@ -677,6 +677,7 @@
   if ((uintptr_t)a->q % 16 || (uintptr_t)a->k % 16 || (uintptr_t)a->v % 16 || (uintptr_t)a->o % 8 ||
       (uintptr_t)a->keyinfo % 4)
     return MCA_E_ALIGN;
+  if (a->q_hstride < 0 || a->kv_hstride < 0 || a->q_hstride % 8 || a->kv_hstride % 8) return MCA_E_ALIGN;
   if (a->heads > 65535 || a->batch > 65535 || a->n_ktiles > MAX_KTILES) return MCA_E_UNSUPPORTED;
   const dim3 grid(a->n_qtiles, a->heads, a->batch);
   if (!(a->flags & MCA_ATTN_Q_PRESCALED)) return MCA_E_UNSUPPORTED;
@@ -739,12 +740,12 @@
 
 __global__ __launch_bounds__(512) void vmean_kernel(const u16* __restrict__ V, int64_t bstride, int64_t ld,
                                                      float* __restrict__ vmean, int nk, int cols,
-                                                     const int32_t* __restrict__ present, int32_t full_bits) {
+                                                     const int32_t* __restrict__ present, int32_t full_bits, int64_t hstride) {
   __shared__ float red[64][65];
   const int b = blockIdx.y, c0 = blockIdx.x * 64;
   if (present && present[b] == full_bits) return;
   const int cl = threadIdx.x & 7, rg = threadIdx.x >> 3;
-  const u16* base = V + (int64_t)b * bstride + c0 + cl * 8;
+  const u16* base = V + (int64_t)b * bstride + (int64_t)blockIdx.x * hstride + cl * 8;
   float acc[8] = {0, 0, 0, 0, 0, 0, 0, 0};
   for (int j = rg; j < nk; j += 64) {
     const bf16x8 v = *reinterpret_cast<const bf16x8*>(base + (int64_t)j * ld);
@@ -767,7 +768,7 @@
   if (kv_ld % 8 || kv_bstride % 8 || (uintptr_t)V % 16) return MCA_E_ALIGN;
   if (batch > 65535) return MCA_E_UNSUPPORTED;
   hipLaunchKernelGGL(vmean_kernel, dim3(heads, batch), dim3(512), 0, as_stream(stream), V, kv_bstride, kv_ld, vmean, nk, cols,
-                     (const int32_t*)nullptr, 0);
+                     (const int32_t*)nullptr, 0, (int64_t)DH);
   return launch_status();
 }
 extern "C" int mca_attn_vmean_if_needed(const uint16_t* V, int64_t kv_bstride, int64_t kv_ld, float* vmean, int batch, int nk,
@@ -777,6 +778,15 @@
   if (kv_ld % 8 || kv_bstride % 8 || (uintptr_t)V % 16) return MCA_E_ALIGN;
   if (batch > 65535) return MCA_E_UNSUPPORTED;
   hipLaunchKernelGGL(vmean_kernel, dim3(heads, batch), dim3(512), 0, as_stream(stream), V, kv_bstride, kv_ld, vmean, nk, cols,
-                     present, full_bits);
+                     present, full_bits, (int64_t)DH);
   return launch_status();
 }
+extern "C" int mca_attn_vmean_heads(const uint16_t* V, int64_t kv_bstride, int64_t kv_hstride, int64_t kv_ld, float* vmean, int batch,
+                                    int nk, int heads, const int32_t* present, int32_t full_bits, mca_stream_t stream) {
+  if (!V || !vmean || batch <= 0 || nk <= 0 || heads <= 0 || kv_hstride < 0) return MCA_E_BADARG;
+  if (kv_ld % 8 || kv_bstride % 8 || kv_hstride % 8 || (uintptr_t)V % 16) return MCA_E_ALIGN;
+  if (batch > 65535) return MCA_E_UNSUPPORTED;
+  hipLaunchKernelGGL(vmean_kernel, dim3(heads, batch), dim3(512), 0, as_stream(stream), V, kv_bstride, kv_ld, vmean, nk, heads * DH,
+                     present, full_bits, kv_hstride ? kv_hstride : (int64_t)DH);
+  return launch_status();
+}
diff --git a/mca-paper_amd/csrc/gemm.hip b/mca-paper_amd/csrc/gemm.hip
--- a/mca-paper_amd/csrc/gemm.hip
+++ b/mca-paper_amd/csrc/gemm.hip
@@ -680,7 +680,7 @@
 template <bool GEGLU>
 __global__ __launch_bounds__(512) void gemm_nt_persist256_kernel(
     const u16* __restrict__ A, int64_t lda, const u16* __restrict__ B, int64_t ldb, u16* __restrict__ C, int64_t ldc,
-    u16* __restrict__ G, int64_t ldg, int M, int N, int K, int tiles_n, int nwg, int dbg) {
+    u16* __restrict__ G, int64_t ldg, int M, int N, int K, int tiles_n, int nwg, int dbg, int seq = 0, int heads = 0) {
   extern __shared__ __attribute__((aligned(16))) u16 lds2[];
   constexpr int NST = GEGLU ? 24 : 16;
   const int tid = threadIdx.x, lane = tid & 63, wave = tid >> 6;
@@ -813,7 +813,12 @@
 #pragma unroll
       for (int u = 0; u < 8; u++) {
         const int m = mw + i * 32 + (lane >> 4) + 4 * u;
-        u16* cp = C + (int64_t)m * ldc + nw + 8 * (lane & 15);
+        u16* cp;
+        if (!GEGLU && seq > 0) {
+          const int c = nw + 8 * (lane & 15), hd = heads * 64, part = c / hd, h = (c - part * hd) >> 6;
+          const int smp = m / seq, n = m - smp * seq;
+          cp = C + ((((int64_t)part * (M / seq) + smp) * heads + h) * seq + n) * 64 + (c & 63);
+        } else cp = C + (int64_t)m * ldc + nw + 8 * (lane & 15);
         if (m < M) PS_GSTORE(cp, o[u]);
       }
       if (GEGLU) {
@@ -919,6 +924,28 @@
   if (pf) { NT_LAUNCH_256(false, 1, 1); return launch_status(); }
   if (out_bf16) { if (res == 0) NT_PICK_PF(true, 0); else if (res == 1) NT_PICK_PF(true, 1); else NT_PICK_PF(true, 2); }
   else { if (res == 0) NT_PICK_PF(false, 0); else if (res == 1) NT_PICK_PF(false, 1); else NT_PICK_PF(false, 2); }
+  return launch_status();
+}
+
+extern "C" int mca_gemm_nt_heads(const uint16_t* A, int64_t lda, const uint16_t* B, int64_t ldb, uint16_t* C, int64_t M, int64_t N,
+                                 int64_t K, int64_t seq, int64_t heads, mca_stream_t stream) {
+  if (!A || !B || !C || M <= 0 || N <= 0 || K <= 0 || seq <= 0 || heads <= 0) return MCA_E_BADARG;
+  if (K % 64 || lda % 8 || ldb % 8 || (uintptr_t)A % 16 || (uintptr_t)B % 16) return MCA_E_ALIGN;
+  if (lda < K || ldb < K) return MCA_E_BADARG;
+  if (M > (1LL << 30) || N > (1LL << 30)) return MCA_E_UNSUPPORTED;
+  if (M < 2048 || g_knob[1] == 1 || g_knob[7] != 0 || g_knob[10] == 1 || N % 256 || K < 192 || (uintptr_t)C % 16) return MCA_E_UNSUPPORTED;
+  if (M % seq || (heads * 64) % 256 || N % (heads * 64)) return MCA_E_UNSUPPORTED;
+  static bool attr_dev[64] = {false}; bool& attr = *mca_dev_flag(attr_dev);
+  if (!attr) {
+    if (hipFuncSetAttribute(reinterpret_cast<const void*>(gemm_nt_persist256_kernel<false>), hipFuncAttributeMaxDynamicSharedMemorySize,
+                            P2_LDS_BYTES) != hipSuccess)
+      return MCA_E_LAUNCH;
+    attr = true;
+  }
+  const int tn2 = (int)(N / 256), nw2 = (int)((M + 255) / 256) * tn2;
+  const int grid = nw2 < num_cus() ? nw2 : num_cus();
+  hipLaunchKernelGGL((gemm_nt_persist256_kernel<false>), dim3(grid), dim3(512), P2_LDS_BYTES, as_stream(stream), A, lda, B, ldb, C,
+                     (int64_t)0, (u16*)nullptr, (int64_t)0, (int)M, (int)N, (int)K, tn2, nw2, g_knob[0], (int)seq, (int)heads);
   return launch_status();
 }
 
diff --git a/mca-paper_amd/engine.py b/mca-paper_amd/engine.py
--- a/mca-paper_amd/engine.py
+++ b/mca-paper_amd/engine.py
@@ -28,7 +28,8 @@
 
 def debug_options() -> dict:
     opts = {"overlap_wgrad": None, "group_wgrad": True, "mask_mfma": True, "dkv_keys": 128, "lazy_softmax": True,
-            "onepass": None}
+            "onepass": None,
+            "headmajor": True}
     for item in filter(None, os.environ.get("MCA_DEBUG", "").split(",")):
         k, _, v = item.partition("=")
         k = k.strip()
@@ -316,7 +317,8 @@
         u8 = lambda *s: torch.empty(*s, dtype=torch.uint8, device=dev)
         ws = dict(b=b, T=T, gen=0)
         ws["x"] = [f32(T, D) for _ in range(self.L + 1)]
-        ws["layers"] = [dict(x1=f32(T, D), m1=f32(T), r1=f32(T), m2=f32(T), r2=f32(T), xn_b=bf(T, D), qkv=bf(T, 3 * D),
+        slack = lambda rows, cols: torch.zeros(rows * cols + 64 * 64, dtype=torch.bfloat16, device=dev)[:rows * cols].view(rows, cols)
+        ws["layers"] = [dict(x1=f32(T, D), m1=f32(T), r1=f32(T), m2=f32(T), r2=f32(T), xn_b=bf(T, D), qkv=slack(T, 3 * D),
                              o=bf(T, D), lse=f32(b, H, N), x1n_b=bf(T, D), h=bf(T, 2 * Ip), g=bf(T, Ip),
                              dxo_b=bf(T, D), dx1_b=bf(T, D), dh=bf(T, 2 * Ip), dqkv=bf(T, 3 * D))
                         for _ in range(self.L)]
@@ -334,7 +336,7 @@
         ws["present"] = torch.zeros(b, dtype=torch.int32, device=dev)
         ws["present_native"] = torch.zeros(b, dtype=torch.int32, device=dev)
         ws["dxa"], ws["dxb"], ws["dx_b"] = f32(T, D), f32(T, D), bf(T, D)
-        ws["dg"], ws["do"] = bf(T, Ip), bf(T, D)
+        ws["dg"], ws["do"] = bf(T, Ip), slack(T, D)
         ws["dpool_b"], ws["dop"], ws["dqp32"], ws["dqp_sum"], ws["dqp_b"] = bf(b * R, D), bf(b * R, D), f32(b * R, D), f32(R, D), bf(R, D)
         ws["dkvp"], ws["drt"] = (None if self.eao else bf(T, 2 * D)), f32(R, D)
         ws["enc"] = {}
@@ -364,6 +366,16 @@
             hip.set_tag("")
 
     @staticmethod
+    def gemm_nt_heads(A, B, C, M, N, K, seq, heads) -> bool:
+        if hip.PROFILE is not None:
+            hip.set_tag(f"{M}x{N}x{K}")
+        ok = call("mca_gemm_nt_heads", ptr(A), A.stride(0), ptr(B), B.stride(0), ptr(C), M, N, K, seq, heads, stream_ptr(),
+                  flops=2.0 * M * N * K, profile_as="mca_gemm_nt", may_refuse=True)
+        if hip.PROFILE is not None:
+            hip.set_tag("")
+        return ok
+
+    @staticmethod
     def gemm_tn_acc(A, B, Cgrad, R, N, K):
         call("mca_gemm_tn_acc", ptr(A), A.stride(0), ptr(B), B.stride(0), ptr(Cgrad), Cgrad.stride(0), R, N, K, stream_ptr(),
              flops=2.0 * R * N * K)
@@ -391,13 +403,15 @@
              ptr(rowmask), ptr(dx), dx.stride(0) if dx is not None else 0, ptr(dx_bf16),
              dx_bf16.stride(0) if dx_bf16 is not None else 0, ptr(dgamma), ptr(dbeta), ptr(dxsum), rows, cols, stream_ptr())
 
-    def _attn_fwd(self, q, q_bstride, q_ld, kv, k_off, v_off, kv_ld, o, lse, qmask, sched, ws, b, nq, layer=0):
+    def _attn_fwd(self, q, q_bstride, q_ld, kv, k_off, v_off, kv_ld, o, lse, qmask, sched, ws, b, nq, layer=0, q_hstride=0,
+                  kv_hstride=0, kv_bstride=None):
         N = self.N
         a = AttnFwdArgs()
         esz = 2
         a.q, a.q_bstride, a.q_ld = q, q_bstride, q_ld
         a.k, a.v = kv.data_ptr() + k_off * esz, kv.data_ptr() + v_off * esz
-        a.kv_bstride, a.kv_ld = N * kv_ld, kv_ld
+        a.kv_bstride, a.kv_ld = (N * kv_ld if kv_bstride is None else kv_bstride), kv_ld
+        a.q_hstride, a.kv_hstride = q_hstride, kv_hstride
         a.o, a.o_bstride, a.o_ld = o.data_ptr(), nq * o.stride(0), o.stride(0)
         a.lse = lse.data_ptr()
         a.qmask, a.keyinfo, a.ktile_flags = qmask.data_ptr(), ws["keyinfo"].data_ptr(), ws["kflags"].data_ptr()
@@ -406,7 +420,10 @@
         a.batch, a.heads, a.nq, a.nk, a.nk_pad = b, self.H, nq, N, self.nk_pad
         a.n_qtiles, a.n_ktiles, a.scale, a.flags = sched.s.n_q, sched.s.n_k, self.scale, self.attn_flags
         a.khot = ws["khot"].data_ptr() if ws.get("khot") is not None else None
-        if ws.get("present_cur") is not None:
+        if kv_hstride:
+            call("mca_attn_vmean_heads", a.v, a.kv_bstride, kv_hstride, a.kv_ld, ws["vmean"].data_ptr(), b, N, self.H, ptr(ws.get("present_cur")),
+                 (1 << self.M) - 1, stream_ptr(), profile_as="mca_attn_vmean_if_needed" if ws.get("present_cur") is not None else "mca_attn_vmean")
+        elif ws.get("present_cur") is not None:
             call("mca_attn_vmean_if_needed", a.v, a.kv_bstride, a.kv_ld, ws["vmean"].data_ptr(), b, N, self.H, ptr(ws["present_cur"]),
                  (1 << self.M) - 1, stream_ptr())
         else:
@@ -477,23 +494,37 @@
             return "bf16 one-pass" + (f" (key blocks split {self.onepass_split(b)} ways)" if self.onepass_split(b) > 1 else "")
         return "fp8 two-pass" if (self.attn_dtype == "fp8" and self.mask_mfma and self.dkv_keys == 128) else "bf16 two-pass"
 
-    def _attn_bwd1(self, q, q_bstride, q_ld, kv, k_off, v_off, kv_ld, o, d_o, lse, dq_ptr, dq_bstride, dq_ld, dkv, dk_off, dv_off, dkv_ld, ws, b):
-        N, esz, sc = self.N, 2, self.sched_onepass
+    def _attn_bwd1(self, q, q_bstride, q_ld, kv, k_off, v_off, kv_ld, o, d_o, lse, dq_ptr, dq_bstride, dq_ld, dkv, dk_off, dv_off, dkv_ld, ws, b,
+                   headmajor=False):
+        N, sc = self.N, self.sched_onepass
         if "rowc" not in ws:
             rc = torch.empty(b, self.H, sc.n_qt + 1, 2, 64, dtype=torch.float32, device=self.device)
             rc[:, :, :, 0] = float("-inf"); rc[:, :, :, 1] = 0.0
             ws["rowc"] = rc
             ws["dq_acc"] = torch.empty(b * self.H * self.onepass_split(b) * (sc.n_qt + 1) * 4096, dtype=torch.float32, device=self.device)
+        hm_b, hm_h = self.H * N * 64, N * 64
+        if headmajor:
+            call("mca_attn_bwd_rowc_onepass", o.data_ptr(), N * o.stride(0), o.stride(0), d_o.data_ptr(), hm_b, hm_h, 64, lse.data_ptr(),
+                 sc.row_slot.data_ptr(), ws["rowc"].data_ptr(), ws["dvmean"].data_ptr(), b, self.H, N, sc.n_qt, stream_ptr(),
+                 profile_as="mca_attn_bwd_prep_onepass")
+            return self._attn_bwd1_launch(q, d_o.data_ptr(), kv, k_off, v_off, hm_b, hm_h, 64, dq_ptr, dq_bstride, dq_ld, dkv, dk_off, dv_off, dkv_ld, ws, b)
+        if "q_hm" not in ws:
             ws["q_hm"] = torch.zeros((b * self.H * N + 64) * 64, dtype=torch.bfloat16, device=self.device)
             ws["do_hm"] = torch.zeros((b * self.H * N + 64) * 64, dtype=torch.bfloat16, device=self.device)
         call("mca_attn_bwd_prep_onepass", o.data_ptr(), d_o.data_ptr(), N * o.stride(0), o.stride(0), lse.data_ptr(), sc.row_slot.data_ptr(),
              ws["rowc"].data_ptr(), ws["dvmean"].data_ptr(), b, self.H, N, sc.n_qt, q, q_bstride, q_ld, ws["q_hm"].data_ptr(),
              ws["do_hm"].data_ptr(), stream_ptr())
+        self._attn_bwd1_launch(ws["q_hm"].data_ptr(), ws["do_hm"].data_ptr(), kv, k_off, v_off, N * kv_ld, 0, kv_ld, dq_ptr, dq_bstride, dq_ld, dkv,
+                               dk_off, dv_off, dkv_ld, ws, b)
+
+    def _attn_bwd1_launch(self, q_hm, do_hm, kv, k_off, v_off, kv_bstride, kv_hstride, kv_ld, dq_ptr, dq_bstride, dq_ld, dkv, dk_off, dv_off,
+                          dkv_ld, ws, b):
+        N, esz, sc = self.N, 2, self.sched_onepass
         a = AttnBwd1Args()
-        a.q, a.q_bstride, a.q_hstride, a.q_ld = ws["q_hm"].data_ptr(), self.H * N * 64, N * 64, 64
+        a.q, a.q_bstride, a.q_hstride, a.q_ld = q_hm, self.H * N * 64, N * 64, 64
         a.k, a.v = kv.data_ptr() + k_off * esz, kv.data_ptr() + v_off * esz
-        a.kv_bstride, a.kv_ld = N * kv_ld, kv_ld
-        a.d_o, a.o_bstride, a.o_hstride, a.o_ld = ws["do_hm"].data_ptr(), self.H * N * 64, N * 64, 64
+        a.kv_bstride, a.kv_hstride, a.kv_ld = kv_bstride, kv_hstride, kv_ld
+        a.d_o, a.o_bstride, a.o_hstride, a.o_ld = do_hm, self.H * N * 64, N * 64, 64
         a.rowc, a.dvmean = ws["rowc"].data_ptr(), ws["dvmean"].data_ptr()
         a.dq, a.dq_bstride, a.dq_ld = dq_ptr, dq_bstride, dq_ld
         a.dk, a.dv = dkv.data_ptr() + dk_off * esz, dkv.data_ptr() + dv_off * esz
@@ -622,14 +653,23 @@
         if ws["khot"] is not None:
             call("mca_build_keyhot", ptr(ws["keyinfo"]), ptr(ws["khot"]), b, self.nk_pad, stream_ptr())
         ln_in_gemm = self.fuse_ln_residual and T >= 2048 and D % 128 == 0 and D >= 512 and Ip >= 512
+        ws["hm"] = bool(self.L) and self.use_onepass(ws, b, N) and self.attn_dtype == "bf16" and self.dbg["headmajor"] is not False
         for i, ly in enumerate(m.layers):
             w, a = self.wl[i], ws["layers"][i]
             xin, xout = ws["x"][i], ws["x"][i + 1]
             g = ly.norm.gamma
             self.ln_fwd(xin, g, T, D, a["m1"], a["r1"], y=None if ln_in_gemm else ws["xn"], ldy=D, y_bf16=a["xn_b"], cols_pad=D)
-            self.gemm_nt(a["xn_b"], w["qkv"], a["qkv"], T, 3 * D, D)
-            self._attn_fwd(a["qkv"].data_ptr(), N * 3 * D, 3 * D, a["qkv"], D, 2 * D, 3 * D, a["o"], a["lse"],
-                           self.qmask_attn, self.sched_attn_f, ws, b, N, layer=i)
+            if ws["hm"] and not self.gemm_nt_heads(a["xn_b"], w["qkv"], a["qkv"], T, 3 * D, D, N, H):
+                if i:
+                    raise hip.MCAHipError("mca_gemm_nt_heads refused a layer after it took the first one")
+                ws["hm"] = False
+            if ws["hm"]:
+                self._attn_fwd(a["qkv"].data_ptr(), H * N * 64, 64, a["qkv"], T * D, 2 * T * D, 64, a["o"], a["lse"], self.qmask_attn,
+                               self.sched_attn_f, ws, b, N, layer=i, q_hstride=N * 64, kv_hstride=N * 64, kv_bstride=H * N * 64)
+            else:
+                self.gemm_nt(a["xn_b"], w["qkv"], a["qkv"], T, 3 * D, D)
+                self._attn_fwd(a["qkv"].data_ptr(), N * 3 * D, 3 * D, a["qkv"], D, 2 * D, 3 * D, a["o"], a["lse"],
+                               self.qmask_attn, self.sched_attn_f, ws, b, N, layer=i)
             if ln_in_gemm:
                 call("mca_gemm_nt_lnres", ptr(a["o"]), D, ptr(w["o"]), D, ptr(a["x1"]), D, ptr(xin), D, ptr(a["m1"]), ptr(a["r1"]),
                      ptr(g.data), T, D, D, stream_ptr(), flops=2.0 * T * D * D)
@@ -782,10 +822,16 @@
             self.ln_bwd(dx_other, D, a["x1"], g, a["m2"], a["r2"], T, D, G(g), dx=dx, dx_bf16=dx1)
             if not grouped:
                 on_side(lambda dx1=dx1, a=a, ly=ly: tn(dx1, a["o"], G(ly.attn.to_out.weight), T, D, D))
-            self.gemm_nt(dx1, w["oT"], ws["do"], T, D, D)
-            self._attn_bwd2(a["qkv"].data_ptr(), N * 3 * D, 3 * D, a["qkv"], D, 2 * D, 3 * D, a["o"], ws["do"], a["lse"],
-                            ws["delta"], dqkv.data_ptr(), N * 3 * D, 3 * D, False, dqkv, D, 2 * D, 3 * D, self.qmask_attn,
-                            self.sched_attn_f, self.sched_attn_b2, ws, b, N, layer=i)
+            if ws["hm"]:
+                if not self.gemm_nt_heads(dx1, w["oT"], ws["do"], T, D, D, N, H):
+                    raise hip.MCAHipError("mca_gemm_nt_heads refused dO after the forward wrote q | k | v head-major")
+                self._attn_bwd1(a["qkv"].data_ptr(), H * N * 64, 64, a["qkv"], T * D, 2 * T * D, 64, a["o"], ws["do"], a["lse"], dqkv.data_ptr(),
+                                N * 3 * D, 3 * D, dqkv, D, 2 * D, 3 * D, ws, b, headmajor=True)
+            else:
+                self.gemm_nt(dx1, w["oT"], ws["do"], T, D, D)
+                self._attn_bwd2(a["qkv"].data_ptr(), N * 3 * D, 3 * D, a["qkv"], D, 2 * D, 3 * D, a["o"], ws["do"], a["lse"],
+                                ws["delta"], dqkv.data_ptr(), N * 3 * D, 3 * D, False, dqkv, D, 2 * D, 3 * D, self.qmask_attn,
+                                self.sched_attn_f, self.sched_attn_b2, ws, b, N, layer=i)
             gq = G(ly.attn.to_q.weight)
             assert G(ly.attn.to_kv.weight).data_ptr() == gq.data_ptr() + D * D * 4
             if grouped:
diff --git a/mca-paper_amd/hip.py b/mca-paper_amd/hip.py
--- a/mca-paper_amd/hip.py
+++ b/mca-paper_amd/hip.py
@@ -58,6 +58,7 @@
         ("batch", C.c_int), ("heads", C.c_int), ("nq", C.c_int), ("nk", C.c_int), ("nk_pad", C.c_int),
         ("n_qtiles", C.c_int), ("n_ktiles", C.c_int), ("scale", C.c_float), ("flags", C.c_int),
         ("khot", C.c_void_p),
+        ("q_hstride", C.c_int64), ("kv_hstride", C.c_int64),
     ]
 
 
@@ -107,6 +108,7 @@
         ("n_qtiles", C.c_int), ("n_kblocks", C.c_int), ("max_list", C.c_int), ("n_entries", C.c_int),
         ("batch", C.c_int), ("heads", C.c_int), ("n", C.c_int), ("nk_pad", C.c_int), ("n_ktiles64", C.c_int),
         ("scale", C.c_float), ("flags", C.c_int), ("split", C.c_int),
+        ("kv_hstride", C.c_int64),
     ]
 
 
@@ -120,6 +122,7 @@
     "mca_segment_mean_fwd": (_I, [_P, _P, _P, _I, _P, _P, _I, _I, _I, _P]),
     "mca_segment_mean_bwd": (_I, [_P, _P, _P, _P, _I, _P, _I, _I, _I, _P]),
     "mca_gemm_nt": (_I, [_P, _I64, _P, _I64, _P, _I64, _I, _P, _P, _I64, _I64, _I64, _I64, _I64, _P]),
+    "mca_gemm_nt_heads": (_I, [_P, _I64, _P, _I64, _P, _I64, _I64, _I64, _I64, _I64, _P]),
     "mca_gemm_nt_geglu_bwd": (_I, [_P, _I64, _P, _I64, _P, _P, _I64, _I64, _I64, _I64, _P]),
     "mca_gemm_nt_lnres": (_I, [_P, _I64, _P, _I64, _P, _I64, _P, _I64, _P, _P, _P, _I64, _I64, _I64, _P]),
     "mca_gemm_nt_geglu_fwd": (_I, [_P, _I64, _P, _I64, _P, _I64, _P, _I64, _I64, _I64, _I64, _P]),
@@ -141,12 +144,14 @@
     "mca_build_keyinfo": (_I, [_P, _P, _P, _P, _I, _I, _I, _P]),
     "mca_attn_vmean": (_I, [_P, _I64, _I64, _P, _I, _I, _I, _P]),
     "mca_attn_vmean_if_needed": (_I, [_P, _I64, _I64, _P, _I, _I, _I, _P, _I, _P]),
+    "mca_attn_vmean_heads": (_I, [_P, _I64, _I64, _I64, _P, _I, _I, _I, _P, _I, _P]),
     "mca_attn_fwd": (_I, [C.POINTER(AttnFwdArgs), _P]),
     "mca_attn_quant_mxfp8": (_I, [_P, _I64, _I64, _P, _P, _I64, _I64, C.POINTER(AttnFp8Operands), _I, _I, _I, _P]),
     "mca_attn_fwd_fp8": (_I, [C.POINTER(AttnFwdArgs), C.POINTER(AttnFp8Operands), _P]),
     "mca_attn_bwd_prep": (_I, [_P, _P, _I64, _I64, _P, _P, _P, _I, _I, _I, _I, _P]),
     "mca_attn_bwd_onepass": (_I, [C.POINTER(AttnBwd1Args), _P]),
     "mca_attn_bwd_prep_onepass": (_I, [_P, _P, _I64, _I64, _P, _P, _P, _P, _I, _I, _I, _I, _P, _I64, _I64, _P, _P, _P]),
+    "mca_attn_bwd_rowc_onepass": (_I, [_P, _I64, _I64, _P, _I64, _I64, _I64, _P, _P, _P, _P, _I, _I, _I, _I, _P]),
     "mca_attn_bwd_dq": (_I, [C.POINTER(AttnBwd2Args), _P]),
     "mca_attn_bwd_dkv": (_I, [C.POINTER(AttnBwd2Args), _P]),
     "mca_attn_quant_bwd_mxfp8": (_I, [_P, _I64, _I64, _P, _P, _I64, _I64, _P, _I64, _I64, C.POINTER(AttnFp8BwdOperands), _I, _I, _I, _I, _P]),
@@ -290,12 +295,17 @@
     return prof["totals"]
 
 
-def call(name: str, *args, flops: float = 0.0):
-    if PROFILE is not None and _PROFILE_ON and name in PROFILE["names"]:
+def call(name: str, *args, flops: float = 0.0, profile_as: Optional[str] = None, may_refuse: bool = False) -> bool:
+    key = profile_as or name
+    timed = PROFILE is not None and _PROFILE_ON and key in PROFILE["names"]
+    if timed:
         s, e = torch.cuda.Event(enable_timing=True), torch.cuda.Event(enable_timing=True)
         s.record()
-        check(getattr(lib(), name)(*args), name)
+    rc = getattr(lib(), name)(*args)
+    if may_refuse and rc == -3:
+        return False
+    check(rc, name)
+    if timed:
         e.record()
-        PROFILE["records"].setdefault(name + ("/" + _TAG if _TAG else ""), []).append((s, e, flops))
-        return
-    check(getattr(lib(), name)(*args), name)
+        PROFILE["records"].setdefault(key + ("/" + _TAG if _TAG else ""), []).append((s, e, flops))
+    return True
```

Result: no change. 1725 samples/s (median of 6 runs) (+0.4%).
